# DhayaaAnbajagane/Baryonification

Measured on AMD Instinct MI355X. Metric: halos/sec for BaryonifyShell NSIDE=1024 (1000000-halo synthetic catalog), higher is better.
Workload: dtype f64 throughout in the parity-grade mode: f64 ring-row geometry, f64 pair math with 1e-11 elementary functions (fp32 seeds + one Newton step), f64 LDS accumulation, pix_offsets stored as two f32 arrays (hi + lo), f64 regrid geometry, f64 map

## Files before the change

### baryonification_amd/csrc/bfgx_api.hip

```cpp
#include <hip/hip_runtime.h>
#include <cmath>
#include <cstdarg>
#include <cstdio>
#include <algorithm>
#include <climits>
#include <cstdint>
#include <cstdlib>
#include <chrono>
#include <cstring>
#include <functional>
#include <map>
#include <mutex>
#include <string>
#include <tuple>
#include <type_traits>
#include <vector>

#include "../../include/bfgx.h"

#include "bfgx_devmem.hpp"
#include "bfgx_tile_arena.hpp"
#include "bfgx_cosmo.hpp"
#include "bfgx_kernels.hpp"
#include "bfgx_scatter2.hpp"
#include "bfgx_regrid2.hpp"
#include "bfgx_tables.hpp"
#include "bfgx_scan.hpp"
#include "bfgx_grid.hpp"
#include "bfgx_grid_pairs.hpp"
#include "bfgx_fft.hpp"
#include "bfgx_bispec.hpp"
#include "bfgx_deposit.hpp"
#include "bfgx_deposit_cloud.hpp"
#include "bfgx_snapshot.hpp"
#include "bfgx_snapshot_pairs.hpp"
#include "bfgx_grid_gather.hpp"
#include "bfgx_fftlog.hpp"
#include "bfgx_sht.hpp"
#include "bfgx_hpx.hpp"
#include "bfgx_mapstats.hpp"
#include "bfgx_pcl.hpp"
#include "bfgx_stack_core.hpp"
#include "bfgx_stack.hpp"
#include "bfgx_snapshot_stack.hpp"
#include "bfgx_grid_stack.hpp"
#include "bfgx_math_probe.hpp"

using namespace bfgx;

namespace {

thread_local std::string g_err;

int fail(int code, const char *fmt, ...)
{
    char buf[512];
    va_list ap;
    va_start(ap, fmt);
    vsnprintf(buf, sizeof(buf), fmt, ap);
    va_end(ap);
    g_err = buf;
    return code;
}

int alloc_fail(const char *what) { return fail(BFGX_ERR_HIP, kDevAllocFailed, what); }

#define HIP_TRY(expr)                                                                          \
    do {                                                                                       \
        hipError_t e_ = (expr);                                                                \
        if (e_ != hipSuccess)                                                                  \
            return fail(BFGX_ERR_HIP, "%s failed: %s (%s:%d)", #expr, hipGetErrorString(e_), __FILE__, __LINE__); \
    } while (0)

int select_device(int device)
{
    if (bfgx_device_count() <= 0) return fail(BFGX_ERR_NO_DEVICE, "no HIP device visible: libbfgx has no CPU fallback");
    HIP_TRY(hipSetDevice(device));
    return BFGX_OK;
}

int validate_cosmo(const bfgx_cosmo &c)
{
    if (!(c.Omega_m > 0) || !(c.h > 0) || !(c.Omega_b >= 0) || c.w0 != c.w0)
        return fail(BFGX_ERR_INVALID, "cosmology needs Omega_m > 0, h > 0, Omega_b >= 0, finite w0");
    return BFGX_OK;
}

int validate_table(const bfgx_table &t)
{
    if (t.ndim < 3 || t.ndim > BFGX_MAX_DIM) return fail(BFGX_ERR_INVALID, "table ndim must be in [3, %d]", BFGX_MAX_DIM);
    if (!t.values) return fail(BFGX_ERR_INVALID, "table values pointer is NULL");
    for (int d = 0; d < t.ndim; ++d) {
        if (t.n[d] < 2) return fail(BFGX_ERR_INVALID, "table axis %d needs >= 2 points", d);
        if (!t.axis[d]) return fail(BFGX_ERR_INVALID, "table axis %d pointer is NULL", d);
        for (int i = 1; i < t.n[d]; ++i)
            if (!(t.axis[d][i] > t.axis[d][i - 1]))
                return fail(BFGX_ERR_INVALID, "table axis %d must be strictly ascending", d);
    }
    double tot = 1.0;
    for (int d = 0; d < t.ndim; ++d) tot *= t.n[d];
    if (tot > 2.0e9) return fail(BFGX_ERR_INVALID, "table too large for 32-bit row offsets");
    return BFGX_OK;
}

int device_cu_count(int device)
{
    hipDeviceProp_t prop;
    return (hipGetDeviceProperties(&prop, device) == hipSuccess && prop.multiProcessorCount > 0) ? prop.multiProcessorCount : 256;
}

struct KernelEvents {
    using Pair = std::pair<hipEvent_t, hipEvent_t>;
    bool timing = false;
    std::vector<Pair> ev[BFGX_NUM_KERNELS], ev_free;
    int enable(int on) { timing = on != 0; return BFGX_OK; }
    int read(int device, hipStream_t stream, double *ms_sum, int64_t *launches)
    {
        if (!ms_sum || !launches) return fail(BFGX_ERR_INVALID, "NULL argument");
        HIP_TRY(hipSetDevice(device));
        HIP_TRY(hipStreamSynchronize(stream));
        for (int k = 0; k < BFGX_NUM_KERNELS; ++k) {
            double tot = 0.0;
            for (auto &e : ev[k]) {
                float ms = 0.f;
                HIP_TRY(hipEventElapsedTime(&ms, e.first, e.second));
                tot += ms;
                ev_free.push_back(e);
            }
            ms_sum[k] = tot;
            launches[k] = (int64_t)ev[k].size();
            ev[k].clear();
        }
        return BFGX_OK;
    }
    void destroy()
    {
        for (int k = 0; k < BFGX_NUM_KERNELS; ++k)
            for (auto &e : ev[k]) { (void)hipEventDestroy(e.first); (void)hipEventDestroy(e.second); }
        for (auto &e : ev_free) { (void)hipEventDestroy(e.first); (void)hipEventDestroy(e.second); }
    }
};

}

struct bfgx_plan {
    int device = 0, num_cus = 256;
    hipStream_t stream = nullptr;
    int64_t nside = 0, max_halos = 0;
    Hpx hpx;
    DevModel model;
    DevList mem;
    HaloRec *recs = nullptr;
    RowSetX *rowsx = nullptr;
    int NC = 4;
    int algo = 1;
    bool blocking_growth = false;
    float *k0_work_est = nullptr;
    int32_t *k1_form = nullptr;
    int64_t k1_nhalos = 0;
    int k1_fluid = 1;
    Tiling tiling;
    TileArena arena;
    int32_t *tile_start = nullptr, *entries = nullptr, *overflow = nullptr;
    int32_t *entries_a = nullptr, *slow_list = nullptr, *slow_cnt = nullptr;
    int32_t entries_a_cap = 0;
    int32_t cnt_pad = 1;
    TileRef *tref = nullptr;
    FarList far;
    int32_t *regrid_lean = nullptr;
    int auto_acc = 0;
    double table_disp_pixels = 0.0;
    int32_t *tile_apron = nullptr;
    int band_reach = 1;
    int route_margin = 0;
    int64_t cat_blk_rows = 0, cat_blk_stride = 0;
    ScanScratch scan;
    bool fast_ok = false;
    RowRec *rowrec = nullptr;
    void *pairrec = nullptr;
    FbRec *fbrec = nullptr;
    const float *tab8f = nullptr;
    const double *tab8d = nullptr;
    unsigned long long *pair_total = nullptr;
    double *tile_sums = nullptr;
    std::vector<int32_t> band_tile0_host;
    int64_t capacity = 0;
    KernelEvents events;
};

namespace {

template <class Plan>
struct KernelTimerT {
    Plan *p; int kind; KernelEvents::Pair e{nullptr, nullptr};
    KernelTimerT(Plan *p_, int kind_) : p(p_), kind(kind_)
    {
        KernelEvents &k = p->events;
        if (!k.timing) return;
        if (!k.ev_free.empty()) { e = k.ev_free.back(); k.ev_free.pop_back(); }
        else { (void)hipEventCreate(&e.first); (void)hipEventCreate(&e.second); }
        (void)hipEventRecord(e.first, p->stream);
    }
    ~KernelTimerT()
    {
        if (!p->events.timing) return;
        (void)hipEventRecord(e.second, p->stream);
        p->events.ev[kind].push_back(e);
    }
};
using KernelTimer = KernelTimerT<bfgx_plan>;

template <typename T>
static int owned_upload(DevList &mem, hipStream_t stream, const T *host, size_t count, const T *&dev_out)
{
    HIP_TRY(mem.upload(dev_out, host, count, stream));
    return BFGX_OK;
}
template <typename T>
static int owned_upload(DevList &mem, hipStream_t stream, const std::vector<T> &v, const T *&dev_out)
{
    return owned_upload(mem, stream, v.data(), v.size(), dev_out);
}

template <typename T>
static int grow_list(DevList &mem, T *&ptr, int64_t &capacity, int64_t needed)
{
    const int64_t cap = needed + needed / 4 + 1024;
    HIP_TRY(mem.regrow(ptr, (size_t)cap));
    capacity = cap;
    return BFGX_OK;
}

static int validate_model(const bfgx_model *model)
{
    if (int rc = validate_cosmo(model->cosmo_runner)) return rc;
    if (int rc = validate_cosmo(model->cosmo_model)) return rc;
    if (int rc = validate_table(model->table)) return rc;
    if (!(model->eps_runner > 0)) return fail(BFGX_ERR_INVALID, "epsilon_max must be > 0");
    if (!(model->massdef_runner.Delta > 0) || !(model->massdef_model.Delta > 0))
        return fail(BFGX_ERR_INVALID, "mass definition needs numeric Delta > 0");
    return BFGX_OK;
}

static int upload_model(DevList &mem, hipStream_t stream, const bfgx_model *model, bool with_da, DevModel &m, int &NC)
{
    const bfgx_table &t = model->table;
    std::memset(&m, 0, sizeof(m));
    m.tab.ndim = t.ndim;
    size_t nvals = 1;
    for (int d = 0; d < t.ndim; ++d) {
        m.tab.n[d] = t.n[d];
        nvals *= (size_t)t.n[d];
        if (int rc = owned_upload(mem, stream, t.axis[d], (size_t)t.n[d], m.tab.axis[d])) return rc;
    }
    {
        std::vector<double> tr;
        const double *src = t.values;
        if (t.ndim > 3) {
            const size_t nz = t.n[0], nm = t.n[1], nr = t.n[2];
            size_t nx = 1;
            for (int d = 3; d < t.ndim; ++d) nx *= (size_t)t.n[d];
            tr.resize(nvals);
            for (size_t zm = 0; zm < nz * nm; ++zm)
                for (size_t ir = 0; ir < nr; ++ir)
                    for (size_t q = 0; q < nx; ++q)
                        tr[(zm * nx + q) * nr + ir] = t.values[(zm * nr + ir) * nx + q];
            src = tr.data();
        }
        if (int rc = owned_upload(mem, stream, src, nvals, m.tab.values)) return rc;
        std::vector<float> v32(nvals);
        for (size_t q = 0; q < nvals; ++q) v32[q] = (float)src[q];
        if (int rc = owned_upload(mem, stream, v32, m.tab.values32)) return rc;
        HIP_TRY(hipStreamSynchronize(stream));
        NC = 4 << (t.ndim - 3);
    }
    m.tab.rdelta = t.rdelta_sampling;
    m.tab.logv = t.log_values;
    m.tab.eps_model = t.eps_model;
    {
        const double *g = t.axis[2];
        const int n = t.n[2];
        const double step = (g[n - 1] - g[0]) / (n - 1);
        bool uni = true;
        for (int i = 0; i < n; ++i)
            if (std::fabs(g[i] - (g[0] + i * step)) > 1e-9 * std::fabs(step)) { uni = false; break; }
        m.tab.r_uniform = uni ? 1 : 0;
        m.tab.r0 = g[0];
        m.tab.r1 = g[n - 1];
        m.tab.inv_dr = 1.0 / step;
    }
    m.bg_runner = make_background(model->cosmo_runner);
    m.bg_model = make_background(model->cosmo_model);
    m.md_runner = model->massdef_runner;
    m.md_model = model->massdef_model;
    m.eps_runner = model->eps_runner;
    m.same_model = (std::memcmp(&m.bg_runner, &m.bg_model, sizeof(Background)) == 0 && m.md_runner.Delta == m.md_model.Delta &&
                    m.md_runner.rho_type == m.md_model.rho_type) ? 1 : 0;
    if (with_da) {
        std::vector<double> knots, coef;
        da_spline(m.bg_runner, knots, coef);
        if (int rc = owned_upload(mem, stream, coef, m.da_coef)) return rc;
        m.da_step = kDaZmax / (kDaKnots - 1);
        HIP_TRY(hipStreamSynchronize(stream));
    }
    return BFGX_OK;
}

static int check_catalog(const bfgx_plan *p, const bfgx_catalog *c)
{
    if (!p || !c) return fail(BFGX_ERR_INVALID, "NULL argument");
    if (c->n < 0 || c->n > p->max_halos) return fail(BFGX_ERR_INVALID, "catalog size %lld exceeds plan max_halos %lld",
                                                     (long long)c->n, (long long)p->max_halos);
    if (c->n > 0 && (!c->M || !c->z || !c->ra || !c->dec)) return fail(BFGX_ERR_INVALID, "catalog column pointer is NULL");
    for (int k = 0; k < p->model.tab.ndim - 3; ++k)
        if (c->n > 0 && !c->extra[k]) return fail(BFGX_ERR_INVALID, "catalog is missing the column of table parameter axis %d", k);
    return BFGX_OK;
}

static bool use_fast(const bfgx_plan *p) { return p->fast_ok && p->algo == 1; }

struct DispMode {
    enum Kind { F32, F64, SPLIT } kind = F32;
    bool fp64() const { return kind != F32; }
    bool split() const { return kind == SPLIT; }
    size_t pixel_bytes() const { return fp64() ? 24 : 12; }
    float *lo(const void *offsets, int64_t n) const { return split() ? (float *)offsets + 3 * (size_t)n : nullptr; }
    int acc() const { return kind == F32 ? BFGX_ACC_F32 : kind == F64 ? BFGX_ACC_F64 : BFGX_ACC_PARITY; }
};

static int disp_mode(const bfgx_plan *p, int acc, bool one_array, DispMode &m)
{
    if (!p) return fail(BFGX_ERR_INVALID, "NULL plan");
    if (acc != BFGX_ACC_AUTO && acc != BFGX_ACC_F32 && acc != BFGX_ACC_F64 && acc != BFGX_ACC_PARITY)
        return fail(BFGX_ERR_INVALID, "acc_f64 = %d: must be BFGX_ACC_AUTO (-1), 0 (f32), 1 (f64) or BFGX_ACC_PARITY (3)", acc);
    if (acc == BFGX_ACC_AUTO) acc = p->auto_acc;
    const bool parity = acc == BFGX_ACC_PARITY && use_fast(p);
    m.kind = acc == BFGX_ACC_F32 ? DispMode::F32 : (parity && !one_array) ? DispMode::SPLIT : DispMode::F64;
    return BFGX_OK;
}

struct PaintMode {
    enum Kind { F32, F64, MIXED } kind = F64;
    bool map_f64() const { return kind != F32; }
    bool k0_f64() const { return kind == F64; }
    bool pair_f32() const { return kind == MIXED; }
};

static int paint_mode(const bfgx_plan *p, int acc, PaintMode &m)
{
    if (!p) return fail(BFGX_ERR_INVALID, "NULL plan");
    if (acc < 0 || acc > 2) return fail(BFGX_ERR_INVALID, "acc_f64 must be 0, 1 or 2");
    m.kind = acc == 0 ? PaintMode::F32 : (acc == 2 && use_fast(p)) ? PaintMode::MIXED : PaintMode::F64;
    return BFGX_OK;
}

struct TileLaunch {
    float *offsets_lo = nullptr;
    bool paint_pair_f32 = false;
    float *omax = nullptr;
    int tile_lo = 0, tile_n = -1;
    int spread_tiles = -1;
};

static int launch_prep(bfgx_plan *p, const bfgx_catalog *c, int fallback4, bool bin, bool f64, bool rec_all)
{
    if (c->n == 0) return BFGX_OK;
    const unsigned grid = (unsigned)((c->n + 255) / 256);
    KernelTimer kt(p, BFGX_K_PREP);
    PrepOut o;
    std::memset(&o, 0, sizeof(o));
    o.rec = p->recs; o.rowsx = p->rowsx;
    o.fast = (bin && use_fast(p)) ? 1 : 0;
    o.rec_all = (rec_all || !o.fast) ? 1 : 0;
    o.rowrec = p->rowrec; o.pairrec = p->pairrec; o.fbrec = p->fbrec;
    if (bin) {
        o.tref = p->tref; o.cnt_a = p->arena.cnt_a_pad; o.cnt_b = p->arena.cnt_b;
        o.cnt_pad = p->cnt_pad;
        o.work_est = o.fast ? p->k0_work_est : nullptr;
        o.entries_a = p->entries_a; o.cap_a = p->entries_a_cap; o.slow_list = p->slow_list; o.slow_cnt = p->slow_cnt;
    }
    o.ncell_m = p->model.tab.n[1] - 1; o.nrm1 = p->model.tab.n[2] - 1;
    o.blk_rows = p->cat_blk_rows; o.blk_stride = p->cat_blk_stride;
    ExtraCols ex;
    for (int k = 0; k < BFGX_MAX_EXTRA; ++k) ex.p[k] = c->extra[k];
#define BFGX_PREP(NCV, REAL)                                                                                        \
    hipLaunchKernelGGL((halo_prep_kernel<NCV, REAL>), dim3(grid), dim3(256), 0, p->stream, p->model, p->hpx, c->n, c->M, c->z, \
                       c->ra, c->dec, ex, c->ln1pz, c->lnM, fallback4, p->tiling, o)
    if (p->NC == 4) { if (f64) BFGX_PREP(4, double); else BFGX_PREP(4, float); }
    else if (p->NC == 8) BFGX_PREP(8, float);
    else if (p->NC == 16) BFGX_PREP(16, float);
    else if (p->NC == 32) BFGX_PREP(32, float);
    else BFGX_PREP(64, float);
#undef BFGX_PREP
    HIP_TRY(hipGetLastError());
    return BFGX_OK;
}

static int launch_place(bfgx_plan *p, const bfgx_catalog *c)
{
    const unsigned grid = (unsigned)((c->n + 255) / 256);
    hipLaunchKernelGGL(tile_place_kernel, dim3(grid), dim3(256), 0, p->stream, p->hpx, p->tiling, c->n,
                       (const TileRef *)p->tref, (const int32_t *)p->tile_start, p->arena.cur_b, p->entries, p->capacity, p->overflow,
                       (const int32_t *)p->slow_list, (const int32_t *)p->slow_cnt);
    HIP_TRY(hipGetLastError());
    return BFGX_OK;
}

static int launch_prep_and_bin(bfgx_plan *p, const bfgx_catalog *c, int fallback4, bool f64)
{
    p->k1_nhalos = c->n;
    HIP_TRY(hipMemsetAsync(p->arena.base, 0, p->arena.zeroed_bytes, p->stream));
    if (int rc = launch_prep(p, c, fallback4, true, f64, false)) return rc;
    KernelTimer kt(p, BFGX_K_BIN);
    const int nt_i = p->tiling.ntiles, nsb = (nt_i + kScanTilesPerWg - 1) / kScanTilesPerWg;
    const int32_t *cnt = p->arena.cnt_b;
    if (nsb <= 1 || nsb > 1024) {
        hipLaunchKernelGGL(tile_scan_kernel, dim3(1), dim3(1024), 0, p->stream, nt_i, cnt, p->tile_start);
    } else {
        int32_t *tot = p->scan.block_tot, *off = p->scan.block_off;
        hipLaunchKernelGGL(tile_scan_part_kernel<0>, dim3(nsb), dim3(1024), 0, p->stream, nt_i, cnt, p->tile_start, tot, (const int32_t *)off);
        hipLaunchKernelGGL(tile_scan_blocks_kernel, dim3(1), dim3(1024), 0, p->stream, nsb, nt_i, (const int32_t *)tot, off, p->tile_start);
        hipLaunchKernelGGL(tile_scan_part_kernel<1>, dim3(nsb), dim3(1024), 0, p->stream, nt_i, cnt, p->tile_start, tot, (const int32_t *)off);
    }
    HIP_TRY(hipGetLastError());
    if (c->n > 0) if (int rc = launch_place(p, c)) return rc;
    return BFGX_OK;
}

template <int MODE, typename ACC>
static int launch_scatter(bfgx_plan *p, int64_t n, ACC *out, int64_t *counts)
{
    if (n == 0) return BFGX_OK;
    const unsigned grid = (unsigned)((n + kWavesPerBlock - 1) / kWavesPerBlock);
    KernelTimer kt(p, MODE == MODE_OFFSETS ? BFGX_K_OFFSETS : (MODE == MODE_PAINT ? BFGX_K_PAINT : BFGX_K_COUNT));
    hipLaunchKernelGGL((halo_scatter_kernel<MODE, ACC>), dim3(grid), dim3(kWave * kWavesPerBlock), 0, p->stream,
                       make_pair_table(p->model.tab), p->hpx, n, (const HaloRec *)p->recs, out, counts);
    HIP_TRY(hipGetLastError());
    return BFGX_OK;
}

template <int MODE, typename ACC, int NC>
static int launch_tile_scatter_nc(bfgx_plan *p, ACC *out, const TileLaunch &k)
{
    constexpr int NCOMP = (MODE == MODE_OFFSETS) ? 3 : 1;
    const size_t lds = tile_lds_bytes<NC>(p->tiling.BR, p->tiling.W, NCOMP);
    auto kern = tile_scatter_kernel<MODE, ACC, NC>;
    HIP_TRY(hipFuncSetAttribute((const void *)kern, hipFuncAttributeMaxDynamicSharedMemorySize, (int)lds));
    KernelTimer kt(p, MODE == MODE_OFFSETS ? BFGX_K_OFFSETS : (MODE == MODE_PAINT ? BFGX_K_PAINT : BFGX_K_COUNT));
    const int grid = k.tile_n < 0 ? p->tiling.ntiles : std::max(k.tile_n, 1);
    hipLaunchKernelGGL(kern, dim3(grid), dim3(kWave * kWavesPerBlock), lds, p->stream,
                       make_pair_table(p->model.tab), p->hpx, p->tiling, (const HaloRec *)p->recs, (const RowSetX *)p->rowsx,
                       (const int32_t *)p->tile_start, (const int32_t *)p->entries, p->capacity, out, p->pair_total,
                       (unsigned int *)k.omax, k.tile_lo, k.tile_n);
    HIP_TRY(hipGetLastError());
    return BFGX_OK;
}

template <int MODE, typename ACC, typename real, int PM = 0>
static int launch_tile_scatter2(bfgx_plan *p, ACC *out, const TileLaunch &k, ACC *out_lo = nullptr)
{
    constexpr int NCOMP = (MODE == MODE_OFFSETS) ? 3 : 1;
    constexpr int kNP = 1;
    const size_t lds = tile2_lds_bytes<real>(p->tiling.BR, p->tiling.W, NCOMP);
    auto kern = tile_scatter2_kernel<MODE, ACC, real, kNP, PM>;
    HIP_TRY(hipFuncSetAttribute((const void *)kern, hipFuncAttributeMaxDynamicSharedMemorySize, (int)lds));
    Tab8T<real> tb;
    tb.v = (sizeof(real) == 4) ? (const real *)p->tab8f : (const real *)p->tab8d;
    tb.r0 = (real)p->model.tab.r0; tb.r1 = (real)p->model.tab.r1; tb.inv_dr = (real)p->model.tab.inv_dr;
    tb.nr = p->model.tab.n[2]; tb._pad = 0;
    unsigned int *tile_counter = p->arena.tile_counter;
    const int ntodo = k.tile_n < 0 ? p->tiling.ntiles : std::max(k.tile_n, 1);
    KernelTimer kt(p, MODE == MODE_OFFSETS ? BFGX_K_OFFSETS : (MODE == MODE_PAINT ? BFGX_K_PAINT : BFGX_K_COUNT));
    int32_t *form = nullptr;
    if constexpr (MODE != MODE_COUNT) {
        const size_t ldsf = tile2f_lds_bytes<real>(p->tiling.BR, p->tiling.W, NCOMP);
        const bool eligible = p->k1_fluid && ldsf <= (size_t)160 * 1024 && p->tiling.BR <= kWave && ntodo >= 2 * p->num_cus;
        const int nspread = k.spread_tiles > 0 ? k.spread_tiles : ntodo;
        const bool dense = (double)p->k1_nhalos * (double)p->tiling.ntiles >= 6.0e5 * (double)nspread;
        const bool forced = p->k1_fluid == 2 && ldsf <= (size_t)160 * 1024 && p->tiling.BR <= kWave;
        if (eligible && !dense && !forced && p->k0_work_est && p->k1_nhalos > 0) {
            const int nblk = (int)((p->k1_nhalos + 255) / 256);
            hipLaunchKernelGGL(k1_form_kernel, dim3(1), dim3(1024), 0, p->stream, nblk, (const float *)p->k0_work_est, 4800.0f * (float)nspread, p->k1_form);
            form = p->k1_form;
        }
        if (forced || (eligible && (dense || form))) {
            auto kf = tile_scatter2f_kernel<MODE, ACC, real, PM>;
            HIP_TRY(hipFuncSetAttribute((const void *)kf, hipFuncAttributeMaxDynamicSharedMemorySize, (int)ldsf));
            const int gridf = std::min(ntodo, p->num_cus);
            hipLaunchKernelGGL(kf, dim3(std::max(gridf, 1)), dim3(kWave * FluidWaves<real>::n), ldsf, p->stream, tb, p->hpx, p->tiling,
                               (const RowRec *)p->rowrec, (const PairRecT<real> *)p->pairrec, (const FbRec *)p->fbrec,
                               (const int32_t *)p->tile_start, (const int32_t *)p->arena.cnt_a_pad, (const int32_t *)p->arena.cnt_b,
                               (const int32_t *)p->entries, p->capacity, (const int32_t *)p->entries_a, (int)p->entries_a_cap, (int)p->cnt_pad, out, out_lo, tile_counter,
                               (unsigned int *)k.omax, k.tile_lo, k.tile_n, p->overflow, (const int32_t *)form, 1);
            HIP_TRY(hipGetLastError());
            if (!form) return BFGX_OK;
        }
    }
    const int grid = std::min(ntodo, 2 * p->num_cus);
    hipLaunchKernelGGL(kern, dim3(grid), dim3(kWave * kW2), lds, p->stream, tb, p->hpx, p->tiling,
                       (const RowRec *)p->rowrec, (const PairRecT<real> *)p->pairrec, (const FbRec *)p->fbrec,
                       (const int32_t *)p->tile_start, (const int32_t *)p->arena.cnt_a_pad, (const int32_t *)p->arena.cnt_b,
                       (const int32_t *)p->entries, p->capacity, (const int32_t *)p->entries_a, (int)p->entries_a_cap, (int)p->cnt_pad, out, out_lo, p->pair_total, tile_counter,
                       (unsigned int *)k.omax, k.tile_lo, k.tile_n, (const int32_t *)form, 0);
    HIP_TRY(hipGetLastError());
    return BFGX_OK;
}

template <int MODE, typename ACC>
static int launch_tile_scatter(bfgx_plan *p, ACC *out, const TileLaunch &k)
{
    if (use_fast(p)) {
        using real = typename std::conditional<sizeof(ACC) == 8, double, float>::type;
        if constexpr (MODE == MODE_OFFSETS && sizeof(ACC) == 4) {
            if (k.offsets_lo) return launch_tile_scatter2<MODE, ACC, double, 1>(p, out, k, (ACC *)k.offsets_lo);
        }
        if constexpr (MODE == MODE_PAINT && sizeof(ACC) == 8) {
            if (k.paint_pair_f32) return launch_tile_scatter2<MODE, ACC, float>(p, out, k);
        }
        return launch_tile_scatter2<MODE, ACC, real>(p, out, k);
    }
    if (p->NC == 4) return launch_tile_scatter_nc<MODE, ACC, 4>(p, out, k);
    if (MODE == MODE_COUNT) return launch_tile_scatter_nc<MODE, ACC, 4>(p, out, k);
    if (p->NC == 8) return launch_tile_scatter_nc<MODE, ACC, 8>(p, out, k);
    if (p->NC == 16) return launch_tile_scatter_nc<MODE, ACC, 16>(p, out, k);
    if (p->NC == 32) return launch_tile_scatter_nc<MODE, ACC, 32>(p, out, k);
    return launch_tile_scatter_nc<MODE, ACC, 64>(p, out, k);
}

static int ensure_entry_capacity(bfgx_plan *p, const bfgx_catalog *c)
{
    int32_t ov = 0, total = 0;
    HIP_TRY(hipMemcpyAsync(&ov, p->overflow, sizeof(ov), hipMemcpyDeviceToHost, p->stream));
    HIP_TRY(hipMemcpyAsync(&total, p->tile_start + p->tiling.ntiles, sizeof(total), hipMemcpyDeviceToHost, p->stream));
    HIP_TRY(hipStreamSynchronize(p->stream));
    if (!(ov & 1)) return BFGX_OK;
    HIP_TRY(p->mem.regrow(p->entries, (size_t)total + 16));
    p->capacity = (int64_t)total + 16;
    HIP_TRY(hipMemsetAsync(p->overflow, 0, sizeof(int32_t), p->stream));
    HIP_TRY(hipMemsetAsync(p->arena.cur_b, 0, p->arena.cursor_bytes, p->stream));
    return launch_place(p, c);
}

template <typename real>
static void build_tab8(const bfgx_table &t, std::vector<real> &out)
{
    const size_t nz = t.n[0], nm = t.n[1], nr = t.n[2];
    out.resize((nz - 1) * (nm - 1) * (nr - 1) * 8);
    for (size_t iz = 0; iz + 1 < nz; ++iz)
        for (size_t im = 0; im + 1 < nm; ++im)
            for (size_t i = 0; i + 1 < nr; ++i) {
                real *o = out.data() + ((iz * (nm - 1) + im) * (nr - 1) + i) * 8;
                for (int c = 0; c < 4; ++c) {
                    const double *row = t.values + ((iz + (c >> 1)) * nm + im + (c & 1)) * nr;
                    o[2 * c] = (real)row[i];
                    o[2 * c + 1] = (real)(row[i + 1] - row[i]);
                }
            }
}

static void build_tiling(int64_t nside, bool paint, int &BR, int &W, std::vector<int32_t> &tile0, std::vector<int32_t> &nphi,
                         std::vector<int32_t> &nrmin, std::vector<int32_t> &tband)
{
    auto pow2_floor = [](int64_t v) { int p = 1; while (2 * p <= v) p *= 2; return p; };
    W = std::max(16, std::min(64, pow2_floor(std::max<int64_t>(1, nside / 2))));
    BR = std::max(4, std::min(paint ? 64 : 32, pow2_floor(std::max<int64_t>(1, nside / 8))));
    if (const char *e = std::getenv("BFGX_TILE_W")) W = pow2_floor(std::max(4, std::min(64, std::atoi(e))));
    if (const char *e = std::getenv("BFGX_TILE_BR")) BR = std::max(1, std::min(64, std::atoi(e)));
    const int64_t nrings = 4 * nside - 1;
    const int nbands = (int)((nrings + BR - 1) / BR);
    auto rlen = [&](int64_t ring) { return 4 * (ring < nside ? ring : (ring > 3 * nside ? 4 * nside - ring : nside)); };
    tile0.assign(nbands + 1, 0); nphi.assign(nbands, 1); nrmin.assign(nbands, 4);
    for (int b = 0; b < nbands; ++b) {
        const int64_t i0 = 1 + (int64_t)b * BR, i1 = std::min<int64_t>(i0 + BR, 4 * nside);
        int64_t lmax = 0, lmin = INT64_MAX;
        for (int64_t i = i0; i < i1; ++i) { lmax = std::max(lmax, rlen(i)); lmin = std::min(lmin, rlen(i)); }
        nphi[b] = (int)((lmax + W - 1) / W);
        nrmin[b] = (int)lmin;
        tile0[b + 1] = tile0[b] + nphi[b];
    }
    tband.resize(tile0[nbands]);
    for (int b = 0; b < nbands; ++b)
        for (int t = tile0[b]; t < tile0[b + 1]; ++t) tband[t] = b;
}


constexpr double kAutoDispPixels = 0.1;
static void plan_pick_precision(bfgx_plan *p, const bfgx_model *model)
{
    const bfgx_table &t = model->table;
    p->auto_acc = BFGX_ACC_F32;
    p->table_disp_pixels = 0.0;
    if (t.log_values) return;
    const Background bgr = make_background(model->cosmo_runner), bgm = make_background(model->cosmo_model);
    const double pix = std::sqrt(4.0 * 3.14159265358979323846 / (double)p->hpx.npix);
    const size_t nz = t.n[0], nm = t.n[1], nr = t.n[2];
    size_t nx = 1;
    for (int d = 3; d < t.ndim; ++d) nx *= (size_t)t.n[d];
    double worst = 0.0;
    for (size_t iz = 0; iz < nz; ++iz) {
        const double z = std::exp(t.axis[0][iz]) - 1.0, a = 1.0 / (1.0 + z);
        const double D = z > 0.0 ? angular_diameter_distance(bgr, z) : 0.0;
        for (size_t im = 0; im < nm; ++im) {
            const double M = std::exp(t.axis[1][im]);
            if (!(M > 0.0) || !(a > 0.0)) continue;
            const double Rm = radius_delta(bgm, model->massdef_model, M, a) / a, Rr = radius_delta(bgr, model->massdef_runner, M, a) / a;
            const double rcut = std::min(t.eps_model * Rm, model->eps_runner * Rr);
            for (size_t ir = 0; ir < nr; ++ir) {
                const double r = std::exp(t.axis[2][ir]) * (t.rdelta_sampling ? Rm : 1.0);
                double m = 0.0;
                const double *v = t.values + ((iz * nm + im) * nr + ir) * nx;
                for (size_t q = 0; q < nx; ++q) if (std::isfinite(v[q])) m = std::max(m, std::fabs(v[q]));
                const double px = (D > 0.0) ? m * a / D / pix : (m > 0.0 ? 1.0e30 : 0.0);
                worst = std::max(worst, px);
                if (r >= rcut) break;
            }
        }
    }
    p->table_disp_pixels = worst;
    if (worst > kAutoDispPixels) p->auto_acc = BFGX_ACC_PARITY;
}

static int plan_init_fast(bfgx_plan *p, const bfgx_table &t, size_t nh)
{
    const size_t n8 = (size_t)(t.n[0] - 1) * (size_t)(t.n[1] - 1) * (size_t)(t.n[2] - 1) * 8;
    p->fast_ok = (t.ndim == 3) && p->model.tab.r_uniform && n8 * sizeof(double) <= ((size_t)256 << 20);
    if (!p->fast_ok) return BFGX_OK;
    std::vector<float> v32;
    std::vector<double> v64;
    build_tab8<float>(t, v32);
    build_tab8<double>(t, v64);
    if (int rc = owned_upload(p->mem, p->stream, v32, p->tab8f)) return rc;
    if (int rc = owned_upload(p->mem, p->stream, v64, p->tab8d)) return rc;
    if (hipStreamSynchronize(p->stream) != hipSuccess) return fail(BFGX_ERR_HIP, "stream sync failed");
    PairRecT<double> *pairrec = nullptr;
    if (p->mem.alloc(p->rowrec, nh)) return alloc_fail("row records");
    if (p->mem.alloc(pairrec, nh)) return alloc_fail("pair records");
    p->pairrec = pairrec;
    if (p->mem.alloc(p->fbrec, nh)) return alloc_fail("fallback records");
    return BFGX_OK;
}

static int plan_init_binning(bfgx_plan *p, const bfgx_table &t, size_t nh)
{
    int BR, W;
    std::vector<int32_t> tile0, nphi, nrmin, tband;
    build_tiling(p->nside, t.log_values != 0, BR, W, tile0, nphi, nrmin, tband);
    Tiling &T = p->tiling;
    T.BR = BR; T.W = W; T.nbands = (int)nphi.size(); T.ntiles = (int)tband.size();
    if (int rc = owned_upload(p->mem, p->stream, tile0, T.band_tile0)) return rc;
    p->band_tile0_host = tile0;
    if (int rc = owned_upload(p->mem, p->stream, nphi, T.band_nphi)) return rc;
    if (int rc = owned_upload(p->mem, p->stream, nrmin, T.band_nrmin)) return rc;
    if (int rc = owned_upload(p->mem, p->stream, tband, T.tile_band)) return rc;
    std::vector<int32_t> order(tband.size());
    {
        std::vector<double> weight(tband.size());
        for (size_t q = 0; q < tband.size(); ++q) { order[q] = (int32_t)q; weight[q] = (double)nrmin[tband[q]] / (double)nphi[tband[q]]; }
        std::stable_sort(order.begin(), order.end(), [&](int32_t x, int32_t y) { return weight[x] > weight[y]; });
    }
    if (int rc = owned_upload(p->mem, p->stream, order, T.tile_order)) return rc;
    {
        RingRec *rings = nullptr;
        const size_t nrec = (size_t)(4 * p->nside + 1);
        if (p->mem.alloc(rings, nrec)) return alloc_fail("ring table");
        hipLaunchKernelGGL(ring_table_kernel, dim3((unsigned)((nrec + 255) / 256)), dim3(256), 0, p->stream, p->hpx, rings);
        if (hipGetLastError() != hipSuccess) return fail(BFGX_ERR_HIP, "ring table launch failed");
        T.rings = rings;
    }
    if (hipStreamSynchronize(p->stream) != hipSuccess) return fail(BFGX_ERR_HIP, "stream sync failed");
    p->capacity = 8 * p->max_halos + 4096;
    if (const char *e = std::getenv("BFGX_K1_FLUID")) p->k1_fluid = std::max(0, std::min(2, std::atoi(e)));
    if (const char *e = std::getenv("BFGX_ENTRY_CAP")) p->capacity = std::max<int64_t>(16, std::atoll(e));
    p->cnt_pad = kCntPadMax;
    while (p->cnt_pad > 1 && (size_t)T.ntiles * p->cnt_pad * sizeof(int32_t) > ((size_t)4 << 20)) p->cnt_pad >>= 1;
    const TileArenaLayout AL = tile_arena_layout((size_t)T.ntiles, (size_t)p->cnt_pad);
    int32_t *arena = nullptr;
    if (p->mem.alloc(arena, AL.total_words) || p->mem.alloc(p->tile_start, (size_t)T.ntiles + 1) ||
        p->mem.alloc(p->entries, (size_t)p->capacity) || p->mem.alloc(p->overflow, 1) || p->mem.alloc(p->pair_total, 1) || p->mem.alloc(p->tref, nh))
        return alloc_fail("binning workspace");
    p->arena.bind(arena, AL);
    const double mean = 1.3 * (double)std::max<int64_t>(p->max_halos, 1) / (double)T.ntiles;
    int cap_a = 64;
    while (cap_a < 32768 && (double)cap_a < (mean > 512.0 ? 4.0 : 16.0) * mean + 64.0) cap_a <<= 1;
    while (cap_a > 64 && (size_t)T.ntiles * cap_a * sizeof(int32_t) > ((size_t)1 << 30)) cap_a >>= 1;
    if (const char *e = std::getenv("BFGX_TILE_LIST_CAP")) cap_a = std::max(1, std::atoi(e));
    const size_t nblk = (nh + 255) / 256;
    if (p->mem.alloc(p->k0_work_est, nblk) || p->mem.alloc(p->k1_form, 4)) return alloc_fail("work estimate");
    if (p->mem.alloc(p->entries_a, (size_t)T.ntiles * cap_a) || p->mem.alloc(p->slow_list, nblk * 256) || p->mem.alloc(p->slow_cnt, nblk))
        return alloc_fail("tile lists");
    p->entries_a_cap = cap_a;
    return BFGX_OK;
}

static int plan_init_regrid(bfgx_plan *p)
{
    const Tiling &T = p->tiling;
    const int64_t npx = p->hpx.npix;
    const int64_t want = p->table_disp_pixels < 0.25 ? npx / 16 : (p->table_disp_pixels < 2.0 ? npx / 2 : 4 * npx);
    p->far.cap = std::min<int64_t>(std::max<int64_t>((int64_t)1 << 20, want), (int64_t)1 << 28);
    if (const char *e = std::getenv("BFGX_FAR_CAP")) p->far.cap = std::max<int64_t>(1024, std::atoll(e));
    if (p->mem.alloc(p->far.pix, (size_t)p->far.cap) || p->mem.alloc(p->far.val, (size_t)p->far.cap) ||
        p->mem.alloc(p->tile_apron, 2 * (size_t)(T.ntiles + 1)))
        return alloc_fail("far list");
    if (p->mem.alloc(p->regrid_lean, (size_t)(T.ntiles + 4))) return alloc_fail("lean tile list");
    if (hipMemsetAsync(p->regrid_lean, 0, sizeof(int32_t) * 4, p->stream) != hipSuccess) return fail(BFGX_ERR_HIP, "hipMemset failed");
    p->far.count = &p->arena.ctrl->far_count;
    p->far.overflow = p->arena.band_overflow;
    if (hipMemsetAsync(p->arena.ctrl, 0, p->arena.tail_bytes, p->stream) != hipSuccess) return fail(BFGX_ERR_HIP, "hipMemset failed");
    return BFGX_OK;
}

}

extern "C" {

int bfgx_abi_version(void) { return BFGX_ABI_VERSION; }

const char *bfgx_last_error(void) { return g_err.c_str(); }

int bfgx_device_count(void)
{
    int n = 0;
    if (hipGetDeviceCount(&n) != hipSuccess) return 0;
    return n;
}

int bfgx_cosmo_E2(const bfgx_cosmo *c, int64_t n, const double *a, double *out)
{
    if (!c || !a || !out) return fail(BFGX_ERR_INVALID, "NULL argument");
    if (int rc = validate_cosmo(*c)) return rc;
    const Background b = make_background(*c);
    for (int64_t i = 0; i < n; ++i) out[i] = E2(b, a[i]);
    return BFGX_OK;
}

int bfgx_cosmo_radius(const bfgx_cosmo *c, const bfgx_massdef *md, int64_t n, const double *M, const double *a, double *out)
{
    if (!c || !md || !M || !a || !out) return fail(BFGX_ERR_INVALID, "NULL argument");
    if (int rc = validate_cosmo(*c)) return rc;
    const Background b = make_background(*c);
    for (int64_t i = 0; i < n; ++i) out[i] = radius_delta(b, *md, M[i], a[i]);
    return BFGX_OK;
}

int bfgx_cosmo_angular_diameter_distance(const bfgx_cosmo *c, int64_t n, const double *z, double *out)
{
    if (!c || !z || !out) return fail(BFGX_ERR_INVALID, "NULL argument");
    if (int rc = validate_cosmo(*c)) return rc;
    const Background b = make_background(*c);
    for (int64_t i = 0; i < n; ++i) out[i] = angular_diameter_distance(b, z[i]);
    return BFGX_OK;
}

int bfgx_cosmo_da_spline(const bfgx_cosmo *c, double *knots, double *coef)
{
    if (!c || !knots || !coef) return fail(BFGX_ERR_INVALID, "NULL argument");
    if (int rc = validate_cosmo(*c)) return rc;
    std::vector<double> k, cf;
    da_spline(make_background(*c), k, cf);
    std::memcpy(knots, k.data(), k.size() * sizeof(double));
    std::memcpy(coef, cf.data(), cf.size() * sizeof(double));
    return BFGX_OK;
}

int bfgx_cosmo_da_eval(const bfgx_cosmo *c, int64_t n, const double *z, double *out)
{
    if (!c || !z || !out) return fail(BFGX_ERR_INVALID, "NULL argument");
    if (int rc = validate_cosmo(*c)) return rc;
    std::vector<double> k, cf;
    da_spline(make_background(*c), k, cf);
    for (int64_t i = 0; i < n; ++i) out[i] = da_eval(k, cf, z[i]);
    return BFGX_OK;
}

int bfgx_plan_create(int device, void *hip_stream, int64_t nside, int64_t max_halos,
                     const bfgx_model *model, bfgx_plan **out)
{
    if (!model || !out) return fail(BFGX_ERR_INVALID, "NULL argument");
    *out = nullptr;
    if (nside < 1 || nside > 8192) return fail(BFGX_ERR_INVALID, "nside must be 1 .. 8192 (the tile kernels index pixels with 32 bits inside a ring table)");
    if (max_halos < 0) return fail(BFGX_ERR_INVALID, "max_halos < 0");
    if (int rc = validate_model(model)) return rc;
    if (bfgx_device_count() <= 0)
        return fail(BFGX_ERR_NO_DEVICE, "no HIP device visible: libbfgx has no CPU fallback");
    HIP_TRY(hipSetDevice(device));

    bfgx_plan *p = new bfgx_plan();
    p->device = device;
    {
        int cus = 0;
        if (hipDeviceGetAttribute(&cus, hipDeviceAttributeMultiprocessorCount, device) == hipSuccess && cus > 0) p->num_cus = cus;
    }
    p->nside = nside;
    p->max_halos = max_halos;
    p->hpx = make_hpx(nside);
    p->stream = (hipStream_t)hip_stream;
    auto bail = [&](int rc) { bfgx_plan_destroy(p); return rc; };

    const bfgx_table &t = model->table;
    if (int rc = upload_model(p->mem, p->stream, model, true, p->model, p->NC)) return bail(rc);
    plan_pick_precision(p, model);
    const size_t nh = (size_t)(max_halos > 0 ? max_halos : 1);
    if (p->mem.alloc(p->recs, nh)) return bail(alloc_fail("halo records"));
    if (p->NC > 4 && p->mem.alloc(p->rowsx, nh)) return bail(alloc_fail("corner rows"));
    if (int rc = plan_init_fast(p, t, nh)) return bail(rc);
    if (int rc = plan_init_binning(p, t, nh)) return bail(rc);
    if (int rc = plan_init_regrid(p)) return bail(rc);
    const ScanScratchLayout SL = scan_scratch_layout();
    int32_t *scan = nullptr;
    if (p->mem.alloc(scan, SL.total_words)) return bail(alloc_fail("tile scan scratch"));
    p->scan.bind(scan, SL);
    if (p->mem.alloc(p->tile_sums, 2 * (size_t)(p->tiling.ntiles + 1))) return bail(alloc_fail("tile sums"));
    if (hipMemsetAsync(p->overflow, 0, sizeof(int32_t), p->stream) != hipSuccess) return bail(fail(BFGX_ERR_HIP, "hipMemset failed"));
    if (hipStreamSynchronize(p->stream) != hipSuccess) return bail(fail(BFGX_ERR_HIP, "stream sync failed"));
    *out = p;
    return BFGX_OK;
}

int bfgx_plan_timing_enable(bfgx_plan *p, int on)
{
    return p ? p->events.enable(on) : fail(BFGX_ERR_INVALID, "NULL plan");
}

int bfgx_plan_timing_read(bfgx_plan *p, double *ms_sum, int64_t *launches)
{
    return p ? p->events.read(p->device, p->stream, ms_sum, launches) : fail(BFGX_ERR_INVALID, "NULL argument");
}

void bfgx_plan_destroy(bfgx_plan *p)
{
    if (!p) return;
    (void)hipSetDevice(p->device);
    (void)hipStreamSynchronize(p->stream);
    p->events.destroy();
    p->mem.release();
    delete p;
}

int bfgx_plan_set_algo(bfgx_plan *p, int algo)
{
    if (!p || (algo != 0 && algo != 1)) return fail(BFGX_ERR_INVALID, "algo must be 0 (per-halo global atomics) or 1 (LDS tiles)");
    p->algo = algo;
    return BFGX_OK;
}

int bfgx_plan_status(bfgx_plan *p)
{
    if (!p) return fail(BFGX_ERR_INVALID, "NULL plan");
    HIP_TRY(hipSetDevice(p->device));
    int32_t ov = 0;
    HIP_TRY(hipMemcpyAsync(&ov, p->overflow, sizeof(ov), hipMemcpyDeviceToHost, p->stream));
    HIP_TRY(hipStreamSynchronize(p->stream));
    if (ov & 4) {
        HIP_TRY(hipMemsetAsync(p->overflow, 0, sizeof(int32_t), p->stream));
        return fail(BFGX_ERR_HIP, "tile_scatter2f_kernel: a wave gave up waiting inside its workgroup; results are incomplete (BFGX_K1_FLUID=0 selects the other form)");
    }
    if (ov) return fail(BFGX_ERR_INVALID, "halo->tile entry list overflowed its capacity (%lld); results are incomplete",
                        (long long)p->capacity);
    int32_t fov = 0;
    HIP_TRY(hipMemcpyAsync(&fov, p->far.overflow, sizeof(fov), hipMemcpyDeviceToHost, p->stream));
    HIP_TRY(hipStreamSynchronize(p->stream));
    if (fov) {
        HIP_TRY(hipMemsetAsync(p->far.overflow, 0, sizeof(int32_t), p->stream));
        return fail(BFGX_ERR_INVALID, "the regrid's list of far deposits overflowed (%lld entries): displacements of many pixels over a large "
                                      "part of the map", (long long)p->far.cap);
    }
    return BFGX_OK;
}

int bfgx_plan_precision(bfgx_plan *p, int acc_requested, int32_t *acc_resolved, double *table_disp_pixels)
{
    DispMode m;
    if (int rc = disp_mode(p, acc_requested, false, m)) return rc;
    if (acc_resolved) *acc_resolved = m.acc();
    if (table_disp_pixels) *table_disp_pixels = p->table_disp_pixels;
    return BFGX_OK;
}

static ReachArgs reach_args(const bfgx_plan *p, double cap)
{
    const double ns = (double)p->hpx.nside, om = 1.0 / (3.0 * ns * ns);
    const double th1 = std::atan2(std::sqrt(om * (2.0 - om)), 1.0 - om);
    return ReachArgs{p->tile_apron, cap, th1, 3.14159265358979323846 - th1};
}

static int64_t ring_first_pixel(const Hpx &h, int64_t ring)
{
    const int64_t ns = h.nside, nl4 = 4 * ns;
    if (ring < 1) return 0;
    if (ring >= nl4) return h.npix;
    const int64_t q = nl4 - ring;
    return (ring < ns) ? 2 * ring * (ring - 1) : (ring < 3 * ns) ? h.ncap + (ring - ns) * 4 * ns : h.npix - 2 * q * (q + 1);
}

struct BandRange { int64_t p0, p1; int t0, nt; };
static BandRange band_range(const bfgx_plan *p, int b0, int b1)
{
    const auto first_pixel = [p](int b) { return ring_first_pixel(p->hpx, 1 + (int64_t)p->tiling.BR * b); };
    return BandRange{first_pixel(b0), first_pixel(b1), p->band_tile0_host[b0], p->band_tile0_host[b1] - p->band_tile0_host[b0]};
}

static int check_band_range(const bfgx_plan *p, int32_t b0, int32_t b1, bool tiles = false)
{
    if (tiles && p->algo != 1) return fail(BFGX_ERR_UNSUPPORTED, "band-restricted passes need the tiled algorithm (algo 1)");
    return (b0 < 0 || b1 > p->tiling.nbands || b0 > b1) ? fail(BFGX_ERR_INVALID, "band range out of bounds") : BFGX_OK;
}

static int check_scatter(const bfgx_plan *p, const bfgx_catalog *cat, const void *out, bool paint, bool bands = false, int32_t band0 = 0, int32_t band1 = 0)
{
    if (int rc = check_catalog(p, cat)) return rc;
    if (bands) if (int rc = check_band_range(p, band0, band1, true)) return rc;
    if ((p->model.tab.logv != 0) != paint) return fail(BFGX_ERR_INVALID, paint ? "profile painting needs a table with log_values = 1"
                                                                               : "displacement read-out needs a table with log_values = 0");
    if ((!bands || band0 < band1) && !out) return fail(BFGX_ERR_INVALID, paint ? "map pointer is NULL" : "offsets pointer is NULL");
    return BFGX_OK;
}

static int launch_k0(bfgx_plan *p, const bfgx_catalog *cat, int fallback4, bool f64)
{
    HIP_TRY(hipSetDevice(p->device));
    if (p->algo == 1) {
        if (int rc = launch_prep_and_bin(p, cat, fallback4, f64)) return rc;
        return p->blocking_growth ? ensure_entry_capacity(p, cat) : BFGX_OK;
    }
    if (p->NC != 4) return fail(BFGX_ERR_UNSUPPORTED, "tables with extra parameter axes need algo 1 (LDS tiles)");
    return launch_prep(p, cat, fallback4, false, false, true);
}

static int launch_offsets(bfgx_plan *p, const DispMode &m, void *slice, int64_t p0, int64_t p1, TileLaunch k1)
{
    if (m.split()) k1.offsets_lo = m.lo(slice, p1 - p0) - 3 * p0;
    if (m.kind != DispMode::F64) return launch_tile_scatter<MODE_OFFSETS, float>(p, (float *)slice - 3 * p0, k1);
    return launch_tile_scatter<MODE_OFFSETS, double>(p, (double *)slice - 3 * p0, k1);
}

static int offsets_impl(bfgx_plan *p, const bfgx_catalog *cat, void *offsets_dev, const DispMode &m, const TileLaunch &k1)
{
    if (int rc = check_scatter(p, cat, offsets_dev, false)) return rc;
    if (int rc = launch_k0(p, cat, 1, m.fp64())) return rc;
    if (p->algo == 1) return launch_offsets(p, m, offsets_dev, 0, p->hpx.npix, k1);
    if (m.fp64()) return launch_scatter<MODE_OFFSETS, double>(p, cat->n, (double *)offsets_dev, nullptr);
    return launch_scatter<MODE_OFFSETS, float>(p, cat->n, (float *)offsets_dev, nullptr);
}

int bfgx_offsets_device(bfgx_plan *p, const bfgx_catalog *cat, void *offsets_dev, int acc_f64)
{
    DispMode m;
    if (int rc = disp_mode(p, acc_f64, false, m)) return rc;
    return offsets_impl(p, cat, offsets_dev, m, TileLaunch{});
}

static int launch_paint(bfgx_plan *p, const PaintMode &m, void *slice, int64_t p0, TileLaunch k3)
{
    k3.paint_pair_f32 = m.pair_f32();
    if (m.map_f64()) return launch_tile_scatter<MODE_PAINT, double>(p, (double *)slice - p0, k3);
    return launch_tile_scatter<MODE_PAINT, float>(p, (float *)slice - p0, k3);
}

int bfgx_max_offset2_device(bfgx_plan *p, const void *offsets_dev, int64_t npixels, int acc_f64, float *out_dev)
{
    if (!p || !out_dev || (npixels > 0 && !offsets_dev)) return fail(BFGX_ERR_INVALID, "NULL argument");
    if (npixels < 0) return fail(BFGX_ERR_INVALID, "npixels < 0");
    DispMode m;
    if (int rc = disp_mode(p, acc_f64, true, m)) return rc;
    HIP_TRY(hipSetDevice(p->device));
    HIP_TRY(hipMemsetAsync(out_dev, 0, sizeof(float), p->stream));
    if (npixels > 0) {
        const unsigned grid = (unsigned)std::min<int64_t>((npixels + 255) / 256, 1024);
        if (m.fp64()) hipLaunchKernelGGL(max_offset_kernel<double>, dim3(grid), dim3(256), 0, p->stream, npixels, (const double *)offsets_dev, (unsigned *)out_dev);
        else hipLaunchKernelGGL(max_offset_kernel<float>, dim3(grid), dim3(256), 0, p->stream, npixels, (const float *)offsets_dev, (unsigned *)out_dev);
        HIP_TRY(hipGetLastError());
    }
    return BFGX_OK;
}

int bfgx_plan_set_catalog_blocks(bfgx_plan *p, int64_t rows, int64_t stride)
{
    if (!p) return fail(BFGX_ERR_INVALID, "NULL plan");
    if (rows < 0 || (rows > 0 && stride < rows)) return fail(BFGX_ERR_INVALID, "blocked catalog: rows >= 0, stride >= rows");
    p->cat_blk_rows = rows; p->cat_blk_stride = rows > 0 ? stride : 0;
    return BFGX_OK;
}

int bfgx_plan_tile_shape(bfgx_plan *p, int32_t *rings_per_band, int32_t *max_columns)
{
    if (!p) return fail(BFGX_ERR_INVALID, "NULL plan");
    if (rings_per_band) *rings_per_band = p->tiling.BR;
    if (max_columns) *max_columns = p->tiling.W;
    return BFGX_OK;
}

static int paint_impl(bfgx_plan *p, const bfgx_catalog *cat, void *map_out_dev, const PaintMode &m)
{
    if (int rc = check_scatter(p, cat, map_out_dev, true)) return rc;
    if (int rc = launch_k0(p, cat, 0, m.k0_f64())) return rc;
    if (p->algo == 1) return launch_paint(p, m, map_out_dev, 0, TileLaunch{});
    if (m.map_f64()) return launch_scatter<MODE_PAINT, double>(p, cat->n, (double *)map_out_dev, nullptr);
    return launch_scatter<MODE_PAINT, float>(p, cat->n, (float *)map_out_dev, nullptr);
}

int bfgx_paint_device(bfgx_plan *p, const bfgx_catalog *cat, void *map_out_dev, int acc_f64)
{
    PaintMode m;
    if (int rc = paint_mode(p, acc_f64, m)) return rc;
    return paint_impl(p, cat, map_out_dev, m);
}

}

constexpr int kSumTilesOneWg = 16384;
static int launch_tile_sums(bfgx_plan *p, int t0, int nt, double *sums_dev)
{
    const double *ts = p->tile_sums + 2 * (size_t)t0;
    if (nt <= kSumTilesOneWg) hipLaunchKernelGGL(sum_tiles_kernel, dim3(1), dim3(256), 0, p->stream, nt, ts, sums_dev);
    else {
        HIP_TRY(hipMemsetAsync(sums_dev, 0, 2 * sizeof(double), p->stream));
        hipLaunchKernelGGL(sum_tiles_multi_kernel, dim3(64), dim3(256), 0, p->stream, nt, ts, sums_dev);
    }
    return BFGX_OK;
}

template <typename ACC, typename real, bool SPLIT = false>
static void launch_regrid_gather(bfgx_plan *p, const double *map_in_dev, const ACC *o, const ACC *o_lo, double *map_out_dev, double *ts, bool from_k1, double *sums_dev)
{
    const size_t lds = regrid3_lds_bytes(p->tiling.BR, p->tiling.W, sizeof(real)),
                 lds_walk = regrid3_lds_bytes(p->tiling.BR, p->tiling.W, sizeof(real), true, SPLIT ? sizeof(ACC) : sizeof(real));
    FarList far = p->far;
    far.overflow = p->arena.far_overflow_full;
    const int nt = p->tiling.ntiles, nfix = std::min(nt, 2 * p->num_cus), nwalk = std::min(nt, 4 * p->num_cus);
    const ReachArgs reach = reach_args(p, regrid_cap(p->hpx.nside));
    if (!from_k1)
        hipLaunchKernelGGL(tile_reach_kernel<ACC>, dim3(nt), dim3(256), 0, p->stream, p->hpx, p->tiling, o, p->arena.omax);
    hipLaunchKernelGGL(tile_apron_kernel, dim3((nt + 255) / 256), dim3(256), 0, p->stream, p->hpx, p->tiling, (const float *)p->arena.omax, 0,
                       reach.cap, 0, nt, p->tile_apron, p->arena.todo, p->regrid_lean);
    hipLaunchKernelGGL((tile_regrid3_kernel<ACC, real, 0, SPLIT>), dim3(std::min(nt, 8 * p->num_cus)), dim3(256), lds, p->stream, p->hpx, p->tiling, map_in_dev, o, o_lo,
                       map_out_dev, far, reach, ts, -1, nt, p->regrid_lean, (double *)nullptr);
    hipLaunchKernelGGL((tile_regrid3_kernel<ACC, real, 2, SPLIT>), dim3(nwalk), dim3(256), lds_walk, p->stream, p->hpx, p->tiling, map_in_dev, o, o_lo,
                       map_out_dev, far, reach, ts, -1, nt, p->arena.todo, (double *)nullptr);
    const bool many = nt > kSumTilesOneWg && sums_dev != nullptr && ts != nullptr;
    hipLaunchKernelGGL((tile_regrid3_kernel<ACC, real, 1, SPLIT>), dim3(nfix), dim3(256), lds, p->stream, p->hpx, p->tiling, map_in_dev, o, o_lo,
                       map_out_dev, far, reach, ts, -1, nt, p->arena.todo, many ? (double *)nullptr : sums_dev, p->regrid_lean);
    if (many) (void)launch_tile_sums(p, 0, nt, sums_dev);
}

extern "C" {

static int regrid_impl(bfgx_plan *p, const double *map_in_dev, const void *offsets_dev, const DispMode &m, double *map_out_dev, double *sums_dev,
                       bool from_k1)
{
    HIP_TRY(hipSetDevice(p->device));
    {
    KernelTimer kt(p, BFGX_K_REGRID);
    if (p->algo == 1) {
        if (!from_k1) HIP_TRY(hipMemsetAsync(p->arena.ctrl, 0, sizeof(RegridCtrl), p->stream));
        double *ts = sums_dev ? p->tile_sums : nullptr;
        if (m.split())
            launch_regrid_gather<float, double, true>(p, map_in_dev, (const float *)offsets_dev, m.lo(offsets_dev, p->hpx.npix),
                                                      map_out_dev, ts, from_k1, sums_dev);
        else if (m.fp64()) launch_regrid_gather<double, double>(p, map_in_dev, (const double *)offsets_dev, (const double *)nullptr, map_out_dev, ts, from_k1, sums_dev);
        else launch_regrid_gather<float, float>(p, map_in_dev, (const float *)offsets_dev, (const float *)nullptr, map_out_dev, ts, from_k1, sums_dev);
    } else {
        const unsigned grid = (unsigned)((p->hpx.npix + 255) / 256);
        if (m.fp64())
            hipLaunchKernelGGL(regrid_kernel<double>, dim3(grid), dim3(256), 0, p->stream, p->hpx, map_in_dev,
                               (const double *)offsets_dev, map_out_dev);
        else
            hipLaunchKernelGGL(regrid_kernel<float>, dim3(grid), dim3(256), 0, p->stream, p->hpx, map_in_dev,
                               (const float *)offsets_dev, map_out_dev);
    }
    }
    HIP_TRY(hipGetLastError());
    if (sums_dev) {
        if (p->algo != 1) {
            KernelTimer kt(p, BFGX_K_SUM);
            HIP_TRY(hipMemsetAsync(sums_dev, 0, 2 * sizeof(double), p->stream));
            hipLaunchKernelGGL(sum2_kernel, dim3(1024), dim3(256), 0, p->stream, p->hpx.npix, map_in_dev,
                               (const double *)map_out_dev, sums_dev);
            HIP_TRY(hipGetLastError());
        }
    }
    return BFGX_OK;
}

int bfgx_regrid_device(bfgx_plan *p, const double *map_in_dev, const void *offsets_dev, int acc_f64,
                       double *map_out_dev, double *sums_dev)
{
    if (!p || !map_in_dev || !offsets_dev || !map_out_dev) return fail(BFGX_ERR_INVALID, "NULL argument");
    DispMode m;
    if (int rc = disp_mode(p, acc_f64, false, m)) return rc;
    return regrid_impl(p, map_in_dev, offsets_dev, m, map_out_dev, sums_dev, false);
}

int bfgx_baryonify_device(bfgx_plan *p, const bfgx_catalog *cat, const double *map_in_dev, void *offsets_work_dev, int acc_f64,
                          double *map_out_dev, double *sums_dev)
{
    if (!p || !map_in_dev || !offsets_work_dev || !map_out_dev) return fail(BFGX_ERR_INVALID, "NULL argument");
    DispMode m;
    if (int rc = disp_mode(p, acc_f64, false, m)) return rc;
    TileLaunch k1;
    const bool fused = p->algo == 1;
    if (fused) k1.omax = p->arena.omax;
    if (int rc = offsets_impl(p, cat, offsets_work_dev, m, k1)) return rc;
    return regrid_impl(p, map_in_dev, offsets_work_dev, m, map_out_dev, sums_dev, fused);
}

int bfgx_count_pairs_device(bfgx_plan *p, const bfgx_catalog *cat, int fallback4, int64_t *counts_dev, int64_t *total_host)
{
    if (int rc = check_catalog(p, cat)) return rc;
    HIP_TRY(hipSetDevice(p->device));
    if (p->algo == 1 && !counts_dev) {
        HIP_TRY(hipMemsetAsync(p->pair_total, 0, sizeof(unsigned long long), p->stream));
        if (int rc = launch_prep_and_bin(p, cat, fallback4, false)) return rc;
        if (int rc = launch_tile_scatter<MODE_COUNT, float>(p, (float *)nullptr, TileLaunch{})) return rc;
        unsigned long long tot = 0;
        HIP_TRY(hipMemcpyAsync(&tot, p->pair_total, sizeof(tot), hipMemcpyDeviceToHost, p->stream));
        HIP_TRY(hipStreamSynchronize(p->stream));
        if (total_host) *total_host = (int64_t)tot;
        return bfgx_plan_status(p);
    }
    int64_t *counts = counts_dev;
    DevBuf tmp;
    if (!counts) {
        HIP_TRY(tmp.alloc(sizeof(int64_t) * (size_t)(cat->n > 0 ? cat->n : 1)));
        counts = tmp.as<int64_t>();
    }
    int rc = launch_prep(p, cat, fallback4, false, false, true);
    if (!rc) rc = launch_scatter<MODE_COUNT, float>(p, cat->n, (float *)nullptr, counts);
    if (!rc && total_host) {
        std::vector<int64_t> h((size_t)cat->n);
        if (hipMemcpyAsync(h.data(), counts, sizeof(int64_t) * (size_t)cat->n, hipMemcpyDeviceToHost, p->stream) != hipSuccess ||
            hipStreamSynchronize(p->stream) != hipSuccess)
            rc = fail(BFGX_ERR_HIP, "count copy-back failed");
        else {
            int64_t tot = 0;
            for (int64_t v : h) tot += v;
            *total_host = tot;
        }
    } else if (!rc) {
        if (hipStreamSynchronize(p->stream) != hipSuccess) rc = fail(BFGX_ERR_HIP, "stream sync failed");
    }
    return rc;
}

}

#include "bfgx_shell_bands.inc"

#include "bfgx_route_api.inc"

#include "bfgx_oneshot.hpp"

namespace {

constexpr int kCatCols = 4 + BFGX_MAX_EXTRA + 2;
constexpr bool catalog_col_used(int i, int nex) { return i < 4 + nex || i >= 4 + BFGX_MAX_EXTRA; }

int catalog_columns(const bfgx_catalog *h, int nex, std::vector<double> &hostlog, const double *src[kCatCols])
{
    const double *lnz = h->ln1pz, *lnm = h->lnM;
    if (h->n > 0 && (!lnz || !lnm)) {
        if (!h->M || !h->z) return fail(BFGX_ERR_INVALID, "catalog column pointer is NULL");
        hostlog.resize(2 * (size_t)h->n);
        for (int64_t i = 0; i < h->n; ++i) {
            const double a = 1.0 / (1.0 + h->z[i]);
            hostlog[i] = std::log(1.0 / a);
            hostlog[(size_t)h->n + i] = std::log(h->M[i]);
        }
        if (!lnz) lnz = hostlog.data();
        if (!lnm) lnm = hostlog.data() + h->n;
    }
    src[0] = h->M; src[1] = h->z; src[2] = h->ra; src[3] = h->dec;
    for (int k = 0; k < BFGX_MAX_EXTRA; ++k) src[4 + k] = k < nex ? h->extra[k] : nullptr;
    src[4 + BFGX_MAX_EXTRA] = lnz; src[5 + BFGX_MAX_EXTRA] = lnm;
    for (int i = 0; i < kCatCols; ++i)
        if (catalog_col_used(i, nex) && h->n > 0 && !src[i]) return fail(BFGX_ERR_INVALID, "catalog column pointer is NULL");
    return BFGX_OK;
}

void catalog_view(int64_t n, int nex, const double *const col[kCatCols], bfgx_catalog *d)
{
    std::memset(d, 0, sizeof(*d));
    d->n = n;
    d->M = col[0]; d->z = col[1]; d->ra = col[2]; d->dec = col[3];
    for (int k = 0; k < nex; ++k) d->extra[k] = col[4 + k];
    d->ln1pz = col[4 + BFGX_MAX_EXTRA]; d->lnM = col[5 + BFGX_MAX_EXTRA];
}

template <class Buf, class Size>
int upload_catalog_columns(bfgx_plan *p, const bfgx_catalog *h, Buf cols[kCatCols], Size size, bfgx_catalog *d, std::vector<double> &hostlog)
{
    const int nex = p->model.tab.ndim - 3;
    const double *src[kCatCols], *dp[kCatCols] = {};
    if (int rc = catalog_columns(h, nex, hostlog, src)) return rc;
    for (int i = 0; i < kCatCols; ++i) {
        if (!catalog_col_used(i, nex)) continue;
        if (size(cols[i], sizeof(double) * (size_t)h->n)) return alloc_fail("catalog");
        if (h->n > 0) HIP_TRY(hipMemcpyAsync(cols[i].p, src[i], sizeof(double) * (size_t)h->n, hipMemcpyHostToDevice, p->stream));
        dp[i] = (const double *)cols[i].p;
    }
    catalog_view(h->n, nex, dp, d);
    return BFGX_OK;
}

int upload_catalog(bfgx_plan *p, const bfgx_catalog *h, DevBuf cols[kCatCols], bfgx_catalog *d, std::vector<double> &hostlog)
{
    return upload_catalog_columns(p, h, cols, [](DevBuf &b, size_t bytes) { return b.alloc(bytes) != hipSuccess; }, d, hostlog);
}

struct ShellEntry : CacheEntry<bfgx_plan> {
    PoolBuf cols[kCatCols], in, out, off, sums;
    uint64_t cat_token = 0;
    int64_t cat_n = -1;
    bfgx_catalog cat_dev;
};
PlanCache<ShellEntry, 4> g_shells;

std::atomic<long long> g_catalog_uploads{0};

int upload_catalog_pooled(ShellEntry *e, const bfgx_catalog *h, bfgx_catalog *d, std::vector<double> &hostlog, uint64_t token)
{
    if (token != 0 && token == e->cat_token && h->n == e->cat_n) {
        *d = e->cat_dev;
        return BFGX_OK;
    }
    e->cat_token = 0;
    g_catalog_uploads.fetch_add(1);
    auto size = [](PoolBuf &b, size_t bytes) { return b.need(std::max(bytes, sizeof(double))); };
    if (int rc = upload_catalog_columns(e->plan, h, e->cols, size, d, hostlog)) return rc;
    e->cat_token = token; e->cat_n = h->n; e->cat_dev = *d;
    return BFGX_OK;
}

int shell_begin(const bfgx_catalog *cat, const bfgx_model *model, int64_t nside, const bfgx_opts &o, ShellEntry **e)
{
    if (o.algo != 0 && o.algo != 1) return fail(BFGX_ERR_INVALID, "opts.algo must be 0 or 1");
    if (cat->n < 0) return fail(BFGX_ERR_INVALID, "catalog size < 0");
    if (int rc = validate_model(model)) return rc;
    CacheKey key = model_key(o.device, model);
    key.add(nside);
    auto make = [&](int64_t cap, bfgx_plan **p) -> int {
        if (int rc = bfgx_plan_create(o.device, nullptr, nside, cap, model, p)) return rc;
        (*p)->blocking_growth = true;
        return BFGX_OK;
    };
    if (int rc = g_shells.acquire(key, o.device, cat->n, make, [](ShellEntry *) -> int { return BFGX_OK; }, e)) return rc;
    (*e)->plan->algo = o.algo;
    return BFGX_OK;
}

constexpr int kChunksMax = 16;
struct Chunks {
    int n = 0;
    bool piped = false, stage = false;
    int cb[kChunksMax + 1] = {};
    std::vector<int64_t> bfp;
};

void chunk_plan(bfgx_plan *p, bool eligible, const PipeKnobs &knobs, Chunks &c)
{
    const size_t npix = (size_t)p->hpx.npix;
    c.n = (int)std::min<size_t>(kChunksMax, npix * sizeof(double) / ((size_t)16 << 20));
    if (knobs.stage) c.n = std::max(2, std::min(kChunksMax, knobs.chunks));
    c.stage = knobs.stage;
    c.piped = eligible && c.n >= 2 && p->tiling.nbands >= 2 * c.n && !knobs.off;
    if (!c.piped) return;
    int nb = 0;
    c.bfp.resize((size_t)p->tiling.nbands + 1);
    (void)bfgx_plan_bands(p, &nb, c.bfp.data());
    c.cb[0] = 0; c.cb[c.n] = nb;
    for (int k = 1; k < c.n; ++k) {
        const int64_t target = (int64_t)(npix * (size_t)k / c.n);
        const int b = (int)(std::lower_bound(c.bfp.begin(), c.bfp.end(), target) - c.bfp.begin());
        c.cb[k] = std::min(std::max(b, c.cb[k - 1] + 1), nb - (c.n - k));
    }
}

constexpr int kOnePass = 1;

int shell_streamed(OneShotCall &call, ShellEntry *e, const DispMode &m, const Chunks &ch, double sums[2], int64_t *first_unsent)
{
    bfgx_plan *p = e->plan;
    const int64_t npix = p->hpx.npix;
    const int kChunks = ch.n, *cb = ch.cb;
    const std::vector<int64_t> &bfp = ch.bfp;
    const double *map_in = call.src<double>(); double *map_out = call.dst<double>();
    if (int rc = e->pools(kChunks, kChunks)) return rc;
    if (e->sums.need((2 * kChunks + 2) * sizeof(double))) return alloc_fail("sums");
    double *dsums = (double *)e->sums.p;
    float *domax = (float *)(dsums + 2 * kChunks);
    int sent = 0;
    auto send = [&]() -> int {
        const int64_t lo = bfp[cb[sent]], n = bfp[cb[sent + 1]] - lo;
        HIP_TRY(hipMemcpyAsync((double *)e->in.p + lo, map_in + lo, (size_t)n * sizeof(double), hipMemcpyHostToDevice, e->up));
        HIP_TRY(hipEventRecord(e->ev_up[sent], e->up));
        *first_unsent = bfp[cb[++sent]];
        return BFGX_OK;
    };
    if (int rc = send()) return rc;
    if (int rc = send()) return rc;
    float m2 = 0.0f;
    if (int rc = bfgx_bands_max_offset2_device(p, 0, p->tiling.nbands, domax)) return rc;
    HIP_TRY(hipMemcpyAsync(&m2, domax, sizeof(float), hipMemcpyDeviceToHost, p->stream));
    HIP_TRY(hipStreamSynchronize(p->stream));
    int32_t rings = kReachMax;
    if (std::isfinite(m2)) { if (int rc = bfgx_plan_reach_rings(p, std::sqrt((double)m2), &rings)) return rc; }
    if (rings > 4) return kOnePass;
    Restore<int> reach{p->band_reach, p->band_reach};
    p->band_reach = rings;
    int next = 0;
    auto run_ready = [&]() -> int {
        while (next < kChunks) {
            int64_t olo = 0, ohi = 0;
            if (int rc = bfgx_plan_band_apron(p, cb[next], cb[next + 1], &olo, &ohi)) return rc;
            int need = next;
            while (need < kChunks - 1 && bfp[cb[need + 1]] < ohi) ++need;
            if (need >= sent) break;
            HIP_TRY(hipStreamWaitEvent(p->stream, e->ev_up[need], 0));
            const int64_t lo = bfp[cb[next]], n = bfp[cb[next + 1]] - lo;
            if (int rc = regrid_bands_impl(p, cb[next], cb[next + 1], (const double *)e->in.p, e->off.p, 0, npix, m,
                                           (double *)e->out.p + lo, dsums + 2 * next, next == 0)) return rc;
            HIP_TRY(hipEventRecord(e->ev_k[next], p->stream));
            HIP_TRY(hipStreamWaitEvent(e->down, e->ev_k[next], 0));
            HIP_TRY(hipMemcpyAsync(map_out + lo, (double *)e->out.p + lo, (size_t)n * sizeof(double), hipMemcpyDeviceToHost, e->down));
            ++next;
        }
        return BFGX_OK;
    };
    int rc = run_ready();
    while (rc == BFGX_OK && sent < kChunks) {
        rc = send();
        if (rc == BFGX_OK) rc = run_ready();
    }
    if (rc) return rc;
    if ((rc = call.mark(1, e->up)) || (rc = call.mark(2, p->stream))) return rc;
    double hs[2 * kChunksMax];
    HIP_TRY(hipMemcpyAsync(hs, dsums, sizeof(double) * 2 * (size_t)kChunks, hipMemcpyDeviceToHost, p->stream));
    HIP_TRY(hipStreamSynchronize(p->stream));
    HIP_TRY(hipStreamSynchronize(e->down));
    if ((rc = call.mark(3, p->stream))) return rc;
    for (int c = 0; c < kChunks; ++c) { sums[0] += hs[2 * c]; sums[1] += hs[2 * c + 1]; }
    int64_t nfar = 0;
    if (bfgx_plan_far_fetch(p, 0, nullptr, nullptr, &nfar) != BFGX_OK) return kOnePass;
    if (nfar > 0) {
        std::vector<int64_t> fp((size_t)nfar);
// ... 248 lines not shown
```

### baryonification_amd/csrc/bfgx_kernels.hpp

```cpp
#pragma once
#include <hip/hip_runtime.h>
#include <stdint.h>
#include "bfgx_cosmo.hpp"
#include "bfgx_math.hpp"

namespace bfgx {

constexpr double kTwoPi    = 6.283185307179586476925286766559005768394;
constexpr double kHalfPi   = 1.570796326794896619231321691639751442099;
constexpr double kInvTwoPi = 1.0 / kTwoPi;
constexpr double kTwoThird = 2.0 / 3.0;
constexpr double kDeg2Rad  = kPi / 180.0;
constexpr double kRad2Deg  = 180.0 / kPi;

constexpr int kWave = 64;
constexpr int kWavesPerBlock = 4;
constexpr int kNC = 4;

enum { MODE_OFFSETS = 0, MODE_PAINT = 1, MODE_COUNT = 2 };

struct Hpx {
    int64_t nside, npix, ncap;
    double fact1, fact2;
};
// ... 1531 lines not shown
    const int tid = threadIdx.x;
    const int lane = tid & (kWave - 1);
    const int wid = __builtin_amdgcn_readfirstlane(tid / kWave);
    if (MODE != MODE_COUNT)
        for (int i = tid; i < acc_n; i += kWave * kWavesPerBlock) acc[i] = 0.0;
    if (tid == 0) *next_chunk = 0;
    if (tid < T.BR && i0 + tid < i1) {
        const int ring = i0 + tid;
        int64_t st, n64; bool shf;
        TileRow tr;
        ring_info_small(h, ring, st, n64, shf);
        ring_z_sth(h, ring, tr.z, tr.sth);
        tr.nr = (int)n64; tr.shifted = shf ? 1 : 0;
        tr.dphi = kTwoPi / (double)tr.nr;
        tr.fnr = (double)n64 * kInvTwoPi;
        tr.ks = tile_ks(tj, tr.nr, nphi); tr.ke = tile_ks(tj + 1, tr.nr, nphi);
        rowtab[tid] = tr;
    }
    __syncthreads();

    const int e0 = tile_start[tile];
    int64_t e1 = tile_start[tile + 1];
    if (e1 > capacity) e1 = capacity;
    const int ne = (int)(e1 > e0 ? e1 - e0 : 0);
    const int chunk = max(1, min(kChunk, (ne + kWavesPerBlock - 1) / kWavesPerBlock));
    const int nchunks = (ne + chunk - 1) / chunk;
    TileWaveLds &L = wl[wid];
    unsigned long long npairs = 0;

    while (true) {
        int c = 0;
        if (lane == 0) c = atomicAdd(next_chunk, 1);
        c = __shfl(c, 0, kWave);
        if (c >= nchunks) break;

        int nrows = 0;
        if (lane < chunk && c * chunk + lane < ne) {
            const int hidx = entries[e0 + c * chunk + lane];
            const HaloRec &r = recs[hidx];
            RingSlot rs;
            rs.z0 = r.z0; rs.xa = r.xa; rs.cosr = r.cosr; rs.phi0 = r.phi0;
            rs.irmin = r.irmin; rs.irmax = r.irmax; rs.fb = r.fb; rs.hidx = hidx;
            if (r.fb) { nrows = 4; rs.ring_lo = 0; }
            else {
                const int lo = max(r.rfirst, i0), hi = min(r.rlast, i1 - 1);
                nrows = max(0, hi - lo + 1);
                rs.ring_lo = lo;
            }
            rs.prefix = 0;
            L.ring[lane] = rs;
            load_pair_halo<NC>(L.pair[lane], r, hidx, rowsx);
        }
        const int incl_e = wave_scan_incl(nrows, lane);
        const int total_rows = __shfl(incl_e, kWave - 1, kWave);
        if (lane < kChunk) L.ring[lane].prefix = incl_e - nrows;
        __builtin_amdgcn_wave_barrier();

        for (int rb = 0; rb < total_rows; rb += kWave) {
            const int R = rb + lane;
            int firstA = 0, cntA = 0, firstB = 0, cntB = 0, nr = 1, ldsbase = 0, es = 0;
            double z = 0.0, sth = 0.0, shift = 0.0, dphv = 0.0;
            if (R < total_rows) {
                int e = 0;
#pragma unroll
                for (int st = kChunk >> 1; st > 0; st >>= 1)
                    if (L.ring[e + st].prefix <= R) e += st;
                es = e;
                const RingSlot &rs = L.ring[e];
                const int q = R - rs.prefix;
                if (rs.fb) {
                    const HaloRec &hr = recs[rs.hidx];
                    const int ring = hr.fb_ring[q], fk = hr.fb_k[q];
                    if (ring >= i0 && ring < i1) {
                        const TileRow &tr = rowtab[ring - i0];
                        z = tr.z; sth = tr.sth; nr = tr.nr; shift = tr.shifted ? 0.5 : 0.0; dphv = tr.dphi;
                        if (fk >= tr.ks && fk < tr.ke) { firstA = fk; cntA = 1; }
                        ldsbase = (ring - i0) * T.W - tr.ks;
                    }
                } else {
                    const int ring = rs.ring_lo + q;
                    const TileRow &tr = rowtab[ring - i0];
                    int slo, scnt;
                    disc_row_span(tr.nr, tr.shifted != 0, tr.z, tr.fnr, ring, rs.z0, rs.xa, rs.cosr, rs.phi0, rs.irmin, rs.irmax, slo, scnt);
                    nr = tr.nr; z = tr.z; sth = tr.sth; shift = tr.shifted ? 0.5 : 0.0; dphv = tr.dphi;
                    const int ks = tr.ks, ke = tr.ke;
                    const int endA = min(slo + scnt, nr);
                    firstA = max(slo, ks);
                    cntA = max(0, min(endA, ke) - firstA);
                    const int endB = slo + scnt - nr;
                    firstB = ks;
                    cntB = max(0, min(endB, ke) - firstB);
                    ldsbase = (ring - i0) * T.W - ks;
                }
            }
            const int cnt = cntA + cntB;
            const int incl = wave_scan_incl(cnt, lane);
            const int total = __shfl(incl, kWave - 1, kWave);
            npairs += (unsigned long long)total;
            if (MODE != MODE_COUNT && total > 0) {
                const int nwords = (total + kWave - 1) / kWave + 2;
                for (int wI = lane; wI < nwords; wI += kWave) L.mask[wI] = 0ull;
                __builtin_amdgcn_wave_barrier();
                const unsigned long long ne = __ballot(cnt > 0);
                const unsigned long long lt = (1ull << lane) - 1ull;
                if (cnt > 0) {
                    const int slot = __popcll(ne & lt);
                    const int pre = incl - cnt;
                    L.prefix[slot] = pre;
                    L.firstA[slot] = firstA; L.cntA[slot] = cntA; L.firstB[slot] = firstB;
                    L.ldsbase[slot] = ldsbase; L.eslot[slot] = es;
                    L.z[slot] = z; L.sth[slot] = sth;
                    L.dphi[slot] = dphv; L.xoff[slot] = shift * dphv - L.pair[es].phi0;
                    atomicOr(&L.mask[pre >> 6], 1ull << (pre & 63));
                }
                __builtin_amdgcn_wave_barrier();

                const unsigned long long le = lt | (1ull << lane);
                const bool fastok = pt.r_uniform != 0;
                int base = 0;
                for (int T0 = 0; T0 < total; T0 += 2 * kWave) {
                    const unsigned long long mA = L.mask[T0 >> 6], mB = L.mask[(T0 >> 6) + 1];
                    const int tA = T0 + lane, tB = T0 + kWave + lane;
                    const bool actA = tA < total, actB = tB < total;
                    const int rowA = actA ? base + __popcll(mA & le) - 1 : 0;
                    base += __popcll(mA);
                    const int rowB = actB ? base + __popcll(mB & le) - 1 : 0;
                    base += __popcll(mB);
                    int kA, kB; double xA, xB;
                    {
                        const int jj = tA - L.prefix[rowA], ca = L.cntA[rowA];
                        kA = (jj < ca) ? (L.firstA[rowA] + jj) : (L.firstB[rowA] + (jj - ca));
                        xA = fold_dphi(__builtin_fma((double)kA, L.dphi[rowA], L.xoff[rowA]));
                    }
                    {
                        const int jj = tB - L.prefix[rowB], ca = L.cntA[rowB];
                        kB = (jj < ca) ? (L.firstA[rowB] + jj) : (L.firstB[rowB] + (jj - ca));
                        xB = fold_dphi(__builtin_fma((double)kB, L.dphi[rowB], L.xoff[rowB]));
                    }
                    const PairH &hA = L.pair[L.eslot[rowA]], &hB = L.pair[L.eslot[rowB]];
                    double vA[3], vB[3];
                    bool okA, okB;
                    const bool small = (!actA || fabs(xA) <= 0.5) && (!actB || fabs(xB) <= 0.5);
                    if (fastok && __all(small)) {
                        if (MODE == MODE_OFFSETS && sizeof(ACC) == 4) {
                            okA = pair_value_fast32<NC>(pt, hA, L.z[rowA], L.sth[rowA], xA, vA);
                            okB = pair_value_fast32<NC>(pt, hB, L.z[rowB], L.sth[rowB], xB, vB);
                        } else {
                            okA = pair_value_fast<MODE, NC>(pt, hA, L.z[rowA], L.sth[rowA], xA, vA);
                            okB = pair_value_fast<MODE, NC>(pt, hB, L.z[rowB], L.sth[rowB], xB, vB);
                        }
                    } else {
                        okA = okB = false;
#pragma unroll 1
                        for (int pass = 0; pass < 2; ++pass) {
                            const PairH &hh = pass ? hB : hA;
                            const int rw = pass ? rowB : rowA;
                            double vv[3] = {0.0, 0.0, 0.0};
                            const bool ok = pair_value<MODE, NC>(pt, hh, L.z[rw], L.sth[rw], (pass ? xB : xA) + hh.phi0, vv);
                            if (pass) { okB = ok; vB[0] = vv[0]; vB[1] = vv[1]; vB[2] = vv[2]; }
                            else { okA = ok; vA[0] = vv[0]; vA[1] = vv[1]; vA[2] = vv[2]; }
                        }
                    }
                    if (actA && okA) {
                        double *o = acc + NCOMP * (L.ldsbase[rowA] + kA);
                        for (int cc = 0; cc < NCOMP; ++cc) atomicAdd(o + cc, vA[cc]);
                    }
                    if (actB && okB) {
                        double *o = acc + NCOMP * (L.ldsbase[rowB] + kB);
                        for (int cc = 0; cc < NCOMP; ++cc) atomicAdd(o + cc, vB[cc]);
                    }
                }
            }
            __builtin_amdgcn_wave_barrier();
        }
    }
    __syncthreads();

    if (MODE == MODE_COUNT) {
        if (lane == 0 && npairs) atomicAdd(pair_total, npairs);
        continue;
    }
    float mcomp = 0.0f;
    for (int rr = wid; rr < i1 - i0; rr += kWavesPerBlock) {
        const int ring = i0 + rr;
        int64_t st, n64; bool shf;
        ring_info_small(h, ring, st, n64, shf);
        const int nr = (int)n64;
        const int ks = tile_ks(tj, nr, nphi), ke = tile_ks(tj + 1, nr, nphi);
        const int n = (ke - ks) * NCOMP;
        ACC *dst = out + NCOMP * (st + ks);
        const double *src = acc + NCOMP * rr * T.W;
        for (int x = lane; x < n; x += kWave) { const ACC v = (ACC)src[x]; dst[x] = v; mcomp = fmaxf(mcomp, fabsf((float)v)); }
    }
    if (MODE == MODE_OFFSETS && omax2 != nullptr) {
#pragma unroll
        for (int sft = kWave >> 1; sft > 0; sft >>= 1) mcomp = fmaxf(mcomp, __shfl_down(mcomp, sft, kWave));
        if (lane == 0 && mcomp > 0.0f) atomicMax(omax2 + tile, __float_as_uint(3.0f * mcomp * mcomp * 1.0001f));
    }
    __syncthreads();
    }
}

template <typename ACC>
__global__ void __launch_bounds__(256)
regrid_kernel(Hpx h, const double *__restrict__ map_in, const ACC *__restrict__ offsets,
              double *__restrict__ map_out)
{
    const int64_t p = (int64_t)blockIdx.x * blockDim.x + threadIdx.x;
    if (p >= h.npix) return;
    const double val = map_in[p];
    if (!(val > 0.0)) return;
    double z, sth, phi;
    pix2loc(h, p, z, sth, phi);
    double s, c;
    sincos(phi, &s, &c);
    const double nx = sth * c + (double)offsets[3 * p + 0];
    const double ny = sth * s + (double)offsets[3 * p + 1];
    const double nz = z + (double)offsets[3 * p + 2];
    const double dnorm = sqrt(nx * nx + ny * ny + nz * nz);
    const double theta = acos(nz / dnorm);
    double ph = atan2(ny, nx);
    if (ph < 0) ph += kTwoPi;
    const double lon = ph * kRad2Deg, lat = 90.0 - theta * kRad2Deg;
    const double th2 = kHalfPi - lat * kDeg2Rad, ph2 = lon * kDeg2Rad;
    int64_t cp[4]; double w[4];
    get_interpol<true>(h, th2, ph2, cp, w);
#pragma unroll
    for (int k = 0; k < 4; ++k) atomicAdd(map_out + cp[k], w[k] * val);
}

__device__ inline double ring_theta(const Hpx &h, int ring)
{
    int64_t st, nr; double th; bool sh;
    ring_info2(h, ring, st, nr, th, sh);
    return th;
}

struct RegRow {
    double theta, z, sth;
    double dphi, inv_dphi;
    double c0, s0;
    int64_t start;
    int32_t nr, ks, ke, shf;
    double lim2;
};

__device__ inline double ring_theta_nolibm(const Hpx &h, int ring)
{
    double z, sth;
    ring_z_sth(h, ring, z, sth);
    return atan2_generic(sth, z);
}

struct alignas(16) RingRec {
    double theta, z, sth;
    double dphi, inv_dphi;
    double inv_dth_up, inv_dth_dn;
    int64_t start;
    int32_t nr, shifted;
};
static_assert(sizeof(RingRec) == 80, "RingRec: five 16-byte loads");

__global__ void __launch_bounds__(256)
ring_table_kernel(Hpx h, RingRec *__restrict__ rings)
{
    const int nl4 = (int)(4 * h.nside);
    const int ring = blockIdx.x * 256 + threadIdx.x;
    if (ring > nl4) return;
    RingRec g;
    g.theta = (ring < 1) ? -1.0e300 : 1.0e300;
    g.z = g.sth = g.dphi = g.inv_dphi = g.inv_dth_up = g.inv_dth_dn = 0.0;
    g.start = 0; g.nr = 0; g.shifted = 0;
    if (ring >= 1 && ring <= nl4 - 1) {
        int64_t st, nr64; bool shf;
        ring_info_small(h, ring, st, nr64, shf);
        ring_z_sth(h, ring, g.z, g.sth);
        g.theta = atan2_generic(g.sth, g.z);
        g.start = st; g.nr = (int)nr64; g.shifted = shf ? 1 : 0;
        g.dphi = kTwoPi / (double)g.nr;
        g.inv_dphi = (double)g.nr * kInvTwoPi;
        if (ring > 1) g.inv_dth_up = 1.0 / (g.theta - ring_theta_nolibm(h, ring - 1));
        if (ring < nl4 - 1) g.inv_dth_dn = 1.0 / (ring_theta_nolibm(h, ring + 1) - g.theta);
    }
    rings[ring] = g;
}

__global__ void __launch_bounds__(256)
ring_functions_kernel(Hpx h, int first, int n, RingRec *__restrict__ out)
{
    const int i = blockIdx.x * 256 + threadIdx.x;
    if (i >= n) return;
    const int ring = first + i;
    RingRec g;
    g.dphi = g.inv_dphi = g.inv_dth_up = g.inv_dth_dn = 0.0;
    int64_t nr64; bool shf;
    ring_info_small(h, ring, g.start, nr64, shf);
    g.nr = (int)nr64; g.shifted = shf ? 1 : 0;
    ring_z_sth(h, ring, g.z, g.sth);
    g.theta = ring_theta_nolibm(h, ring);
    out[i] = g;
}

__global__ void __launch_bounds__(256)
sum_tiles_kernel(int ntiles, const double *__restrict__ tile_sums, double *__restrict__ sums)
{
    __shared__ double sa[256 / kWave], sb[256 / kWave];
    double xa = 0.0, xb = 0.0;
    for (int t = threadIdx.x; t < ntiles; t += 256) { xa += tile_sums[2 * t]; xb += tile_sums[2 * t + 1]; }
#pragma unroll
    for (int s = kWave >> 1; s > 0; s >>= 1) { xa += __shfl_down(xa, s, kWave); xb += __shfl_down(xb, s, kWave); }
    const int lane = threadIdx.x & (kWave - 1), wid = threadIdx.x / kWave;
    if (lane == 0) { sa[wid] = xa; sb[wid] = xb; }
    __syncthreads();
    if (threadIdx.x == 0) {
        double ta = 0.0, tb = 0.0;
        for (int w = 0; w < 256 / kWave; ++w) { ta += sa[w]; tb += sb[w]; }
        sums[0] = ta; sums[1] = tb;
    }
}

__global__ void __launch_bounds__(256)
sum_tiles_multi_kernel(int ntiles, const double *__restrict__ tile_sums, double *__restrict__ sums)
{
    __shared__ double sa[256 / kWave], sb[256 / kWave];
    double xa = 0.0, xb = 0.0;
    const double2 *ts = reinterpret_cast<const double2 *>(tile_sums);
    for (int t = blockIdx.x * 256 + threadIdx.x; t < ntiles; t += gridDim.x * 256) { const double2 v = ts[t]; xa += v.x; xb += v.y; }
#pragma unroll
    for (int s = kWave >> 1; s > 0; s >>= 1) { xa += __shfl_down(xa, s, kWave); xb += __shfl_down(xb, s, kWave); }
    const int lane = threadIdx.x & (kWave - 1), wid = threadIdx.x / kWave;
    if (lane == 0) { sa[wid] = xa; sb[wid] = xb; }
    __syncthreads();
    if (threadIdx.x == 0) {
        double ta = 0.0, tb = 0.0;
        for (int w = 0; w < 256 / kWave; ++w) { ta += sa[w]; tb += sb[w]; }
        atomicAdd(sums + 0, ta); atomicAdd(sums + 1, tb);
    }
}

__global__ void __launch_bounds__(256)
sum2_kernel(int64_t n, const double *__restrict__ a, const double *__restrict__ b, double *__restrict__ sums)
{
    __shared__ double sa[256 / kWave], sb[256 / kWave];
    double xa = 0.0, xb = 0.0;
    for (int64_t i = (int64_t)blockIdx.x * blockDim.x + threadIdx.x; i < n; i += (int64_t)gridDim.x * blockDim.x) {
        xa += a[i]; xb += b[i];
    }
#pragma unroll
    for (int s = kWave >> 1; s > 0; s >>= 1) { xa += __shfl_down(xa, s, kWave); xb += __shfl_down(xb, s, kWave); }
    const int lane = threadIdx.x & (kWave - 1), wid = threadIdx.x / kWave;
    if (lane == 0) { sa[wid] = xa; sb[wid] = xb; }
    __syncthreads();
    if (threadIdx.x == 0) {
        double ta = 0.0, tb = 0.0;
        for (int w = 0; w < 256 / kWave; ++w) { ta += sa[w]; tb += sb[w]; }
        atomicAdd(sums + 0, ta);
        atomicAdd(sums + 1, tb);
    }
}

}
```

### baryonification_amd/csrc/bfgx_regrid2.hpp

```cpp
#pragma once
#include "bfgx_kernels.hpp"
#include "bfgx_scatter2.hpp"

namespace bfgx {

template <typename real>
struct alignas(16) RegRowC {
    real z, sth, dphi, inv_dphi;
    real c0, s0;
    real inv_dth_up, inv_dth_dn;
};
template <>
struct alignas(16) RegRowC<double> { double inv_dth_up, inv_dth_dn; };
template <typename real> struct RowGeom { real z, sth, dphi, inv_dphi, c0, s0, inv_dth_up, inv_dth_dn; };
__device__ inline RowGeom<float> row_geom(const RegRow *, const RegRowC<float> *rowc, int t)
{
    const RegRowC<float> c = rowc[t];
    return RowGeom<float>{c.z, c.sth, c.dphi, c.inv_dphi, c.c0, c.s0, c.inv_dth_up, c.inv_dth_dn};
}
__device__ inline RowGeom<double> row_geom(const RegRow *rows, const RegRowC<double> *rowc, int t)
{
    const RegRow &r = rows[t];
    const RegRowC<double> c = rowc[t];
    return RowGeom<double>{r.z, r.sth, r.dphi, r.inv_dphi, r.c0, r.s0, c.inv_dth_up, c.inv_dth_dn};
}
__device__ inline float row_inv_dphi(const RegRow *, const RegRowC<float> *rowc, int t) { return rowc[t].inv_dphi; }
__device__ inline double row_inv_dphi(const RegRow *rows, const RegRowC<double> *, int t) { return rows[t].inv_dphi; }
__host__ __device__ inline size_t regrowc_bytes(size_t real_size) { return real_size == 4 ? sizeof(RegRowC<float>) : sizeof(RegRowC<double>); }

__device__ inline void regrid_targets_generic(const Hpx &h, const RingRec *__restrict__ rings, const RegRow *rows, int LR, int rth0, int ti, int x,
                                                    double o0, double o1, double o2, int tr[4], int tk[4], double w[4])
{
    const int nl4 = (int)(4 * h.nside);
    const RegRow &rw = rows[ti];
    const double z = rw.z, sth = rw.sth;
    const double phi = ((double)(rw.ks + x) + (rw.shf ? 0.5 : 0.0)) * rw.dphi;
    double s, c;
    sincos_bounded(phi, s, c);
    const double nx = sth * c + o0, ny = sth * s + o1, nz = z + o2;
    const double xr = nx * c + ny * s, yr = ny * c - nx * s;
    const double inv = fast_rsq(nx * nx + ny * ny + nz * nz);
    const double zc = nz * inv;
    const double tq = yr * fast_rcp(xr);
    const double sn = fast_sqrt(xr * xr + yr * yr) * inv;
    const double q = sn * z - zc * sth;
    double theta, ph;
    if (xr > 0.0 && fabs(tq) <= 0.1 && fabs(q) <= 0.05) {
        ph = phi + atan_small(tq);
        theta = rw.theta + asin_small(q);
    } else {
        theta = atan2_generic(sn, zc);
        ph = atan2_generic(ny, nx);
    }
    if (ph < 0) ph += kTwoPi;
    if (ph >= kTwoPi) ph -= kTwoPi;
    int t1 = ti;
    while (t1 > 0 && theta < rows[t1].theta) --t1;
    while (t1 < LR + 1 && theta >= rows[t1 + 1].theta) ++t1;
    const bool in_window = (theta >= rows[t1].theta) && (t1 < LR + 1) && (theta < rows[t1 + 1].theta);
    const int ir1 = in_window ? rth0 + t1 : (int)ring_above(h, zc);
    const int ir2 = ir1 + 1;
    double theta1 = 0.0, theta2 = 0.0;
    for (int q4 = 0; q4 < 4; ++q4) { tr[q4] = 0; tk[q4] = 0; w[q4] = 0.0; }
#pragma unroll
    for (int half = 0; half < 2; ++half) {
        const int ir = half ? ir2 : ir1;
        if (half ? (ir < nl4) : (ir > 0)) {
            const int t2 = ir - rth0;
            int n2; double shd, invd, th;
            if (t2 >= 0 && t2 < LR + 2) {
                const RegRow &r2 = rows[t2];
                n2 = r2.nr; shd = r2.shf ? 0.5 : 0.0; invd = r2.inv_dphi; th = r2.theta;
            } else {
                const RingRec &g2 = rings[ir];
                n2 = g2.nr; shd = g2.shifted ? 0.5 : 0.0; invd = g2.inv_dphi; th = g2.theta;
            }
            const double tmp = ph * invd - shd;
            int j1 = (int)floor(tmp);
            const double w1 = tmp - (double)j1;
            int j2 = j1 + 1;
            if (j1 < 0) j1 += n2;
            if (j2 >= n2) j2 -= n2;
            tr[2 * half] = ir; tr[2 * half + 1] = ir;
            tk[2 * half] = j1; tk[2 * half + 1] = j2;
            w[2 * half] = 1.0 - w1; w[2 * half + 1] = w1;
            if (half) theta2 = th; else theta1 = th;
        }
    }
    if (ir1 == 0) {
        const double wtheta = theta / theta2;
        w[2] *= wtheta; w[3] *= wtheta;
        const double fac = (1.0 - wtheta) * 0.25;
        w[0] = fac; w[1] = fac; w[2] += fac; w[3] += fac;
        tr[0] = 1; tr[1] = 1; tk[0] = (tk[2] + 2) & 3; tk[1] = (tk[3] + 2) & 3;
    } else if (ir2 == nl4) {
        const double wtheta = (theta - theta1) / (kPi - theta1);
        w[0] *= (1.0 - wtheta); w[1] *= (1.0 - wtheta);
        const double fac = wtheta * 0.25;
        w[0] += fac; w[1] += fac; w[2] = fac; w[3] = fac;
        tr[2] = nl4 - 1; tr[3] = nl4 - 1; tk[2] = (tk[0] + 2) & 3; tk[3] = (tk[1] + 2) & 3;
    } else {
        const double wtheta = (theta - theta1) * fast_rcp(theta2 - theta1);
        w[0] *= (1.0 - wtheta); w[1] *= (1.0 - wtheta);
        w[2] *= wtheta; w[3] *= wtheta;
    }
}

__device__ inline float abs_(float v) { return __builtin_fabsf(v); }
__device__ inline double abs_(double v) { return __builtin_fabs(v); }
template <typename real> struct RMath;
template <> struct RMath<float> {
    static __device__ inline float rcp(float x) { const float y = __builtin_amdgcn_rcpf(x); return y * __builtin_fmaf(-x, y, 2.0f); }
    static __device__ inline float inv_norm(float e) { return fma_(e, fma_(e, fma_(e, fma_(e, 0.2734375f, -0.3125f), 0.375f), -0.5f), 1.0f); }
    static __device__ inline float sqrt1pm1(float t2) { return t2 * fma_(t2, fma_(t2, 0.0625f, -0.125f), 0.5f); }
    static __device__ inline float asin_(float q) { const float q2 = q * q; return q * fma_(q2, fma_(q2, fma_(q2, (float)(15.0 / 336.0), 0.075f), (float)(1.0 / 6.0)), 1.0f); }
    static __device__ inline float atan_(float t) { const float t2 = t * t; return t * fma_(t2, fma_(t2, fma_(t2, fma_(t2, (float)(1.0 / 9.0), (float)(-1.0 / 7.0)), 0.2f), (float)(-1.0 / 3.0)), 1.0f); }
};
template <> struct RMath<double> {
    static __device__ inline double rcp(double x) { return fast_rcp(x); }
    static __device__ inline double inv_norm(double e) { return fast_rsq(1.0 + e); }
    static __device__ inline double sqrt1pm1(double t2) { const double h = 1.0 + t2; return t2 * fast_rcp(1.0 + h * fast_rsq(h)); }
    static __device__ inline double asin_(double q) { return asin_small(q); }
    static __device__ inline double atan_(double t) { return atan_small(t); }
};

struct RMathE {
    static __device__ inline double rcp(double x) { const double y = (double)__builtin_amdgcn_rcpf((float)x); return __builtin_fma(y, __builtin_fma(-x, y, 1.0), y); }
    static __device__ inline double inv_norm(double e)
    {
        const double x = 1.0 + e, y = (double)__builtin_amdgcn_rsqf((float)x);
        const double h = 0.5 * y, r = __builtin_fma(-x * y, h, 0.5);
        return __builtin_fma(y, r, y);
    }
    static __device__ inline double sqrt1pm1(double t2) { return t2 * __builtin_fma(t2, __builtin_fma(t2, __builtin_fma(t2, __builtin_fma(t2, 7.0 / 256.0, -5.0 / 128.0), 0.0625), -0.125), 0.5); }
    static __device__ inline double asin_(double q) { const double q2 = q * q; return q * __builtin_fma(q2, __builtin_fma(q2, __builtin_fma(q2, 15.0 / 336.0, 0.075), 1.0 / 6.0), 1.0); }
    static __device__ inline double atan_(double t)
    {
        const double t2 = t * t;
        return t * __builtin_fma(t2, __builtin_fma(t2, __builtin_fma(t2, __builtin_fma(t2, __builtin_fma(t2, -1.0 / 11.0, 1.0 / 9.0), -1.0 / 7.0), 0.2), -1.0 / 3.0), 1.0);
    }
};

constexpr int kReachMax = 16;
constexpr int kReachColsMax = 256;

__host__ __device__ inline double regrid_cap(int64_t nside)
{
    const double c = 9.9 / (double)nside;
    return c < 0.02 ? c : 0.02;
}
__host__ __device__ inline int regrid_reach_rings(int64_t nside, double m)
{
    const double r = m * 1.5 * (double)nside;
    const int R = (r < (double)kReachMax ? (int)r : kReachMax) + 1;
    return R > kReachMax ? kReachMax : R;
}
__host__ __device__ inline double regrid_cap_for_rings(int64_t nside, int R)
{
    const double c = 0.999 * (double)R / (1.5 * (double)nside), cap = regrid_cap(nside);
    return (R >= kReachMax || c > cap) ? cap : c;
}

struct alignas(16) RowScan {
    int32_t start, nr, ks, span;
    float need2, cf2, lim2;
    int32_t klr;
};

struct FarList {
    unsigned long long *count;
    int64_t *pix;
    double *val;
    int64_t cap;
    int32_t *overflow;
};

struct ReachArgs {
    const int32_t *apron;
    double cap;
    double theta_first, theta_last;
};

constexpr int kWalkQ = 128;
constexpr int kWalkFar = (256 / kWave) * kWalkQ;
__host__ __device__ inline size_t regrid3_lds_bytes(int BR, int W, size_t real_size, bool walk = false, size_t acc_size = 0)
{
    if (acc_size == 0) acc_size = real_size;
    const size_t base = (size_t)BR * W * sizeof(double) + (size_t)(BR + 2 * kReachMax + 2) * (sizeof(RegRow) + regrowc_bytes(real_size)) + 16;
    if (!walk) return base;
    return base + (size_t)(BR + 2 * kReachMax + 2) * sizeof(RowScan) + (size_t)(256 / kWave) * kWalkQ * (sizeof(double) + sizeof(int32_t) + 3 * acc_size)
           + (size_t)(kWalkFar + 4) * sizeof(int32_t);
}

template <typename ACC>
__global__ void __launch_bounds__(256)
tile_reach_kernel(Hpx h, Tiling T, const ACC *__restrict__ offsets, float *__restrict__ tile_omax)
{
    __shared__ float red[256 / kWave];
    const int tile = blockIdx.x;
    const int band = T.tile_band[tile];
    const int nphi = T.band_nphi[band];
    const int tj = tile - T.band_tile0[band];
    const int nl4 = (int)(4 * h.nside);
    const int i0 = 1 + band * T.BR, i1 = min(i0 + T.BR, nl4);
    const int lane = threadIdx.x & (kWave - 1), wid = threadIdx.x / kWave;
    float m2 = 0.0f;
    for (int ring = i0 + wid; ring < i1; ring += 256 / kWave) {
        int64_t st, nr64; bool shf;
        ring_info_small(h, ring, st, nr64, shf);
        const int nr = (int)nr64, ks = tile_ks(tj, nr, nphi), ke = tile_ks(tj + 1, nr, nphi);
        const ACC *o = offsets + 3 * (st + ks);
        for (int x = lane; x < ke - ks; x += kWave) {
            const float a = (float)o[3 * x], b = (float)o[3 * x + 1], c = (float)o[3 * x + 2];
            m2 = fmaxf(m2, fma_(a, a, fma_(b, b, c * c)));
        }
    }
#pragma unroll
    for (int sft = kWave >> 1; sft > 0; sft >>= 1) m2 = fmaxf(m2, __shfl_down(m2, sft, kWave));
    if (lane == 0) red[wid] = m2;
    __syncthreads();
    if (threadIdx.x == 0) {
        for (int w = 1; w < 256 / kWave; ++w) m2 = fmaxf(m2, red[w]);
        tile_omax[tile] = m2;
    }
}

__global__ void __launch_bounds__(256)
tile_apron_kernel(Hpx h, Tiling T, const float *__restrict__ tile_omax, int rings, double cap, int tile0, int ntiles,
                  int32_t *__restrict__ apron, int32_t *__restrict__ todo, int32_t *__restrict__ lean = nullptr)
{
    const int i = blockIdx.x * 256 + threadIdx.x;
    bool is_lean = false;
    if (i < ntiles) {
    const int tile = tile0 + i;
    const int band = T.tile_band[tile];
    const int nphi = T.band_nphi[band];
    const int tj = tile - T.band_tile0[band];
    const int nl4 = (int)(4 * h.nside);
    float m = (float)cap;
    int R = rings;
    if (tile_omax != nullptr) {
        m = 0.0f;
        const int nb = (kReachMax + T.BR - 1) / T.BR;
        for (int db = -nb; db <= nb; ++db) {
            const int b2 = band + db;
            if (b2 < 0 || b2 >= T.nbands) continue;
            const int n2 = T.band_nphi[b2], t20 = T.band_tile0[b2];
            int lo = (int)(((int64_t)tj * n2) / nphi) - 1, hi = (int)(((int64_t)(tj + 1) * n2 + nphi - 1) / nphi) + 1;
            if (T.W < 32 || hi - lo >= n2) { lo = 0; hi = n2; }
            for (int t2 = lo; t2 < hi; ++t2) {
                const int u = t2 < 0 ? t2 + n2 : (t2 >= n2 ? t2 - n2 : t2);
                m = fmaxf(m, tile_omax[t20 + u]);
            }
        }
        const bool still = !(m > 0.0f);
        m = fminf(__builtin_sqrtf(m) * 1.001f, (float)cap);
        R = still ? 0 : regrid_reach_rings(h.nside, (double)m);
    }
    const int i0 = 1 + band * T.BR, i1 = min(i0 + T.BR, nl4);
    const int rlo = max(i0 - R, 1), rhi = min(i1 + R, nl4) - 1, ns = (int)h.nside;
    int nmin = 0x7fffffff, nmax = 0;
    float mc = 0.0f;
    const int probe[4] = {rlo, rhi, ns, 3 * ns};
#pragma unroll
    for (int q = 0; q < 4; ++q) {
        const int ring = probe[q];
        if (ring < rlo || ring > rhi) continue;
        double z, sth;
        ring_z_sth(h, ring, z, sth);
        const int nr = ring_len(h, ring);
        nmin = min(nmin, nr); nmax = max(nmax, nr);
        const float limf = fminf(m, (float)(0.09 * sth)), den = (float)sth - limf;
        if (den > 0.0f) mc = fmaxf(mc, limf / den * 1.02f * (float)nr * (float)kInvTwoPi);
    }
    const float kk = mc + (float)nmax / (float)nmin + 2.5f;
    apron[2 * tile] = R;
    apron[2 * tile + 1] = (nphi == 1) ? 0 : (kk < (float)kReachColsMax ? (int)kk + 1 : kReachColsMax);
    if (todo != nullptr && R > 1) todo[1 + atomicAdd(todo, 1)] = tile;
    is_lean = R <= 1;
    }
    if (lean != nullptr) {
        const unsigned long long m = __ballot(is_lean);
        if (m) {
            const int lane = threadIdx.x & (kWave - 1), leader = __ffsll((long long)m) - 1;
            int base = 0;
            if (lane == leader) base = atomicAdd(lean, __popcll(m));
            base = __shfl(base, leader, kWave);
            const int pos = base + __popcll(m & ((1ull << lane) - 1ull));
            if (is_lean && pos < ntiles) lean[1 + pos] = tile0 + i;
        }
    }
}

template <typename ACC>
__global__ void __launch_bounds__(256)
max_offset_kernel(int64_t n, const ACC *__restrict__ offsets, unsigned *__restrict__ out)
{
    float m2 = 0.0f;
    for (int64_t i = (int64_t)blockIdx.x * 256 + threadIdx.x; i < n; i += (int64_t)gridDim.x * 256) {
        const float a = (float)offsets[3 * i], b = (float)offsets[3 * i + 1], c = (float)offsets[3 * i + 2];
        m2 = fmaxf(m2, fma_(a, a, fma_(b, b, c * c)));
    }
#pragma unroll
    for (int sft = kWave >> 1; sft > 0; sft >>= 1) m2 = fmaxf(m2, __shfl_down(m2, sft, kWave));
    __shared__ float wm[256 / kWave];
    if ((threadIdx.x & (kWave - 1)) == 0) wm[threadIdx.x / kWave] = m2;
    __syncthreads();
    if (threadIdx.x == 0) {
        float m = 0.0f;
        for (int w = 0; w < 256 / kWave; ++w) m = fmaxf(m, wm[w]);
        if (m > 0.0f) atomicMax(out, __float_as_uint(m));
    }
}

__global__ void __launch_bounds__(1024)
max_bits_kernel(int n, const unsigned *__restrict__ v, unsigned *__restrict__ out)
{
    unsigned m = 0u;
    for (int i = threadIdx.x; i < n; i += 1024) m = max(m, v[i]);
#pragma unroll
    for (int sft = kWave >> 1; sft > 0; sft >>= 1) m = max(m, (unsigned)__shfl_down((int)m, sft, kWave));
    if ((threadIdx.x & (kWave - 1)) == 0 && m) atomicMax(out, m);
}

template <typename real, bool WALK, bool ECON = false>
__device__ inline bool regrid_gather_targets(const RegRow *rows, const RegRowC<real> *rowc, int NT, int ti, int x,
                                             real o0, real o1, real o2, int tt[4], int tk[4], real w[4])
{
    using RM = typename std::conditional<ECON, RMathE, RMath<real>>::type;
    using PMx = typename std::conditional<ECON, PMathE, PMath<real>>::type;
    const RowGeom<real> rc = row_geom(rows, rowc, ti);
    const RegRow &rw = rows[ti];
    real c, s;
    const real alpha = (real)x * rc.dphi;
    if (abs_(alpha) <= (real)0.45) {
        real sa, oma;
        PMx::sin_omc(alpha, sa, oma);
        c = rc.c0 - (rc.c0 * oma + rc.s0 * sa);
        s = rc.s0 - (rc.s0 * oma - rc.c0 * sa);
    } else {
        double s64, c64;
        sincos_bounded(((double)(rw.ks + x) + (rw.shf ? 0.5 : 0.0)) * rw.dphi, s64, c64);
        c = (real)c64; s = (real)s64;
    }
    const real a = o0 * c + o1 * s, b = o1 * c - o0 * s;
    const real xr = rc.sth + a;
    const real t = b * RM::rcp(xr);
    const real t2 = t * t;
    const real e = (real)2 * (rc.sth * a + rc.z * o2) + (a * a + b * b + o2 * o2);
    const real invn = RM::inv_norm(e);
    const real q = (fma_(a, rc.z, -(o2 * rc.sth)) + xr * rc.z * RM::sqrt1pm1(t2)) * invn;
    const real dth = RM::asin_(q);
    const real dph = RM::atan_(t);
    const bool down = dth >= (real)0;
    const real wq = down ? dth * rc.inv_dth_dn : -dth * rc.inv_dth_up;
    int t1 = ti;
    real wtheta;
    const bool near = wq < (real)1 && (down ? rc.inv_dth_dn : rc.inv_dth_up) > (real)0;
    if (!WALK || near) {
        wtheta = down ? wq : (real)1 - wq;
    } else {
        const double d = (double)dth, th0 = rw.theta;
        const int stp = (int)(wq < (real)(2 * kReachMax) ? wq : (real)(2 * kReachMax));
        t1 = down ? ti + stp : ti - 1 - stp;
        t1 = t1 < 0 ? 0 : (t1 > NT - 2 ? NT - 2 : t1);
        while (t1 + 2 < NT && d >= rows[t1 + 1].theta - th0) ++t1;
        while (t1 > 0 && d < rows[t1].theta - th0) --t1;
        const double lo = rows[t1].theta - th0, hi = rows[t1 + 1].theta - th0;
        if (!(d >= lo && d < hi) || rows[t1].nr == 0 || rows[t1 + 1].nr == 0) return false;
        wtheta = (real)((d - lo) * fast_rcp(hi - lo));
    }
    const int nro = rw.nr;
    int kown = rw.ks + x;
    if (kown < 0) kown += nro;
    if (kown >= nro) kown -= nro;
    auto other_ring = [&](int tr, int &j, real &wj) {
        const RegRow &rn = rows[tr];
        const double B = ((double)kown + (rw.shf ? 0.5 : 0.0)) * ((double)rn.nr * rw.dphi * kInvTwoPi) - (rn.shf ? 0.5 : 0.0);
        const double Bf = floor(B);
        const real wall = (real)(B - Bf) + dph * row_inv_dphi(rows, rowc, tr), f = __builtin_floor(wall);
        wj = wall - f; j = (int)Bf + (int)f;
    };
    const bool nr_ = !WALK || near;
    const bool x_upper = !nr_ || down;
    const int tx = nr_ ? ti : t1, ty = nr_ ? (down ? ti + 1 : ti - 1) : t1 + 1;
    int jx, jy; real wx, wy;
    if (nr_) {
        const real wall = dph * rc.inv_dphi, f = __builtin_floor(wall);
        wx = wall - f; jx = kown + (int)f;
    } else {
        other_ring(tx, jx, wx);
    }
    other_ring(ty, jy, wy);
    const int nrx = rows[tx].nr, nry = rows[ty].nr;
    int jx2 = jx + 1, jy2 = jy + 1;
    jx = jx < 0 ? jx + nrx : (jx >= nrx ? jx - nrx : jx);
    jx2 = jx2 < 0 ? jx2 + nrx : (jx2 >= nrx ? jx2 - nrx : jx2);
    jy = jy < 0 ? jy + nry : (jy >= nry ? jy - nry : jy);
    jy2 = jy2 < 0 ? jy2 + nry : (jy2 >= nry ? jy2 - nry : jy2);
    const real wtx = x_upper ? (real)1 - wtheta : wtheta, wty = (real)1 - wtx;
    tt[0] = tx; tt[1] = tx; tk[0] = jx; tk[1] = jx2;
    w[0] = ((real)1 - wx) * wtx; w[1] = wx * wtx;
    tt[2] = ty; tt[3] = ty; tk[2] = jy; tk[3] = jy2;
    w[2] = ((real)1 - wy) * wty; w[3] = wy * wty;
    return true;
}

__device__ inline double regrid_far_pixel(
    const Hpx &h, const RingRec *__restrict__ rings, const RegRow *rows, int LR, int rth0, int ti, int x, double o0, double o1, double o2,
                                                double val, FarList far)
{
    int tr[4], tk[4];
    double w[4], tot = 0.0;
    regrid_targets_generic(h, rings, rows, LR, rth0, ti, x, o0, o1, o2, tr, tk, w);
    const unsigned long long act = __ballot(1);
    const int rank = (int)__builtin_amdgcn_mbcnt_hi((unsigned)(act >> 32), __builtin_amdgcn_mbcnt_lo((unsigned)act, 0u));
    const int leader = __ffsll((long long)act) - 1;
    unsigned long long base = 0;
    if (rank == 0) base = atomicAdd(far.count, 4ull * (unsigned long long)__popcll(act));
    base = ((unsigned long long)(unsigned)__shfl((int)(base >> 32), leader, kWave) << 32) | (unsigned)__shfl((int)base, leader, kWave);
    for (int q4 = 0; q4 < 4; ++q4) {
        const double v = w[q4] * val;
        const unsigned long long i = base + 4ull * (unsigned long long)rank + (unsigned long long)q4;
        if ((int64_t)i < far.cap) { far.pix[i] = rings[tr[q4]].start + tk[q4]; far.val[i] = v; } else atomicOr(far.overflow, 1);
        tot += v;
    }
    return tot;
}

constexpr int kK2Occ = 4;
template <typename ACC, typename real, int PASS, bool SPLIT = false>
__global__ void __launch_bounds__(256, kK2Occ)
tile_regrid3_kernel(Hpx h, Tiling T, const double *__restrict__ map_in, const ACC *__restrict__ offsets, const ACC *__restrict__ offsets_lo,
                    double *__restrict__ map_out, FarList far, ReachArgs reach, double *__restrict__ tile_sums, int tile_off, int ntiles,
                    int *__restrict__ todo, double *__restrict__ sums_out, int *__restrict__ lean_reset = nullptr)
{
    static_assert(!SPLIT || (sizeof(ACC) == 4 && sizeof(real) == 8), "split pix_offsets: fp32 halves, fp64 geometry");
    extern __shared__ __align__(16) unsigned char smem[];
    const int NTmax = T.BR + 2 * kReachMax + 2;
    double *acc = reinterpret_cast<double *>(smem);
    RegRow *rows = reinterpret_cast<RegRow *>(acc + T.BR * T.W);
    RegRowC<real> *rowc = reinterpret_cast<RegRowC<real> *>(rows + NTmax);
    const int tid = threadIdx.x;
    const int nl4 = (int)(4 * h.nside);
    if (PASS == 1 && lean_reset != nullptr && blockIdx.x == 0 && tid == 0) *lean_reset = 0;
    if (PASS == 1 && sums_out != nullptr && blockIdx.x == 0) {
        double sa = 0.0, sb = 0.0;
        for (int i = tid; i < ntiles; i += 256) { sa += tile_sums[2 * (int64_t)i]; sb += tile_sums[2 * (int64_t)i + 1]; }
#pragma unroll
        for (int sft = kWave >> 1; sft > 0; sft >>= 1) { sa += __shfl_down(sa, sft, kWave); sb += __shfl_down(sb, sft, kWave); }
        double *red = reinterpret_cast<double *>(smem);
        if ((tid & (kWave - 1)) == 0) { red[2 * (tid / kWave)] = sa; red[2 * (tid / kWave) + 1] = sb; }
        __syncthreads();
        if (tid == 0) {
            double ta = 0.0, tb = 0.0;
            for (int w = 0; w < 256 / kWave; ++w) { ta += red[2 * w]; tb += red[2 * w + 1]; }
            sums_out[0] = ta; sums_out[1] = tb;
        }
        __syncthreads();
    }
    if (PASS == 1 && *far.overflow == 0) {
        const unsigned long long n = *far.count;
        for (unsigned long long i = (unsigned long long)blockIdx.x * 256 + tid; i < n; i += (unsigned long long)gridDim.x * 256)
            atomicAdd(map_out + far.pix[i], far.val[i]);
        return;
    }
    const bool listed = (PASS == 2 || PASS == 0) && todo != nullptr;
    if (listed) ntiles = min(todo[0], ntiles);
    for (int blk = blockIdx.x; blk < ntiles; blk += ((PASS == 0 && !listed) ? ntiles : (int)gridDim.x)) {
    const int tile = listed ? todo[1 + blk] : ((tile_off < 0) ? T.tile_order[blk] : tile_off + blk);
    const int band = T.tile_band[tile];
    const int nphi = T.band_nphi[band];
    const int tj = tile - T.band_tile0[band];
    const int i0 = 1 + band * T.BR;
    const int i1 = min(i0 + T.BR, nl4);
    double sum_in = 0.0, sum_out = 0.0;
    __syncthreads();

    const int R = (PASS == 2) ? reach.apron[2 * tile] : 1;
    const int kap = (PASS == 1 || nphi == 1) ? 0 : reach.apron[2 * tile + 1];
    if (PASS == 0 && reach.apron[2 * tile] > 1) continue;
    if (PASS == 0 && reach.apron[2 * tile] == 0) {
        const int lane = tid & (kWave - 1), wid = tid / kWave;
        for (int rr = wid; rr < i1 - i0; rr += 256 / kWave) {
            const int64_t st = T.rings[i0 + rr].start;
            const int nr = T.rings[i0 + rr].nr, ks = tile_ks(tj, nr, nphi), ke = tile_ks(tj + 1, nr, nphi);
            for (int k = ks + lane; k < ke; k += kWave) {
                const double v = map_in[st + k];
                const double dep = (v > 0.0) ? v : 0.0;
                map_out[st + k] = dep;
                sum_in += v; sum_out += dep;
            }
        }
        if (tile_sums) {
#pragma unroll
            for (int sft = kWave >> 1; sft > 0; sft >>= 1) { sum_in += __shfl_down(sum_in, sft, kWave); sum_out += __shfl_down(sum_out, sft, kWave); }
            if (lane == 0) { acc[2 * wid] = sum_in; acc[2 * wid + 1] = sum_out; }
            __syncthreads();
            if (tid == 0) {
                double sa_ = 0.0, sb_ = 0.0;
                for (int wv = 0; wv < 256 / kWave; ++wv) { sa_ += acc[2 * wv]; sb_ += acc[2 * wv + 1]; }
                tile_sums[2 * (int64_t)tile] = sa_; tile_sums[2 * (int64_t)tile + 1] = sb_;
            }
        }
        continue;
    }
    for (int i = tid; i < T.BR * T.W; i += 256) acc[i] = 0.0;
    const int NT = T.BR + 2 * R + 2;
    const int rth0 = i0 - R - 1;
    if (tid < NT) {
        const int ring = rth0 + tid;
        const RingRec g = T.rings[min(max(ring, 0), nl4)];
        RegRow rw;
        rw.theta = g.theta; rw.z = g.z; rw.sth = g.sth; rw.dphi = g.dphi; rw.inv_dphi = g.inv_dphi;
        rw.c0 = rw.s0 = 0.0;
        rw.start = g.start; rw.nr = g.nr; rw.ks = 0; rw.ke = 0; rw.shf = g.shifted; rw.lim2 = 0.0;
        if (g.nr > 0) {
            rw.ks = tile_ks(tj, rw.nr, nphi);
            rw.ke = tile_ks(tj + 1, rw.nr, nphi);
            sincos_bounded(((double)rw.ks + (g.shifted ? 0.5 : 0.0)) * rw.dphi, rw.s0, rw.c0);
            const double lim = fmin(fmin(reach.cap, 0.09 * rw.sth), 0.999 * fmin(rw.theta - reach.theta_first, reach.theta_last - rw.theta));
            rw.lim2 = (lim > 0.0 && ring > 1 && ring < nl4 - 1) ? (double)(float)(lim * lim) : 0.0;
        }
        rows[tid] = rw;
        RegRowC<real> rc;
        if constexpr (sizeof(real) == 4) {
            rc.z = (real)rw.z; rc.sth = (real)rw.sth; rc.dphi = (real)rw.dphi; rc.inv_dphi = (real)rw.inv_dphi;
            rc.c0 = (real)rw.c0; rc.s0 = (real)rw.s0;
        }
        rc.inv_dth_up = (tid > 0) ? (real)g.inv_dth_up : (real)0;
        rc.inv_dth_dn = (tid < NT - 1) ? (real)g.inv_dth_dn : (real)0;
        rowc[tid] = rc;
        if (PASS == 2) {
            RowScan *scan = reinterpret_cast<RowScan *>(rowc + NTmax);
            const int T0 = R + 1, T1 = R + (i1 - i0);
            const RingRec &gup = T.rings[i0 - 1], &gdn = T.rings[i1];
            double need = 0.0;
            if (tid < T0 - 1 && gup.nr > 0) need = gup.theta - rw.theta;
            else if (tid > T1 + 1 && gdn.nr > 0) need = rw.theta - gdn.theta;
            const float nf = (rw.nr > 0 && need > 0.0) ? (float)(0.999 * need) : 0.0f;
            const double den = rw.sth - fast_sqrt(rw.lim2);
            const float cf = (rw.nr > 0 && den > 0.0) ? (float)(1.02 * rw.inv_dphi / den) : 3.0e18f;
            const int span = rw.ke - rw.ks, rest = rw.nr - span;
            const int kl = min(kap, rest >> 1), kr = min(kap, rest - kl);
            RowScan rs;
            rs.start = (int32_t)rw.start; rs.nr = rw.nr; rs.ks = rw.ks; rs.span = span;
            rs.need2 = nf * nf; rs.cf2 = cf * cf; rs.lim2 = (float)rw.lim2;
            rs.klr = kl | (kr << 10) | ((tid >= T0 && tid <= T1) ? (1 << 20) : 0);
            scan[tid] = rs;
        }
    }
    if (PASS == 2 && tid == 0) reinterpret_cast<int32_t *>(reinterpret_cast<RowScan *>(rowc + NTmax) + NTmax)[0] = 0;
    __syncthreads();
    auto far_add = [&](int64_t p, double v) {
        if (PASS != 1) {
            const unsigned long long i = atomicAdd(far.count, 1ull);
            if ((int64_t)i < far.cap) { far.pix[i] = p; far.val[i] = v; } else atomicOr(far.overflow, 1);
            sum_out += v;
        } else {
            atomicAdd(map_out + p, v);
        }
    };

    const int NR = T.BR + 2 * R;
    int maxspan = 0, nrmin = 0x7fffffff, nrmax = 1;
    for (int i = 1; i <= NR; ++i) {
        maxspan = max(maxspan, rows[i].ke - rows[i].ks);
        if (PASS == 2 && rows[i].nr > 0) { nrmin = min(nrmin, rows[i].nr); nrmax = max(nrmax, rows[i].nr); }
    }
    const int LWs = maxspan + 2 * kap;
    const unsigned inv_lws = (unsigned)((0x100000000ull + (unsigned)LWs - 1u) / (unsigned)LWs);
    using OT = typename std::conditional<SPLIT, double, ACC>::type;
    struct Src { int ti, x; bool ok, own; double val; OT o0, o1, o2; float hsq; };
    auto fetch = [&](int idx) {
        Src sx;
        sx.ok = false; sx.own = false; sx.ti = 0; sx.x = 0; sx.val = 0.0; sx.o0 = sx.o1 = sx.o2 = (OT)0; sx.hsq = 0.0f;
        if (idx < NR * LWs) {
            const int r = (int)__umulhi((unsigned)idx, inv_lws), x = idx - r * LWs - kap;
            const RegRow &rw = rows[r + 1];
            const int span = rw.ke - rw.ks, rest = rw.nr - span;
            const int kl = min(kap, rest >> 1), kr = min(kap, rest - kl);
            if (rw.nr > 0 && x >= -kl && x < span + kr) {
                int k = rw.ks + x;
                if (k < 0) k += rw.nr;
                if (k >= rw.nr) k -= rw.nr;
                const int64_t p = rw.start + k;
                sx.own = (r >= R) && (r < R + (i1 - i0)) && (x >= 0) && (x < span);
                if (PASS != 1 || sx.own) {
                    sx.ok = true; sx.ti = r + 1; sx.x = x;
                    sx.val = map_in[p];
                    if (SPLIT) {
                        const ACC h0 = offsets[3 * p + 0], h1 = offsets[3 * p + 1], h2 = offsets[3 * p + 2];
                        const ACC l0 = offsets_lo[3 * p + 0], l1 = offsets_lo[3 * p + 1], l2 = offsets_lo[3 * p + 2];
                        sx.o0 = (OT)((double)h0 + (double)l0); sx.o1 = (OT)((double)h1 + (double)l1); sx.o2 = (OT)((double)h2 + (double)l2);
                        sx.hsq = (float)fma_(h0, h0, fma_(h1, h1, h2 * h2));
                    } else {
                    sx.o0 = offsets[3 * p + 0]; sx.o1 = offsets[3 * p + 1]; sx.o2 = offsets[3 * p + 2];
                    }
                }
            }
        }
        return sx;
    };
    if constexpr (PASS == 2) {
        const int lane = tid & (kWave - 1), wid = __builtin_amdgcn_readfirstlane(tid / kWave);
        const RowScan *scan = reinterpret_cast<const RowScan *>(rowc + NTmax);
        int32_t *nfar = reinterpret_cast<int32_t *>(const_cast<RowScan *>(scan) + NTmax), *farq = nfar + 4;
        double *qval = reinterpret_cast<double *>(farq + kWalkFar) + wid * kWalkQ;
        using QT = typename std::conditional<SPLIT, ACC, real>::type;
        QT *qo = reinterpret_cast<QT *>(reinterpret_cast<double *>(farq + kWalkFar) + (256 / kWave) * kWalkQ) + wid * 3 * kWalkQ;
        int32_t *qpos = reinterpret_cast<int32_t *>(reinterpret_cast<QT *>(reinterpret_cast<double *>(farq + kWalkFar) + (256 / kWave) * kWalkQ)
                                                    + (256 / kWave) * 3 * kWalkQ) + wid * kWalkQ;
        const float colslack = 2.5f + (float)nrmax / (float)nrmin;
        const int nown = i1 - i0, total = NR * LWs;
        auto deposit = [&](int ti, int x, QT q0, QT q1, QT q2, double val) {
            int tt[4], tk[4];
            real w[4];
            real o0 = (real)q0, o1 = (real)q1, o2 = (real)q2;
            if (SPLIT) {
                const RegRow &rs_ = rows[ti];
                int k = rs_.ks + x;
                k += (k < 0) ? rs_.nr : 0;
                k -= (k >= rs_.nr) ? rs_.nr : 0;
                const int64_t p = rs_.start + k;
                o0 += (real)offsets_lo[3 * p + 0]; o1 += (real)offsets_lo[3 * p + 1]; o2 += (real)offsets_lo[3 * p + 2];
            }
            if (!regrid_gather_targets<real, true, SPLIT>(rows, rowc, NT, ti, x, o0, o1, o2, tt, tk, w)) return;
#pragma unroll
            for (int q4 = 0; q4 < 4; ++q4) {
                const int rr = tt[q4] - (R + 1);
                if (rr >= 0 && rr < nown) {
                    const RegRow &rt = rows[tt[q4]];
                    if (tk[q4] >= rt.ks && tk[q4] < rt.ke) {
                        const double v = (double)w[q4] * val;
                        atomicAdd(acc + rr * T.W + (tk[q4] - rt.ks), v);
                    }
                }
            }
        };
        auto far_from = [&](int pk) {
            const int ti = pk >> 16, x = (pk & 0xffff) - kap;
            const RegRow &rw = rows[ti];
            int k = rw.ks + x;
            if (k < 0) k += rw.nr;
            if (k >= rw.nr) k -= rw.nr;
            const int64_t p = rw.start + k;
            double f0 = (double)offsets[3 * p + 0], f1 = (double)offsets[3 * p + 1], f2 = (double)offsets[3 * p + 2];
            if (SPLIT) { f0 += (double)offsets_lo[3 * p + 0]; f1 += (double)offsets_lo[3 * p + 1]; f2 += (double)offsets_lo[3 * p + 2]; }
            sum_out += regrid_far_pixel(h, T.rings, rows, NT - 2, rth0, ti, x, f0, f1, f2, map_in[p], far);
        };
        int32_t *fq = farq + wid * kWalkQ;
        int fn = 0;
        int qn = 0;
        constexpr int U = 2;
        const int64_t pdummy = rows[R + 1].start + rows[R + 1].ks;
        for (int base = wid * kWave; base < total; base += 256 * U) {
            int cpos[U], cx[U], cspan[U];
            bool cin[U], cown[U];
            float cneed2[U], ccf2[U], clim2[U];
            ACC ca0[U], ca1[U], ca2[U];
            double cval[U];
#pragma unroll
            for (int u = 0; u < U; ++u) {
                const int idx = base + u * 256 + lane, idc = min(idx, total - 1);
                const int r = (int)__umulhi((unsigned)idc, inv_lws), x = idc - r * LWs - kap;
                const RowScan rs = scan[r + 1];
                cx[u] = x; cpos[u] = ((r + 1) << 16) | (x + kap); cspan[u] = rs.span;
                cneed2[u] = rs.need2; ccf2[u] = rs.cf2; clim2[u] = rs.lim2;
                cin[u] = idx < total && rs.nr > 0 && x >= -(rs.klr & 1023) && x < rs.span + ((rs.klr >> 10) & 1023);
                cown[u] = cin[u] && (rs.klr >> 20) && x >= 0 && x < rs.span;
                int k = rs.ks + x;
                k += (k < 0) ? rs.nr : 0;
                k -= (k >= rs.nr) ? rs.nr : 0;
                const int64_t p = cin[u] ? (int64_t)(rs.start + k) : pdummy;
                ca0[u] = offsets[3 * p + 0]; ca1[u] = offsets[3 * p + 1]; ca2[u] = offsets[3 * p + 2];
                cval[u] = map_in[p];
            }
            bool cpush[U], cfar[U];
#pragma unroll
            for (int u = 0; u < U; ++u) {
                const int x = cx[u];
                if (cown[u]) sum_in += cval[u];
                const QT o0 = (QT)ca0[u], o1 = (QT)ca1[u], o2 = (QT)ca2[u];
                const QT osq = fma_(o0, o0, fma_(o1, o1, o2 * o2));
                const bool live = cin[u] && cval[u] > 0.0;
                const bool gathered = osq < (QT)clim2[u];
                const int dc = x < 0 ? -x : (x >= cspan[u] ? x - cspan[u] + 1 : 0);
                const float g = (float)dc - colslack, of = (float)osq;
                const bool reaches = cown[u] || (of >= cneed2[u] && (g <= 0.0f || of * ccf2[u] >= g * g));
                cpush[u] = live && gathered && reaches;
                cfar[u] = live && !gathered && cown[u];
            }
#pragma unroll
            for (int u = 0; u < U; ++u) {
                const unsigned long long m = __ballot(cpush[u]);
                if (m == 0ull) continue;
                if (cpush[u]) {
                    const int sl = qn + (int)__builtin_amdgcn_mbcnt_hi((unsigned)(m >> 32), __builtin_amdgcn_mbcnt_lo((unsigned)m, 0u));
                    qval[sl] = cval[u]; qo[sl] = (QT)ca0[u]; qo[kWalkQ + sl] = (QT)ca1[u]; qo[2 * kWalkQ + sl] = (QT)ca2[u]; qpos[sl] = cpos[u];
                }
                qn += __popcll(m);
                __builtin_amdgcn_wave_barrier();
                if (qn >= kWave) {
                    qn -= kWave;
                    const int sl = qn + lane, pk = qpos[sl];
                    deposit(pk >> 16, (pk & 0xffff) - kap, qo[sl], qo[kWalkQ + sl], qo[2 * kWalkQ + sl], qval[sl]);
                    __builtin_amdgcn_wave_barrier();
                }
            }
#pragma unroll
            for (int u = 0; u < U; ++u) {
                const unsigned long long m = __ballot(cfar[u]);
                if (m == 0ull) continue;
                if (cfar[u]) fq[fn + (int)__builtin_amdgcn_mbcnt_hi((unsigned)(m >> 32), __builtin_amdgcn_mbcnt_lo((unsigned)m, 0u))] = cpos[u];
                fn += __popcll(m);
                __builtin_amdgcn_wave_barrier();
                if (fn >= kWave) {
                    fn -= kWave;
                    far_from(fq[fn + lane]);
                    __builtin_amdgcn_wave_barrier();
                }
            }
        }
        if (lane < qn) {
            const int pk = qpos[lane];
            deposit(pk >> 16, (pk & 0xffff) - kap, qo[lane], qo[kWalkQ + lane], qo[2 * kWalkQ + lane], qval[lane]);
        }
        if (lane < fn) far_from(fq[lane]);
    } else {
    auto handle = [&](const Src &cur) {
        if (cur.ok && cur.own) sum_in += cur.val;
        if (!cur.ok || !(cur.val > 0.0)) return;
        const double val = cur.val;
        const real o0 = (real)cur.o0, o1 = (real)cur.o1, o2 = (real)cur.o2;
        const real osq = fma_(o0, o0, fma_(o1, o1, o2 * o2));
        const bool gathered = SPLIT ? (cur.hsq < (float)rows[cur.ti].lim2) : ((double)osq < rows[cur.ti].lim2);
        if (gathered) {
            if (PASS == 1) return;
            int tt[4], tk[4];
            real w[4];
            if (!regrid_gather_targets<real, false, SPLIT>(rows, rowc, NT, cur.ti, cur.x, o0, o1, o2, tt, tk, w)) return;
#pragma unroll
            for (int q4 = 0; q4 < 4; ++q4) {
                const int rr = tt[q4] - (R + 1);
                if (rr >= 0 && rr < i1 - i0) {
                    const RegRow &rt = rows[tt[q4]];
                    if (tk[q4] >= rt.ks && tk[q4] < rt.ke) {
                        const double v = (double)w[q4] * val;
                        atomicAdd(acc + rr * T.W + (tk[q4] - rt.ks), v);
                    }
                }
            }
        } else if (cur.own) {
            int tr[4], tk[4];
            double w[4];
            regrid_targets_generic(h, T.rings, rows, NT - 2, rth0, cur.ti, cur.x, (double)cur.o0, (double)cur.o1, (double)cur.o2, tr, tk, w);
            for (int q4 = 0; q4 < 4; ++q4) far_add(T.rings[tr[q4]].start + tk[q4], w[q4] * val);
        }
    };
    for (int idx = tid; idx < NR * LWs; idx += 512) {
        const Src a = fetch(idx), b = fetch(idx + 256);
        handle(a);
        handle(b);
    }
    }
    if (PASS == 1) continue;
    __syncthreads();

    const int lane = tid & (kWave - 1), wid = tid / kWave;
    for (int rr = wid; rr < i1 - i0; rr += 256 / kWave) {
        const RegRow &rt = rows[rr + R + 1];
        double *dst = map_out + rt.start + rt.ks;
        const int n = rt.ke - rt.ks;
        for (int xx = lane; xx < n; xx += kWave) {
            const double v = acc[rr * T.W + xx];
            dst[xx] = v;
            sum_out += v;
        }
    }
    if (tile_sums) {
        __syncthreads();
#pragma unroll
        for (int sft = kWave >> 1; sft > 0; sft >>= 1) { sum_in += __shfl_down(sum_in, sft, kWave); sum_out += __shfl_down(sum_out, sft, kWave); }
        if (lane == 0) { acc[2 * wid] = sum_in; acc[2 * wid + 1] = sum_out; }
        __syncthreads();
        if (tid == 0) {
            double sa_ = 0.0, sb_ = 0.0;
            for (int wv = 0; wv < 256 / kWave; ++wv) { sa_ += acc[2 * wv]; sb_ += acc[2 * wv + 1]; }
            tile_sums[2 * (int64_t)tile] = sa_; tile_sums[2 * (int64_t)tile + 1] = sb_;
        }
    }
    __syncthreads();
    }
}

__global__ void __launch_bounds__(256)
regrid_far_local_kernel(FarList far, double *__restrict__ out_slice, int64_t p0, int64_t p1, unsigned long long *__restrict__ foreign,
                        int ntiles = 0, const double *__restrict__ tile_sums = nullptr, double *__restrict__ sums = nullptr)
{
    if (tile_sums != nullptr && blockIdx.x == gridDim.x - 1) {
        __shared__ double sa[256 / kWave], sb[256 / kWave];
        double xa = 0.0, xb = 0.0;
        for (int t = threadIdx.x; t < ntiles; t += 256) { xa += tile_sums[2 * t]; xb += tile_sums[2 * t + 1]; }
#pragma unroll
        for (int sft = kWave >> 1; sft > 0; sft >>= 1) { xa += __shfl_down(xa, sft, kWave); xb += __shfl_down(xb, sft, kWave); }
        const int lane = threadIdx.x & (kWave - 1), wid = threadIdx.x / kWave;
        if (lane == 0) { sa[wid] = xa; sb[wid] = xb; }
        __syncthreads();
        if (threadIdx.x == 0) {
            double ta = 0.0, tb = 0.0;
            for (int w = 0; w < 256 / kWave; ++w) { ta += sa[w]; tb += sb[w]; }
            sums[0] = ta; sums[1] = tb;
        }
    }
    unsigned long long n = *far.count;
    if ((int64_t)n > far.cap) n = (unsigned long long)far.cap;
    for (unsigned long long i = (unsigned long long)blockIdx.x * blockDim.x + threadIdx.x; i < n; i += (unsigned long long)gridDim.x * blockDim.x) {
        const int64_t p = far.pix[i];
        if (p >= p0 && p < p1) atomicAdd(out_slice + (p - p0), far.val[i]);
        else if (foreign) atomicAdd(foreign, 1ull);
    }
}

}
```

### baryonification_amd/csrc/bfgx_shell_bands.inc

```

extern "C" {

int bfgx_plan_bands(bfgx_plan *p, int32_t *nbands, int64_t *band_first_pixel)
{
    if (!p || !nbands) return fail(BFGX_ERR_INVALID, "NULL argument");
    *nbands = p->tiling.nbands;
    if (band_first_pixel)
        for (int b = 0; b <= p->tiling.nbands; ++b) band_first_pixel[b] = band_range(p, b, b).p0;
    return BFGX_OK;
}

int bfgx_plan_band_apron(bfgx_plan *p, int32_t band0, int32_t band1, int64_t *olo, int64_t *ohi)
{
    if (!p || !olo || !ohi) return fail(BFGX_ERR_INVALID, "NULL argument");
    if (int rc = check_band_range(p, band0, band1)) return rc;
    const int64_t i0 = 1 + (int64_t)p->tiling.BR * band0, i1 = 1 + (int64_t)p->tiling.BR * band1;
    *olo = ring_first_pixel(p->hpx, i0 - p->band_reach);
    *ohi = ring_first_pixel(p->hpx, i1 + p->band_reach);
    return BFGX_OK;
}

int bfgx_plan_reach_rings(bfgx_plan *p, double max_offset, int32_t *rings)
{
    if (!p || !rings) return fail(BFGX_ERR_INVALID, "NULL argument");
    if (!(max_offset >= 0.0)) return fail(BFGX_ERR_INVALID, "max_offset must be >= 0");
    *rings = regrid_reach_rings(p->hpx.nside, std::min(max_offset * 1.001, regrid_cap(p->hpx.nside)));
    return BFGX_OK;
}

int bfgx_plan_set_band_reach(bfgx_plan *p, int32_t rings)
{
    if (!p) return fail(BFGX_ERR_INVALID, "NULL plan");
    if (rings < 1 || rings > kReachMax) return fail(BFGX_ERR_INVALID, "band reach must be 1 .. %d rings", kReachMax);
    p->band_reach = rings;
    return BFGX_OK;
}

static int regrid_bands_impl(bfgx_plan *p, int32_t band0, int32_t band1, const double *map_in_dev, const void *offsets_dev,
                             int64_t olo, int64_t ohi, const DispMode &m, double *out_slice_dev, double *sums_dev, bool reset_far,
                             bool sums_later = false)
{
    if (p->algo != 1) return fail(BFGX_ERR_UNSUPPORTED, "banded regrid needs the tiled algorithm (algo 1)");
    int64_t need_lo = 0, need_hi = 0;
    if (int rc = bfgx_plan_band_apron(p, band0, band1, &need_lo, &need_hi)) return rc;
    if (band0 == band1) {
        HIP_TRY(hipSetDevice(p->device));
        if (reset_far) HIP_TRY(hipMemsetAsync(p->far.count, 0, sizeof(unsigned long long), p->stream));
        if (sums_dev) HIP_TRY(hipMemsetAsync(sums_dev, 0, 2 * sizeof(double), p->stream));
        return BFGX_OK;
    }
    if (!map_in_dev || !offsets_dev || !out_slice_dev) return fail(BFGX_ERR_INVALID, "NULL argument");
    if (olo > need_lo || ohi < need_hi || olo < 0 || ohi > p->hpx.npix)
        return fail(BFGX_ERR_INVALID, "pix_offsets range [%lld, %lld) does not cover the bands and %d ring(s) either side [%lld, %lld)",
                    (long long)olo, (long long)ohi, p->band_reach, (long long)need_lo, (long long)need_hi);
    HIP_TRY(hipSetDevice(p->device));
    if (reset_far) HIP_TRY(hipMemsetAsync(p->far.count, 0, sizeof(unsigned long long), p->stream));
    const BandRange r = band_range(p, band0, band1);
    {
        KernelTimer kt(p, BFGX_K_REGRID);
        const size_t lds = regrid3_lds_bytes(p->tiling.BR, p->tiling.W, m.fp64() ? sizeof(double) : sizeof(float), p->band_reach > 1,
                                             m.split() ? sizeof(float) : 0);
        double *out_base = out_slice_dev - r.p0;
        const ReachArgs reach = reach_args(p, regrid_cap_for_rings(p->hpx.nside, p->band_reach));
        hipLaunchKernelGGL(tile_apron_kernel, dim3((r.nt + 255) / 256), dim3(256), 0, p->stream, p->hpx, p->tiling, (const float *)nullptr,
                           p->band_reach, reach.cap, r.t0, r.nt, p->tile_apron, (int32_t *)nullptr);
        double *ts = sums_dev ? p->tile_sums : nullptr;
        const dim3 grid(r.nt), blk(256);
        int *none = nullptr;
#define BFGX_REGRID3(ACC, REAL, SPLIT, OL)                                                                                                     \
        do {                                                                                                                                    \
            const ACC *o = (const ACC *)offsets_dev - 3 * olo;                                                                                  \
            if (p->band_reach == 1) hipLaunchKernelGGL((tile_regrid3_kernel<ACC, REAL, 0, SPLIT>), grid, blk, lds, p->stream, p->hpx, p->tiling, map_in_dev, o, OL, \
                                                       out_base, p->far, reach, ts, r.t0, r.nt, none, (double *)nullptr);                       \
            else hipLaunchKernelGGL((tile_regrid3_kernel<ACC, REAL, 2, SPLIT>), grid, blk, lds, p->stream, p->hpx, p->tiling, map_in_dev, o, OL, \
                                    out_base, p->far, reach, ts, r.t0, r.nt, none, (double *)nullptr);                                          \
        } while (0)
        if (m.split()) BFGX_REGRID3(float, double, true, m.lo(offsets_dev, ohi - olo) - 3 * olo);
        else if (m.fp64()) BFGX_REGRID3(double, double, false, (const double *)nullptr);
        else BFGX_REGRID3(float, float, false, (const float *)nullptr);
#undef BFGX_REGRID3
        HIP_TRY(hipGetLastError());
    }
    if (sums_dev && !sums_later) {
        KernelTimer kt(p, BFGX_K_SUM);
        if (int rc = launch_tile_sums(p, r.t0, r.nt, sums_dev)) return rc;
        HIP_TRY(hipGetLastError());
    }
    return BFGX_OK;
}

static int offsets_bands(bfgx_plan *p, const bfgx_catalog *cat, int32_t band0, int32_t band1, void *slice, const DispMode &m)
{
    const BandRange r = band_range(p, band0, band1);
    TileLaunch k1;
    k1.tile_lo = r.t0; k1.tile_n = r.nt;
    if (int rc = launch_k0(p, cat, 1, m.fp64())) return rc;
    k1.omax = p->arena.omax;
    return launch_offsets(p, m, slice, r.p0, r.p1, k1);
}

int bfgx_regrid_bands_device(bfgx_plan *p, int32_t band0, int32_t band1, const double *map_in_dev, const void *offsets_dev,
                             int64_t olo, int64_t ohi, int acc_f64, double *out_slice_dev, double *sums_dev)
{
    DispMode m;
    if (int rc = disp_mode(p, acc_f64, true, m)) return rc;
    return regrid_bands_impl(p, band0, band1, map_in_dev, offsets_dev, olo, ohi, m, out_slice_dev, sums_dev, true);
}

int bfgx_offsets_bands_device(bfgx_plan *p, const bfgx_catalog *cat, int32_t band0, int32_t band1, void *offsets_slice_dev, int acc_f64)
{
    if (int rc = check_scatter(p, cat, offsets_slice_dev, false, true, band0, band1)) return rc;
    if (band0 == band1) return BFGX_OK;
    DispMode m;
    if (int rc = disp_mode(p, acc_f64, true, m)) return rc;
    return offsets_bands(p, cat, band0, band1, offsets_slice_dev, m);
}

int bfgx_paint_bands_device(bfgx_plan *p, const bfgx_catalog *cat, int32_t band0, int32_t band1, void *map_slice_dev, int acc_f64)
{
    if (int rc = check_scatter(p, cat, map_slice_dev, true, true, band0, band1)) return rc;
    if (band0 == band1) return BFGX_OK;
    PaintMode m;
    if (int rc = paint_mode(p, acc_f64, m)) return rc;
    const BandRange r = band_range(p, band0, band1);
    TileLaunch k3;
    k3.tile_lo = r.t0; k3.tile_n = r.nt;
    if (int rc = launch_k0(p, cat, 0, m.k0_f64())) return rc;
    return launch_paint(p, m, map_slice_dev, r.p0, k3);
}

int bfgx_offsets_regrid_bands_device(bfgx_plan *p, const bfgx_catalog *cat, int32_t B0, int32_t B1, void *offsets_dev, int acc_f64,
                                     int32_t b0, int32_t b1, const double *map_in_dev, double *out_slice_dev, double *sums_dev,
                                     unsigned long long *foreign_dev)
{
    if (!p || !cat) return fail(BFGX_ERR_INVALID, "NULL argument");
    if (B0 < 0 || B1 > p->tiling.nbands || B0 > b0 || b1 > B1 || b0 > b1) return fail(BFGX_ERR_INVALID, "band ranges must nest: [B0, B1) around [b0, b1)");
    DispMode m;
    if (int rc = disp_mode(p, acc_f64, false, m)) return rc;
    const BandRange w = band_range(p, B0, B1), r = band_range(p, b0, b1);
    if (int rc = check_scatter(p, cat, offsets_dev, false, true, B0, B1)) return rc;
    if (B0 < B1) if (int rc = offsets_bands(p, cat, B0, B1, offsets_dev, m)) return rc;
    if (b0 == b1) {
        if (sums_dev) HIP_TRY(hipMemsetAsync(sums_dev, 0, 2 * sizeof(double), p->stream));
        return BFGX_OK;
    }
    if (int rc = regrid_bands_impl(p, b0, b1, map_in_dev, offsets_dev, w.p0, w.p1, m, out_slice_dev, sums_dev, false, true)) return rc;
    hipLaunchKernelGGL(regrid_far_local_kernel, dim3(64), dim3(256), 0, p->stream, p->far, out_slice_dev, r.p0, r.p1, foreign_dev, r.nt,
                       sums_dev ? (const double *)(p->tile_sums + 2 * (size_t)r.t0) : (const double *)nullptr, sums_dev);
    HIP_TRY(hipGetLastError());
    return BFGX_OK;
}

int bfgx_bands_max_offset2_device(bfgx_plan *p, int32_t band0, int32_t band1, float *out_dev)
{
    if (!p || !out_dev) return fail(BFGX_ERR_INVALID, "NULL argument");
    if (int rc = check_band_range(p, band0, band1, true)) return rc;
    HIP_TRY(hipSetDevice(p->device));
    HIP_TRY(hipMemsetAsync(out_dev, 0, sizeof(float), p->stream));
    const BandRange r = band_range(p, band0, band1);
    if (r.nt > 0) {
        hipLaunchKernelGGL(max_bits_kernel, dim3(1), dim3(1024), 0, p->stream, r.nt, (const unsigned *)p->arena.omax + r.t0, (unsigned *)out_dev);
        HIP_TRY(hipGetLastError());
    }
    return BFGX_OK;
}

int bfgx_plan_far_apply_device(bfgx_plan *p, double *out_slice_dev, int64_t p0, int64_t p1, unsigned long long *foreign_dev)
{
    if (!p || !out_slice_dev) return fail(BFGX_ERR_INVALID, "NULL argument");
    HIP_TRY(hipSetDevice(p->device));
    hipLaunchKernelGGL(regrid_far_local_kernel, dim3(64), dim3(256), 0, p->stream, p->far, out_slice_dev, p0, p1, foreign_dev);
    HIP_TRY(hipGetLastError());
    return BFGX_OK;
}

int bfgx_plan_far_fetch(bfgx_plan *p, int64_t cap, int64_t *pix_host, double *val_host, int64_t *n_host)
{
    if (!p || !n_host) return fail(BFGX_ERR_INVALID, "NULL argument");
    HIP_TRY(hipSetDevice(p->device));
    unsigned long long n = 0;
    HIP_TRY(hipMemcpyAsync(&n, p->far.count, sizeof(n), hipMemcpyDeviceToHost, p->stream));
    HIP_TRY(hipStreamSynchronize(p->stream));
    if ((int64_t)n > p->far.cap) return fail(BFGX_ERR_INVALID, "the regrid's list of far deposits overflowed (%lld entries)", (long long)p->far.cap);
    *n_host = (int64_t)n;
    if (n == 0 || (!pix_host && !val_host)) return BFGX_OK;
    if ((int64_t)n > cap || !pix_host || !val_host) return fail(BFGX_ERR_INVALID, "far-deposit buffers hold %lld entries, %lld are listed", (long long)cap, (long long)n);
    HIP_TRY(hipMemcpyAsync(pix_host, p->far.pix, sizeof(int64_t) * n, hipMemcpyDeviceToHost, p->stream));
    HIP_TRY(hipMemcpyAsync(val_host, p->far.val, sizeof(double) * n, hipMemcpyDeviceToHost, p->stream));
    HIP_TRY(hipStreamSynchronize(p->stream));
    return BFGX_OK;
}

int bfgx_plan_regrid_stats(bfgx_plan *p, int64_t *far_listed, int32_t *far_overflowed, int32_t *tiles_walked, int32_t *max_reach_rings)
{
    if (!p) return fail(BFGX_ERR_INVALID, "NULL plan");
    if (p->algo != 1) return fail(BFGX_ERR_UNSUPPORTED, "regrid statistics exist for the tiled algorithm (algo 1) only");
    HIP_TRY(hipSetDevice(p->device));
    RegridCtrl ctrl = {0, 0, 0};
    HIP_TRY(hipMemcpyAsync(&ctrl, p->arena.ctrl, sizeof(ctrl), hipMemcpyDeviceToHost, p->stream));
    std::vector<int32_t> apron;
    if (max_reach_rings) {
        apron.resize(2 * (size_t)p->tiling.ntiles);
        HIP_TRY(hipMemcpyAsync(apron.data(), p->tile_apron, sizeof(int32_t) * apron.size(), hipMemcpyDeviceToHost, p->stream));
    }
    HIP_TRY(hipStreamSynchronize(p->stream));
    if (far_listed) *far_listed = (int64_t)ctrl.far_count;
    if (far_overflowed) *far_overflowed = ctrl.far_overflow_full;
    if (tiles_walked) *tiles_walked = ctrl.todo_count;
    if (max_reach_rings) {
        int32_t m = 0;
        for (int t = 0; t < p->tiling.ntiles; ++t) m = std::max(m, apron[2 * (size_t)t]);
        *max_reach_rings = m;
    }
    return BFGX_OK;
}

}
```

### baryonification_amd/csrc/bfgx_tile_arena.hpp

```cpp
#pragma once
#include <cstddef>
#include <cstdint>

namespace bfgx {

struct RegridCtrl {
    unsigned long long far_count;
    int32_t far_overflow_full;
    int32_t todo_count;
};
static_assert(sizeof(RegridCtrl) == 16 && alignof(RegridCtrl) == 8, "RegridCtrl is four words, the first two a 64-bit counter");

constexpr size_t kCtrlWords = sizeof(RegridCtrl) / sizeof(int32_t);
constexpr size_t round_up4(size_t words) { return (words + 3) & ~(size_t)3; }

struct TileArenaLayout {
    size_t cnt_a_pad, cnt_b, cur_b, tile_counter, omax, ctrl, far_overflow_full, todo, todo_list, band_overflow;
    size_t cursor_words;
    size_t zeroed_words;
    size_t tail_words;
    size_t total_words;
};

constexpr TileArenaLayout tile_arena_layout(size_t ntiles, size_t cnt_pad)
{
    const size_t blk = ntiles + 1;
    TileArenaLayout L{};
    L.cnt_a_pad = 0;
    L.cnt_b = round_up4(ntiles * cnt_pad);
    L.cur_b = L.cnt_b + blk;
    L.tile_counter = L.cur_b + blk;
    L.omax = L.tile_counter + 1;
    L.ctrl = L.cnt_b + round_up4(L.omax + blk - L.cnt_b);
    L.far_overflow_full = L.ctrl + offsetof(RegridCtrl, far_overflow_full) / sizeof(int32_t);
    L.todo = L.ctrl + offsetof(RegridCtrl, todo_count) / sizeof(int32_t);
    L.todo_list = L.ctrl + kCtrlWords;
    L.band_overflow = L.todo_list + ntiles;
    L.cursor_words = L.tile_counter - L.cur_b;
    L.zeroed_words = L.ctrl + kCtrlWords;
    L.total_words = L.band_overflow + 4;
    L.tail_words = L.total_words - L.ctrl;
    return L;
}

struct TileArena {
    int32_t *base = nullptr;
    int32_t *cnt_a_pad = nullptr, *cnt_b = nullptr, *cur_b = nullptr;
    unsigned int *tile_counter = nullptr;
    float *omax = nullptr;
    RegridCtrl *ctrl = nullptr;
    int32_t *far_overflow_full = nullptr;
    int32_t *todo = nullptr;
    int32_t *band_overflow = nullptr;
    size_t cursor_bytes = 0, zeroed_bytes = 0, tail_bytes = 0;

    void bind(int32_t *b, const TileArenaLayout &L)
    {
        base = b;
        cnt_a_pad = b + L.cnt_a_pad; cnt_b = b + L.cnt_b; cur_b = b + L.cur_b;
        tile_counter = (unsigned int *)(b + L.tile_counter);
        omax = (float *)(b + L.omax);
        ctrl = (RegridCtrl *)(b + L.ctrl);
        far_overflow_full = b + L.far_overflow_full;
        todo = b + L.todo;
        band_overflow = b + L.band_overflow;
        cursor_bytes = sizeof(int32_t) * L.cursor_words;
        zeroed_bytes = sizeof(int32_t) * L.zeroed_words;
        tail_bytes = sizeof(int32_t) * L.tail_words;
    }
};

constexpr size_t kScanBlocksRoom = 1024;
struct ScanScratchLayout { size_t block_tot, block_off, total_words; };
constexpr ScanScratchLayout scan_scratch_layout()
{
    ScanScratchLayout L{};
    L.block_tot = 0;
    L.block_off = L.block_tot + kScanBlocksRoom;
    L.total_words = L.block_off + kScanBlocksRoom;
    return L;
}
struct ScanScratch {
    int32_t *block_tot = nullptr, *block_off = nullptr;
    void bind(int32_t *b, const ScanScratchLayout &L) { block_tot = b + L.block_tot; block_off = b + L.block_off; }
};

template <size_t NT, size_t PAD>
struct TileArenaCheck {
    static constexpr TileArenaLayout L = tile_arena_layout(NT, PAD);
    static constexpr size_t blk = NT + 1;
    static constexpr bool unrounded = (NT * PAD) % 4 == 0;
    static constexpr size_t n3p = round_up4(3 * blk + 1);
    static_assert(L.cnt_a_pad == 0 && L.cnt_b >= NT * PAD, "the padded counters start the arena and hold ntiles * cnt_pad words");
    static_assert(L.cur_b == L.cnt_b + blk && L.cursor_words == blk && L.tile_counter == L.cur_b + L.cursor_words,
                  "cnt_b and cur_b: ntiles + 1 words each, and nothing else lies in the cursors' span");
    static_assert(L.omax == L.tile_counter + 1, "the |offset|^2 block follows the tile counter");
    static_assert(L.ctrl >= L.omax + blk && L.ctrl - (L.omax + blk) < 4, "the control words follow the three blocks and the tile counter, rounded up to four words");
    static_assert(L.far_overflow_full == L.ctrl + 2 && L.todo == L.ctrl + 3 && L.todo_list == L.todo + 1, "count (64 bits), overflow, todo count, todo tiles");
    static_assert(L.band_overflow == L.todo_list + NT && L.total_words > L.band_overflow, "the banded overflow flag follows the todo tiles, inside the allocation");
    static_assert(L.zeroed_words == L.ctrl + kCtrlWords, "the zeroed span starts at the base and ends exactly after RegridCtrl");
    static_assert(L.zeroed_words % 4 == 0, "the zeroed span is a multiple of 16 bytes");
    static_assert(L.todo_list >= L.zeroed_words && L.band_overflow >= L.zeroed_words, "the step's memset touches neither the todo tiles nor the banded overflow flag");
    static_assert(L.ctrl % 2 == 0, "RegridCtrl's 64-bit counter is 8-byte aligned (the base is a device allocation)");
    static_assert(L.tail_words == L.total_words - L.ctrl && L.tail_words == NT + 8, "plan creation zeroes the control words and all behind them");
    static_assert(L.cnt_b == round_up4(NT * PAD) && (!unrounded || L.cnt_b == NT * PAD), "only a padded region that is no multiple of four words is rounded up");
    static_assert(L.tile_counter == L.cnt_b + 2 * blk && L.omax == L.cnt_b + 2 * blk + 1 && L.ctrl == L.cnt_b + n3p, "the three blocks, the tile counter between the second and the third");
    static_assert(L.zeroed_words == L.cnt_b + n3p + 4 && L.total_words == L.cnt_b + n3p + NT + 8, "lengths of the memset and of the allocation");
    static constexpr bool ok = true;
};
static_assert(TileArenaCheck<1, 32>::ok && TileArenaCheck<2, 32>::ok && TileArenaCheck<14, 32>::ok && TileArenaCheck<52, 32>::ok &&
              TileArenaCheck<6208, 32>::ok && TileArenaCheck<98560, 8>::ok && TileArenaCheck<393728, 2>::ok &&
              TileArenaCheck<3, 1>::ok && TileArenaCheck<12289, 1>::ok, "tile arena layout");

static_assert(scan_scratch_layout().block_tot == 0 && scan_scratch_layout().block_off == 1024 && scan_scratch_layout().total_words == 2048,
              "scan scratch: 1024 totals, then 1024 offsets: one word each per scan block");

}
```

Measured before the change: 936.6 million.

## Defer far-pixel regrid evaluation to a dedicated grid-wide kernel via source list

Far (out-of-window) source pixels found in the regrid tile kernels are now appended as (ring, k) entries to a new global source list instead of being evaluated inline. A separate regrid_far_eval_kernel with a fixed number of workgroups then processes them in parallel, and its per-workgroup sums are folded into the tile-sum reductions. The generic target search is templated over a ring-source abstraction so it can run either from tile LDS rows or from the global ring table, and tiles compute a wave-reduced span and nr range in LDS. The intent is to stop a few tiles with heavy far work from stalling the tile kernels. The cost is an extra launch, extra counters and memsets, and a source list with a fixed capacity that can overflow.

```diff
diff --git a/baryonification_amd/csrc/bfgx_api.hip b/baryonification_amd/csrc/bfgx_api.hip
--- a/baryonification_amd/csrc/bfgx_api.hip
+++ b/baryonification_amd/csrc/bfgx_api.hip
@@ -167,6 +167,7 @@
     int32_t cnt_pad = 1;
     TileRef *tref = nullptr;
     FarList far;
+    FarSrc far_src;
     int32_t *regrid_lean = nullptr;
     int auto_acc = 0;
     double table_disp_pixels = 0.0;
@@ -699,12 +700,14 @@
     const int64_t want = p->table_disp_pixels < 0.25 ? npx / 16 : (p->table_disp_pixels < 2.0 ? npx / 2 : 4 * npx);
     p->far.cap = std::min<int64_t>(std::max<int64_t>((int64_t)1 << 20, want), (int64_t)1 << 28);
     if (const char *e = std::getenv("BFGX_FAR_CAP")) p->far.cap = std::max<int64_t>(1024, std::atoll(e));
+    p->far_src.cap = p->far.cap / 4;
     if (p->mem.alloc(p->far.pix, (size_t)p->far.cap) || p->mem.alloc(p->far.val, (size_t)p->far.cap) ||
-        p->mem.alloc(p->tile_apron, 2 * (size_t)(T.ntiles + 1)))
+        p->mem.alloc(p->far_src.ent, (size_t)p->far_src.cap) || p->mem.alloc(p->tile_apron, 2 * (size_t)(T.ntiles + 1)))
         return alloc_fail("far list");
     if (p->mem.alloc(p->regrid_lean, (size_t)(T.ntiles + 4))) return alloc_fail("lean tile list");
     if (hipMemsetAsync(p->regrid_lean, 0, sizeof(int32_t) * 4, p->stream) != hipSuccess) return fail(BFGX_ERR_HIP, "hipMemset failed");
     p->far.count = &p->arena.ctrl->far_count;
+    p->far_src.count = &p->arena.ctrl->far_src_count;
     p->far.overflow = p->arena.band_overflow;
     if (hipMemsetAsync(p->arena.ctrl, 0, p->arena.tail_bytes, p->stream) != hipSuccess) return fail(BFGX_ERR_HIP, "hipMemset failed");
     return BFGX_OK;
@@ -810,7 +813,9 @@
     int32_t *scan = nullptr;
     if (p->mem.alloc(scan, SL.total_words)) return bail(alloc_fail("tile scan scratch"));
     p->scan.bind(scan, SL);
-    if (p->mem.alloc(p->tile_sums, 2 * (size_t)(p->tiling.ntiles + 1))) return bail(alloc_fail("tile sums"));
+    if (p->mem.alloc(p->tile_sums, 2 * (size_t)(p->tiling.ntiles + 1) + kFarEvalWgs)) return bail(alloc_fail("tile sums"));
+    p->far_src.sums = p->tile_sums + 2 * (size_t)(p->tiling.ntiles + 1);
+    if (hipMemsetAsync(p->far_src.sums, 0, sizeof(double) * kFarEvalWgs, p->stream) != hipSuccess) return bail(fail(BFGX_ERR_HIP, "hipMemset failed"));
     if (hipMemsetAsync(p->overflow, 0, sizeof(int32_t), p->stream) != hipSuccess) return bail(fail(BFGX_ERR_HIP, "hipMemset failed"));
     if (hipStreamSynchronize(p->stream) != hipSuccess) return bail(fail(BFGX_ERR_HIP, "stream sync failed"));
     *out = p;
@@ -1012,10 +1017,11 @@
 static int launch_tile_sums(bfgx_plan *p, int t0, int nt, double *sums_dev)
 {
     const double *ts = p->tile_sums + 2 * (size_t)t0;
-    if (nt <= kSumTilesOneWg) hipLaunchKernelGGL(sum_tiles_kernel, dim3(1), dim3(256), 0, p->stream, nt, ts, sums_dev);
+    const double *fs = p->far_src.sums;
+    if (nt <= kSumTilesOneWg) hipLaunchKernelGGL(sum_tiles_kernel, dim3(1), dim3(256), 0, p->stream, nt, ts, sums_dev, fs, kFarEvalWgs);
     else {
         HIP_TRY(hipMemsetAsync(sums_dev, 0, 2 * sizeof(double), p->stream));
-        hipLaunchKernelGGL(sum_tiles_multi_kernel, dim3(64), dim3(256), 0, p->stream, nt, ts, sums_dev);
+        hipLaunchKernelGGL(sum_tiles_multi_kernel, dim3(64), dim3(256), 0, p->stream, nt, ts, sums_dev, fs, kFarEvalWgs);
     }
     return BFGX_OK;
 }
@@ -1034,12 +1040,13 @@
     hipLaunchKernelGGL(tile_apron_kernel, dim3((nt + 255) / 256), dim3(256), 0, p->stream, p->hpx, p->tiling, (const float *)p->arena.omax, 0,
                        reach.cap, 0, nt, p->tile_apron, p->arena.todo, p->regrid_lean);
     hipLaunchKernelGGL((tile_regrid3_kernel<ACC, real, 0, SPLIT>), dim3(std::min(nt, 8 * p->num_cus)), dim3(256), lds, p->stream, p->hpx, p->tiling, map_in_dev, o, o_lo,
-                       map_out_dev, far, reach, ts, -1, nt, p->regrid_lean, (double *)nullptr);
+                       map_out_dev, far, p->far_src, reach, ts, -1, nt, p->regrid_lean, (double *)nullptr);
     hipLaunchKernelGGL((tile_regrid3_kernel<ACC, real, 2, SPLIT>), dim3(nwalk), dim3(256), lds_walk, p->stream, p->hpx, p->tiling, map_in_dev, o, o_lo,
-                       map_out_dev, far, reach, ts, -1, nt, p->arena.todo, (double *)nullptr);
+                       map_out_dev, far, p->far_src, reach, ts, -1, nt, p->arena.todo, (double *)nullptr);
+    hipLaunchKernelGGL((regrid_far_eval_kernel<ACC, SPLIT>), dim3(kFarEvalWgs), dim3(256), 0, p->stream, p->hpx, p->tiling.rings, map_in_dev, o, o_lo, p->far_src, far);
     const bool many = nt > kSumTilesOneWg && sums_dev != nullptr && ts != nullptr;
     hipLaunchKernelGGL((tile_regrid3_kernel<ACC, real, 1, SPLIT>), dim3(nfix), dim3(256), lds, p->stream, p->hpx, p->tiling, map_in_dev, o, o_lo,
-                       map_out_dev, far, reach, ts, -1, nt, p->arena.todo, many ? (double *)nullptr : sums_dev, p->regrid_lean);
+                       map_out_dev, far, p->far_src, reach, ts, -1, nt, p->arena.todo, many ? (double *)nullptr : sums_dev, p->regrid_lean);
     if (many) (void)launch_tile_sums(p, 0, nt, sums_dev);
 }
 
diff --git a/baryonification_amd/csrc/bfgx_kernels.hpp b/baryonification_amd/csrc/bfgx_kernels.hpp
--- a/baryonification_amd/csrc/bfgx_kernels.hpp
+++ b/baryonification_amd/csrc/bfgx_kernels.hpp
@@ -1857,11 +1857,12 @@
 }
 
 __global__ void __launch_bounds__(256)
-sum_tiles_kernel(int ntiles, const double *__restrict__ tile_sums, double *__restrict__ sums)
+sum_tiles_kernel(int ntiles, const double *__restrict__ tile_sums, double *__restrict__ sums, const double *__restrict__ extra = nullptr, int nextra = 0)
 {
     __shared__ double sa[256 / kWave], sb[256 / kWave];
     double xa = 0.0, xb = 0.0;
     for (int t = threadIdx.x; t < ntiles; t += 256) { xa += tile_sums[2 * t]; xb += tile_sums[2 * t + 1]; }
+    for (int t = threadIdx.x; t < nextra; t += 256) xb += extra[t];
 #pragma unroll
     for (int s = kWave >> 1; s > 0; s >>= 1) { xa += __shfl_down(xa, s, kWave); xb += __shfl_down(xb, s, kWave); }
     const int lane = threadIdx.x & (kWave - 1), wid = threadIdx.x / kWave;
@@ -1875,12 +1876,13 @@
 }
 
 __global__ void __launch_bounds__(256)
-sum_tiles_multi_kernel(int ntiles, const double *__restrict__ tile_sums, double *__restrict__ sums)
+sum_tiles_multi_kernel(int ntiles, const double *__restrict__ tile_sums, double *__restrict__ sums, const double *__restrict__ extra = nullptr, int nextra = 0)
 {
     __shared__ double sa[256 / kWave], sb[256 / kWave];
     double xa = 0.0, xb = 0.0;
     const double2 *ts = reinterpret_cast<const double2 *>(tile_sums);
     for (int t = blockIdx.x * 256 + threadIdx.x; t < ntiles; t += gridDim.x * 256) { const double2 v = ts[t]; xa += v.x; xb += v.y; }
+    if (blockIdx.x == 0) for (int t = threadIdx.x; t < nextra; t += 256) xb += extra[t];
 #pragma unroll
     for (int s = kWave >> 1; s > 0; s >>= 1) { xa += __shfl_down(xa, s, kWave); xb += __shfl_down(xb, s, kWave); }
     const int lane = threadIdx.x & (kWave - 1), wid = threadIdx.x / kWave;
diff --git a/baryonification_amd/csrc/bfgx_regrid2.hpp b/baryonification_amd/csrc/bfgx_regrid2.hpp
--- a/baryonification_amd/csrc/bfgx_regrid2.hpp
+++ b/baryonification_amd/csrc/bfgx_regrid2.hpp
@@ -28,13 +28,41 @@
 __device__ inline double row_inv_dphi(const RegRow *rows, const RegRowC<double> *, int t) { return rows[t].inv_dphi; }
 __host__ __device__ inline size_t regrowc_bytes(size_t real_size) { return real_size == 4 ? sizeof(RegRowC<float>) : sizeof(RegRowC<double>); }
 
-__device__ inline void regrid_targets_generic(const Hpx &h, const RingRec *__restrict__ rings, const RegRow *rows, int LR, int rth0, int ti, int x,
-                                                    double o0, double o1, double o2, int tr[4], int tk[4], double w[4])
+struct GenRing { double theta, inv_dphi; int nr; bool shf; };
+struct GenSrc { double theta, z, sth, dphi; int ring, k; bool shf; };
+struct GenRows {
+    const RegRow *rows; const RingRec *__restrict__ rings; int rth0, LR;
+    __device__ inline int lo() const { return rth0; }
+    __device__ inline int hi() const { return rth0 + LR + 1; }
+    __device__ inline double theta(int ir) const { return rows[ir - rth0].theta; }
+    __device__ inline GenRing ring(int ir) const
+    {
+        const int t2 = ir - rth0;
+        if (t2 >= 0 && t2 < LR + 2) { const RegRow &r2 = rows[t2]; return GenRing{r2.theta, r2.inv_dphi, r2.nr, r2.shf != 0}; }
+        const RingRec &g2 = rings[ir];
+        return GenRing{g2.theta, g2.inv_dphi, g2.nr, g2.shifted != 0};
+    }
+    __device__ inline GenSrc source(int ti, int x) const
+    {
+        const RegRow &rw = rows[ti];
+        return GenSrc{rw.theta, rw.z, rw.sth, rw.dphi, rth0 + ti, rw.ks + x, rw.shf != 0};
+    }
+};
+constexpr int kGenWalk = 17;
+struct GenTable {
+    const RingRec *__restrict__ rings; int lo_, hi_;
+    __device__ inline int lo() const { return lo_; }
+    __device__ inline int hi() const { return hi_; }
+    __device__ inline double theta(int ir) const { return rings[ir].theta; }
+    __device__ inline GenRing ring(int ir) const { const RingRec &g2 = rings[ir]; return GenRing{g2.theta, g2.inv_dphi, g2.nr, g2.shifted != 0}; }
+};
+
+template <typename RS>
+__device__ inline void regrid_targets_generic(const Hpx &h, const RS &rs, const GenSrc &src, double o0, double o1, double o2, int tr[4], int tk[4], double w[4])
 {
     const int nl4 = (int)(4 * h.nside);
-    const RegRow &rw = rows[ti];
-    const double z = rw.z, sth = rw.sth;
-    const double phi = ((double)(rw.ks + x) + (rw.shf ? 0.5 : 0.0)) * rw.dphi;
+    const double z = src.z, sth = src.sth;
+    const double phi = ((double)src.k + (src.shf ? 0.5 : 0.0)) * src.dphi;
     double s, c;
     sincos_bounded(phi, s, c);
     const double nx = sth * c + o0, ny = sth * s + o1, nz = z + o2;
@@ -47,18 +75,20 @@
     double theta, ph;
     if (xr > 0.0 && fabs(tq) <= 0.1 && fabs(q) <= 0.05) {
         ph = phi + atan_small(tq);
-        theta = rw.theta + asin_small(q);
+        theta = src.theta + asin_small(q);
     } else {
         theta = atan2_generic(sn, zc);
         ph = atan2_generic(ny, nx);
     }
     if (ph < 0) ph += kTwoPi;
     if (ph >= kTwoPi) ph -= kTwoPi;
-    int t1 = ti;
-    while (t1 > 0 && theta < rows[t1].theta) --t1;
-    while (t1 < LR + 1 && theta >= rows[t1 + 1].theta) ++t1;
-    const bool in_window = (theta >= rows[t1].theta) && (t1 < LR + 1) && (theta < rows[t1 + 1].theta);
-    const int ir1 = in_window ? rth0 + t1 : (int)ring_above(h, zc);
+    const int rlo = rs.lo(), rhi = rs.hi();
+    const int rz = (int)ring_above(h, zc);
+    int r1 = rz < rlo ? rlo : (rz > rhi ? rhi : rz);
+    while (r1 > rlo && theta < rs.theta(r1)) --r1;
+    while (r1 < rhi && theta >= rs.theta(r1 + 1)) ++r1;
+    const bool in_window = (theta >= rs.theta(r1)) && (r1 < rhi) && (theta < rs.theta(r1 + 1));
+    const int ir1 = in_window ? r1 : rz;
     const int ir2 = ir1 + 1;
     double theta1 = 0.0, theta2 = 0.0;
     for (int q4 = 0; q4 < 4; ++q4) { tr[q4] = 0; tk[q4] = 0; w[q4] = 0.0; }
@@ -66,15 +96,9 @@
     for (int half = 0; half < 2; ++half) {
         const int ir = half ? ir2 : ir1;
         if (half ? (ir < nl4) : (ir > 0)) {
-            const int t2 = ir - rth0;
-            int n2; double shd, invd, th;
-            if (t2 >= 0 && t2 < LR + 2) {
-                const RegRow &r2 = rows[t2];
-                n2 = r2.nr; shd = r2.shf ? 0.5 : 0.0; invd = r2.inv_dphi; th = r2.theta;
-            } else {
-                const RingRec &g2 = rings[ir];
-                n2 = g2.nr; shd = g2.shifted ? 0.5 : 0.0; invd = g2.inv_dphi; th = g2.theta;
-            }
+            const GenRing g2 = rs.ring(ir);
+            const int n2 = g2.nr;
+            const double shd = g2.shf ? 0.5 : 0.0, invd = g2.inv_dphi, th = g2.theta;
             const double tmp = ph * invd - shd;
             int j1 = (int)floor(tmp);
             const double w1 = tmp - (double)j1;
@@ -175,6 +199,28 @@
     int32_t *overflow;
 };
 
+constexpr int kFarEvalWgs = 1024;
+struct FarSrc {
+    unsigned int *count;
+    int2 *ent;
+    int64_t cap;
+    double *sums;
+};
+
+__device__ inline bool far_src_append(const FarSrc &fs, int ring, int k)
+{
+    const unsigned long long act = __ballot(1);
+    const int rank = (int)__builtin_amdgcn_mbcnt_hi((unsigned)(act >> 32), __builtin_amdgcn_mbcnt_lo((unsigned)act, 0u));
+    const int leader = __ffsll((long long)act) - 1;
+    unsigned base = 0;
+    if (rank == 0) base = atomicAdd(fs.count, (unsigned)__popcll(act));
+    base = (unsigned)__shfl((int)base, leader, kWave);
+    const unsigned i = base + (unsigned)rank;
+    if ((int64_t)i >= fs.cap) return false;
+    fs.ent[i] = make_int2(ring, k);
+    return true;
+}
+
 struct ReachArgs {
     const int32_t *apron;
     double cap;
@@ -186,7 +232,7 @@
 __host__ __device__ inline size_t regrid3_lds_bytes(int BR, int W, size_t real_size, bool walk = false, size_t acc_size = 0)
 {
     if (acc_size == 0) acc_size = real_size;
-    const size_t base = (size_t)BR * W * sizeof(double) + (size_t)(BR + 2 * kReachMax + 2) * (sizeof(RegRow) + regrowc_bytes(real_size)) + 16;
+    const size_t base = (size_t)BR * W * sizeof(double) + (size_t)(BR + 2 * kReachMax + 2) * (sizeof(RegRow) + regrowc_bytes(real_size)) + 16 + 32;
     if (!walk) return base;
     return base + (size_t)(BR + 2 * kReachMax + 2) * sizeof(RowScan) + (size_t)(256 / kWave) * kWalkQ * (sizeof(double) + sizeof(int32_t) + 3 * acc_size)
            + (size_t)(kWalkFar + 4) * sizeof(int32_t);
@@ -406,13 +452,13 @@
     return true;
 }
 
-__device__ inline double regrid_far_pixel(
-    const Hpx &h, const RingRec *__restrict__ rings, const RegRow *rows, int LR, int rth0, int ti, int x, double o0, double o1, double o2,
-                                                double val, FarList far)
+template <typename RS>
+__device__ inline double regrid_far_pixel(const Hpx &h, const RingRec *__restrict__ rings, const RS &rs, const GenSrc &src, double o0, double o1, double o2,
+                                          double val, FarList far)
 {
     int tr[4], tk[4];
     double w[4], tot = 0.0;
-    regrid_targets_generic(h, rings, rows, LR, rth0, ti, x, o0, o1, o2, tr, tk, w);
+    regrid_targets_generic(h, rs, src, o0, o1, o2, tr, tk, w);
     const unsigned long long act = __ballot(1);
     const int rank = (int)__builtin_amdgcn_mbcnt_hi((unsigned)(act >> 32), __builtin_amdgcn_mbcnt_lo((unsigned)act, 0u));
     const int leader = __ffsll((long long)act) - 1;
@@ -432,7 +478,7 @@
 template <typename ACC, typename real, int PASS, bool SPLIT = false>
 __global__ void __launch_bounds__(256, kK2Occ)
 tile_regrid3_kernel(Hpx h, Tiling T, const double *__restrict__ map_in, const ACC *__restrict__ offsets, const ACC *__restrict__ offsets_lo,
-                    double *__restrict__ map_out, FarList far, ReachArgs reach, double *__restrict__ tile_sums, int tile_off, int ntiles,
+                    double *__restrict__ map_out, FarList far, FarSrc fsrc, ReachArgs reach, double *__restrict__ tile_sums, int tile_off, int ntiles,
                     int *__restrict__ todo, double *__restrict__ sums_out, int *__restrict__ lean_reset = nullptr)
 {
     static_assert(!SPLIT || (sizeof(ACC) == 4 && sizeof(real) == 8), "split pix_offsets: fp32 halves, fp64 geometry");
@@ -447,6 +493,7 @@
     if (PASS == 1 && sums_out != nullptr && blockIdx.x == 0) {
         double sa = 0.0, sb = 0.0;
         for (int i = tid; i < ntiles; i += 256) { sa += tile_sums[2 * (int64_t)i]; sb += tile_sums[2 * (int64_t)i + 1]; }
+        for (int i = tid; i < kFarEvalWgs; i += 256) sb += fsrc.sums[i];
 #pragma unroll
         for (int sft = kWave >> 1; sft > 0; sft >>= 1) { sa += __shfl_down(sa, sft, kWave); sb += __shfl_down(sb, sft, kWave); }
         double *red = reinterpret_cast<double *>(smem);
@@ -508,6 +555,8 @@
     for (int i = tid; i < T.BR * T.W; i += 256) acc[i] = 0.0;
     const int NT = T.BR + 2 * R + 2;
     const int rth0 = i0 - R - 1;
+    const int NR = T.BR + 2 * R;
+    int my_span = 0, my_nrmin = 0x7fffffff, my_nrmax = 1;
     if (tid < NT) {
         const int ring = rth0 + tid;
         const RingRec g = T.rings[min(max(ring, 0), nl4)];
@@ -523,6 +572,10 @@
             rw.lim2 = (lim > 0.0 && ring > 1 && ring < nl4 - 1) ? (double)(float)(lim * lim) : 0.0;
         }
         rows[tid] = rw;
+        if (tid >= 1 && tid <= NR) {
+            my_span = rw.ke - rw.ks;
+            if (PASS == 2 && rw.nr > 0) { my_nrmin = rw.nr; my_nrmax = rw.nr; }
+        }
         RegRowC<real> rc;
         if constexpr (sizeof(real) == 4) {
             rc.z = (real)rw.z; rc.sth = (real)rw.sth; rc.dphi = (real)rw.dphi; rc.inv_dphi = (real)rw.inv_dphi;
@@ -550,24 +603,22 @@
             scan[tid] = rs;
         }
     }
-    if (PASS == 2 && tid == 0) reinterpret_cast<int32_t *>(reinterpret_cast<RowScan *>(rowc + NTmax) + NTmax)[0] = 0;
+    int32_t *tred = reinterpret_cast<int32_t *>(smem + regrid3_lds_bytes(T.BR, T.W, sizeof(real), PASS == 2, SPLIT ? sizeof(ACC) : sizeof(real)) - 32);
+    if (tid < 2 * kWave) {
+#pragma unroll
+        for (int sft = kWave >> 1; sft > 0; sft >>= 1) {
+            my_span = max(my_span, __shfl_xor(my_span, sft, kWave));
+            my_nrmin = min(my_nrmin, __shfl_xor(my_nrmin, sft, kWave));
+            my_nrmax = max(my_nrmax, __shfl_xor(my_nrmax, sft, kWave));
+        }
+        if ((tid & (kWave - 1)) == 0) { int32_t *t3 = tred + 3 * (tid / kWave); t3[0] = my_span; t3[1] = my_nrmin; t3[2] = my_nrmax; }
+    }
     __syncthreads();
-    auto far_add = [&](int64_t p, double v) {
-        if (PASS != 1) {
-            const unsigned long long i = atomicAdd(far.count, 1ull);
-            if ((int64_t)i < far.cap) { far.pix[i] = p; far.val[i] = v; } else atomicOr(far.overflow, 1);
-            sum_out += v;
-        } else {
-            atomicAdd(map_out + p, v);
-        }
+    auto far_list = [&](int ring, int k, int64_t p) {
+        if (!far_src_append(fsrc, ring, k)) { atomicOr(far.overflow, 1); sum_out += map_in[p]; }
     };
 
-    const int NR = T.BR + 2 * R;
-    int maxspan = 0, nrmin = 0x7fffffff, nrmax = 1;
-    for (int i = 1; i <= NR; ++i) {
-        maxspan = max(maxspan, rows[i].ke - rows[i].ks);
-        if (PASS == 2 && rows[i].nr > 0) { nrmin = min(nrmin, rows[i].nr); nrmax = max(nrmax, rows[i].nr); }
-    }
+    const int maxspan = max(tred[0], tred[3]), nrmin = min(tred[1], tred[4]), nrmax = max(tred[2], tred[5]);
     const int LWs = maxspan + 2 * kap;
     const unsigned inv_lws = (unsigned)((0x100000000ull + (unsigned)LWs - 1u) / (unsigned)LWs);
     using OT = typename std::conditional<SPLIT, double, ACC>::type;
@@ -644,10 +695,7 @@
             int k = rw.ks + x;
             if (k < 0) k += rw.nr;
             if (k >= rw.nr) k -= rw.nr;
-            const int64_t p = rw.start + k;
-            double f0 = (double)offsets[3 * p + 0], f1 = (double)offsets[3 * p + 1], f2 = (double)offsets[3 * p + 2];
-            if (SPLIT) { f0 += (double)offsets_lo[3 * p + 0]; f1 += (double)offsets_lo[3 * p + 1]; f2 += (double)offsets_lo[3 * p + 2]; }
-            sum_out += regrid_far_pixel(h, T.rings, rows, NT - 2, rth0, ti, x, f0, f1, f2, map_in[p], far);
+            far_list(rth0 + ti, k, rw.start + k);
         };
         int32_t *fq = farq + wid * kWalkQ;
         int fn = 0;
@@ -752,10 +800,16 @@
                 }
             }
         } else if (cur.own) {
-            int tr[4], tk[4];
-            double w[4];
-            regrid_targets_generic(h, T.rings, rows, NT - 2, rth0, cur.ti, cur.x, (double)cur.o0, (double)cur.o1, (double)cur.o2, tr, tk, w);
-            for (int q4 = 0; q4 < 4; ++q4) far_add(T.rings[tr[q4]].start + tk[q4], w[q4] * val);
+            if constexpr (PASS == 0) {
+                const RegRow &rw = rows[cur.ti];
+                far_list(rth0 + cur.ti, rw.ks + cur.x, rw.start + rw.ks + cur.x);
+            } else {
+                int tr[4], tk[4];
+                double w[4];
+                const GenRows rs{rows, T.rings, rth0, NT - 2};
+                regrid_targets_generic(h, rs, rs.source(cur.ti, cur.x), (double)cur.o0, (double)cur.o1, (double)cur.o2, tr, tk, w);
+                for (int q4 = 0; q4 < 4; ++q4) atomicAdd(map_out + (T.rings[tr[q4]].start + tk[q4]), w[q4] * val);
+            }
         }
     };
     for (int idx = tid; idx < NR * LWs; idx += 512) {
@@ -794,14 +848,53 @@
     }
 }
 
+template <typename ACC, bool SPLIT>
+__global__ void __launch_bounds__(256)
+regrid_far_eval_kernel(Hpx h, const RingRec *__restrict__ rings, const double *__restrict__ map_in, const ACC *__restrict__ offsets,
+                       const ACC *__restrict__ offsets_lo, FarSrc fsrc, FarList far)
+{
+    __shared__ double red[256 / kWave];
+    const int tid = threadIdx.x;
+    const unsigned listed = *fsrc.count;
+    if (listed == 0u) {
+        if (tid == 0) fsrc.sums[blockIdx.x] = 0.0;
+        return;
+    }
+    const unsigned n = (int64_t)listed < fsrc.cap ? listed : (unsigned)fsrc.cap;
+    if (listed > n && blockIdx.x == 0 && tid == 0) atomicAdd(far.count, 4ull * (unsigned long long)(listed - n));
+    const int nl4 = (int)(4 * h.nside);
+    double tot = 0.0;
+    for (unsigned i = blockIdx.x * 256u + (unsigned)tid; i < n; i += (unsigned)kFarEvalWgs * 256u) {
+        const int2 e = fsrc.ent[i];
+        const RingRec &g = rings[e.x];
+        const int64_t p = g.start + e.y;
+        double o0 = (double)offsets[3 * p + 0], o1 = (double)offsets[3 * p + 1], o2 = (double)offsets[3 * p + 2];
+        if (SPLIT) { o0 += (double)offsets_lo[3 * p + 0]; o1 += (double)offsets_lo[3 * p + 1]; o2 += (double)offsets_lo[3 * p + 2]; }
+        const GenTable rs{rings, max(e.x - kGenWalk, 0), min(e.x + kGenWalk, nl4)};
+        const GenSrc src{g.theta, g.z, g.sth, g.dphi, e.x, e.y, g.shifted != 0};
+        tot += regrid_far_pixel(h, rings, rs, src, o0, o1, o2, map_in[p], far);
+    }
+#pragma unroll
+    for (int sft = kWave >> 1; sft > 0; sft >>= 1) tot += __shfl_down(tot, sft, kWave);
+    if ((tid & (kWave - 1)) == 0) red[tid / kWave] = tot;
+    __syncthreads();
+    if (tid == 0) {
+        double t = 0.0;
+        for (int w = 0; w < 256 / kWave; ++w) t += red[w];
+        fsrc.sums[blockIdx.x] = t;
+    }
+}
+
 __global__ void __launch_bounds__(256)
 regrid_far_local_kernel(FarList far, double *__restrict__ out_slice, int64_t p0, int64_t p1, unsigned long long *__restrict__ foreign,
-                        int ntiles = 0, const double *__restrict__ tile_sums = nullptr, double *__restrict__ sums = nullptr)
+                        int ntiles = 0, const double *__restrict__ tile_sums = nullptr, double *__restrict__ sums = nullptr,
+                        const double *__restrict__ far_sums = nullptr)
 {
     if (tile_sums != nullptr && blockIdx.x == gridDim.x - 1) {
         __shared__ double sa[256 / kWave], sb[256 / kWave];
         double xa = 0.0, xb = 0.0;
         for (int t = threadIdx.x; t < ntiles; t += 256) { xa += tile_sums[2 * t]; xb += tile_sums[2 * t + 1]; }
+        if (far_sums != nullptr) for (int t = threadIdx.x; t < kFarEvalWgs; t += 256) xb += far_sums[t];
 #pragma unroll
         for (int sft = kWave >> 1; sft > 0; sft >>= 1) { xa += __shfl_down(xa, sft, kWave); xb += __shfl_down(xb, sft, kWave); }
         const int lane = threadIdx.x & (kWave - 1), wid = threadIdx.x / kWave;
diff --git a/baryonification_amd/csrc/bfgx_shell_bands.inc b/baryonification_amd/csrc/bfgx_shell_bands.inc
--- a/baryonification_amd/csrc/bfgx_shell_bands.inc
+++ b/baryonification_amd/csrc/bfgx_shell_bands.inc
@@ -38,14 +38,14 @@
 
 static int regrid_bands_impl(bfgx_plan *p, int32_t band0, int32_t band1, const double *map_in_dev, const void *offsets_dev,
                              int64_t olo, int64_t ohi, const DispMode &m, double *out_slice_dev, double *sums_dev, bool reset_far,
-                             bool sums_later = false)
+                             bool sums_later = false, bool src_zeroed = false)
 {
     if (p->algo != 1) return fail(BFGX_ERR_UNSUPPORTED, "banded regrid needs the tiled algorithm (algo 1)");
     int64_t need_lo = 0, need_hi = 0;
     if (int rc = bfgx_plan_band_apron(p, band0, band1, &need_lo, &need_hi)) return rc;
     if (band0 == band1) {
         HIP_TRY(hipSetDevice(p->device));
-        if (reset_far) HIP_TRY(hipMemsetAsync(p->far.count, 0, sizeof(unsigned long long), p->stream));
+        if (reset_far) HIP_TRY(hipMemsetAsync(p->far.count, 0, kFarCountersBytes, p->stream));
         if (sums_dev) HIP_TRY(hipMemsetAsync(sums_dev, 0, 2 * sizeof(double), p->stream));
         return BFGX_OK;
     }
@@ -54,7 +54,8 @@
         return fail(BFGX_ERR_INVALID, "pix_offsets range [%lld, %lld) does not cover the bands and %d ring(s) either side [%lld, %lld)",
                     (long long)olo, (long long)ohi, p->band_reach, (long long)need_lo, (long long)need_hi);
     HIP_TRY(hipSetDevice(p->device));
-    if (reset_far) HIP_TRY(hipMemsetAsync(p->far.count, 0, sizeof(unsigned long long), p->stream));
+    if (reset_far) HIP_TRY(hipMemsetAsync(p->far.count, 0, kFarCountersBytes, p->stream));
+    else if (!src_zeroed) HIP_TRY(hipMemsetAsync(p->far_src.count, 0, sizeof(uint32_t), p->stream));
     const BandRange r = band_range(p, band0, band1);
     {
         KernelTimer kt(p, BFGX_K_REGRID);
@@ -71,9 +72,10 @@
         do {                                                                                                                                    \
             const ACC *o = (const ACC *)offsets_dev - 3 * olo;                                                                                  \
             if (p->band_reach == 1) hipLaunchKernelGGL((tile_regrid3_kernel<ACC, REAL, 0, SPLIT>), grid, blk, lds, p->stream, p->hpx, p->tiling, map_in_dev, o, OL, \
-                                                       out_base, p->far, reach, ts, r.t0, r.nt, none, (double *)nullptr);                       \
+                                                       out_base, p->far, p->far_src, reach, ts, r.t0, r.nt, none, (double *)nullptr);           \
             else hipLaunchKernelGGL((tile_regrid3_kernel<ACC, REAL, 2, SPLIT>), grid, blk, lds, p->stream, p->hpx, p->tiling, map_in_dev, o, OL, \
-                                    out_base, p->far, reach, ts, r.t0, r.nt, none, (double *)nullptr);                                          \
+                                    out_base, p->far, p->far_src, reach, ts, r.t0, r.nt, none, (double *)nullptr);                              \
+            hipLaunchKernelGGL((regrid_far_eval_kernel<ACC, SPLIT>), dim3(kFarEvalWgs), blk, 0, p->stream, p->hpx, p->tiling.rings, map_in_dev, o, OL, p->far_src, p->far); \
         } while (0)
         if (m.split()) BFGX_REGRID3(float, double, true, m.lo(offsets_dev, ohi - olo) - 3 * olo);
         else if (m.fp64()) BFGX_REGRID3(double, double, false, (const double *)nullptr);
@@ -144,9 +146,9 @@
         if (sums_dev) HIP_TRY(hipMemsetAsync(sums_dev, 0, 2 * sizeof(double), p->stream));
         return BFGX_OK;
     }
-    if (int rc = regrid_bands_impl(p, b0, b1, map_in_dev, offsets_dev, w.p0, w.p1, m, out_slice_dev, sums_dev, false, true)) return rc;
+    if (int rc = regrid_bands_impl(p, b0, b1, map_in_dev, offsets_dev, w.p0, w.p1, m, out_slice_dev, sums_dev, false, true, B0 < B1)) return rc;
     hipLaunchKernelGGL(regrid_far_local_kernel, dim3(64), dim3(256), 0, p->stream, p->far, out_slice_dev, r.p0, r.p1, foreign_dev, r.nt,
-                       sums_dev ? (const double *)(p->tile_sums + 2 * (size_t)r.t0) : (const double *)nullptr, sums_dev);
+                       sums_dev ? (const double *)(p->tile_sums + 2 * (size_t)r.t0) : (const double *)nullptr, sums_dev, (const double *)p->far_src.sums);
     HIP_TRY(hipGetLastError());
     return BFGX_OK;
 }
@@ -196,7 +198,7 @@
     if (!p) return fail(BFGX_ERR_INVALID, "NULL plan");
     if (p->algo != 1) return fail(BFGX_ERR_UNSUPPORTED, "regrid statistics exist for the tiled algorithm (algo 1) only");
     HIP_TRY(hipSetDevice(p->device));
-    RegridCtrl ctrl = {0, 0, 0};
+    RegridCtrl ctrl = {};
     HIP_TRY(hipMemcpyAsync(&ctrl, p->arena.ctrl, sizeof(ctrl), hipMemcpyDeviceToHost, p->stream));
     std::vector<int32_t> apron;
     if (max_reach_rings) {
diff --git a/baryonification_amd/csrc/bfgx_tile_arena.hpp b/baryonification_amd/csrc/bfgx_tile_arena.hpp
--- a/baryonification_amd/csrc/bfgx_tile_arena.hpp
+++ b/baryonification_amd/csrc/bfgx_tile_arena.hpp
@@ -6,12 +6,16 @@
 
 struct RegridCtrl {
     unsigned long long far_count;
+    uint32_t far_src_count;
+    int32_t spare[3];
     int32_t far_overflow_full;
     int32_t todo_count;
 };
-static_assert(sizeof(RegridCtrl) == 16 && alignof(RegridCtrl) == 8, "RegridCtrl is four words, the first two a 64-bit counter");
+static_assert(sizeof(RegridCtrl) == 32 && alignof(RegridCtrl) == 8, "RegridCtrl is eight words, the first two a 64-bit counter");
+static_assert(offsetof(RegridCtrl, far_src_count) == 8 && offsetof(RegridCtrl, todo_count) == 28, "the two list counters are adjacent; the todo count is the last word");
 
-constexpr size_t kCtrlWords = sizeof(RegridCtrl) / sizeof(int32_t);
+constexpr size_t kFarCountersBytes = offsetof(RegridCtrl, far_src_count) + sizeof(uint32_t);
+constexpr size_t kCtrlWords =sizeof(RegridCtrl) / sizeof(int32_t);
 constexpr size_t round_up4(size_t words) { return (words + 3) & ~(size_t)3; }
 
 struct TileArenaLayout {
@@ -96,16 +100,16 @@
                   "cnt_b and cur_b: ntiles + 1 words each, and nothing else lies in the cursors' span");
     static_assert(L.omax == L.tile_counter + 1, "the |offset|^2 block follows the tile counter");
     static_assert(L.ctrl >= L.omax + blk && L.ctrl - (L.omax + blk) < 4, "the control words follow the three blocks and the tile counter, rounded up to four words");
-    static_assert(L.far_overflow_full == L.ctrl + 2 && L.todo == L.ctrl + 3 && L.todo_list == L.todo + 1, "count (64 bits), overflow, todo count, todo tiles");
+    static_assert(L.far_overflow_full == L.ctrl + 6 && L.todo == L.ctrl + 7 && L.todo_list == L.todo + 1, "count (64 bits), source count, three spare, overflow, todo count, todo tiles");
     static_assert(L.band_overflow == L.todo_list + NT && L.total_words > L.band_overflow, "the banded overflow flag follows the todo tiles, inside the allocation");
     static_assert(L.zeroed_words == L.ctrl + kCtrlWords, "the zeroed span starts at the base and ends exactly after RegridCtrl");
     static_assert(L.zeroed_words % 4 == 0, "the zeroed span is a multiple of 16 bytes");
     static_assert(L.todo_list >= L.zeroed_words && L.band_overflow >= L.zeroed_words, "the step's memset touches neither the todo tiles nor the banded overflow flag");
     static_assert(L.ctrl % 2 == 0, "RegridCtrl's 64-bit counter is 8-byte aligned (the base is a device allocation)");
-    static_assert(L.tail_words == L.total_words - L.ctrl && L.tail_words == NT + 8, "plan creation zeroes the control words and all behind them");
+    static_assert(L.tail_words == L.total_words - L.ctrl && L.tail_words == NT + 12, "plan creation zeroes the control words and all behind them");
     static_assert(L.cnt_b == round_up4(NT * PAD) && (!unrounded || L.cnt_b == NT * PAD), "only a padded region that is no multiple of four words is rounded up");
     static_assert(L.tile_counter == L.cnt_b + 2 * blk && L.omax == L.cnt_b + 2 * blk + 1 && L.ctrl == L.cnt_b + n3p, "the three blocks, the tile counter between the second and the third");
-    static_assert(L.zeroed_words == L.cnt_b + n3p + 4 && L.total_words == L.cnt_b + n3p + NT + 8, "lengths of the memset and of the allocation");
+    static_assert(L.zeroed_words == L.cnt_b + n3p + 8 && L.total_words == L.cnt_b + n3p + NT + 12, "lengths of the memset and of the allocation");
     static constexpr bool ok = true;
 };
 static_assert(TileArenaCheck<1, 32>::ok && TileArenaCheck<2, 32>::ok && TileArenaCheck<14, 32>::ok && TileArenaCheck<52, 32>::ok &&
```

Result: faster. 949.9 million (median of 6 runs) (+1.4%).
